# pola-rs/polars

Measured on AMD Instinct MI355X. Metric: rows/sec + achieved HBM GB/s, TPC-H Q1/Q3 SF100, 1/2/4/8 GPU vs CPU, higher is better.
Workload: dtype f64; 1 GPU; tpch_q1_sf100; rows_per_gpu=600000000, algorithmic_bytes_per_gpu_step=25200000000, parallelism=single GPU

## Files before the change

### include/polars_amd.h

```cpp
#ifndef POLARS_AMD_H
#define POLARS_AMD_H

#include <stddef.h>
#include <stdint.h>

#ifdef __cplusplus
extern "C" {
#endif

#define PLX_ABI_MAJOR 0
#define PLX_ABI_MINOR 1

#define PLX_OK 0
#define PLX_ERR_INVALID 1
#define PLX_ERR_HIP 2
#define PLX_ERR_UNSUPPORTED 3
#define PLX_ERR_OOM 4
#define PLX_ERR_SHAPE 5
#define PLX_ERR_NOT_FOUND 6
#define PLX_ERR_CANCELLED 7

typedef enum plx_dtype {
  PLX_BOOL = 0,
  PLX_I8 = 1,
// ... 226 lines not shown
  PLX_AE_CUMULATIVE = 16,
  PLX_AE_RANK = 17,
  PLX_AE_SHIFT = 18,
  PLX_AE_ROLLING = 19
} plx_aexpr_kind;

typedef enum plx_operator {
  PLX_OP_EQ = 0, PLX_OP_NE = 1, PLX_OP_LT = 2, PLX_OP_LE = 3, PLX_OP_GT = 4, PLX_OP_GE = 5,
  PLX_OP_PLUS = 6, PLX_OP_MINUS = 7, PLX_OP_MULTIPLY = 8, PLX_OP_TRUE_DIVIDE = 9,
  PLX_OP_FLOOR_DIVIDE = 10, PLX_OP_MODULUS = 11, PLX_OP_AND = 12, PLX_OP_OR = 13, PLX_OP_XOR = 14
} plx_operator;

typedef struct plx_aexpr {
  int32_t kind;
  int32_t op;
  int32_t lhs;
  int32_t rhs;
  int32_t dtype;
  int32_t is_null;
  plx_scalar lit;
  const char* name;
  int32_t cond;
} plx_aexpr;

typedef enum plx_ir_kind {
  PLX_IR_SCAN = 0,
  PLX_IR_FILTER = 1,
  PLX_IR_SELECT = 2,
  PLX_IR_HSTACK = 3,
  PLX_IR_GROUPBY = 4,
  PLX_IR_JOIN = 5,
  PLX_IR_SORT = 6,
  PLX_IR_SLICE = 7,
  PLX_IR_DISTINCT = 8
} plx_ir_kind;

typedef enum plx_join_order {
  PLX_JOIN_ORDER_NONE = 0,
  PLX_JOIN_ORDER_LEFT = 1,
  PLX_JOIN_ORDER_RIGHT = 2,
  PLX_JOIN_ORDER_LEFT_RIGHT = 3,
  PLX_JOIN_ORDER_RIGHT_LEFT = 4
} plx_join_order;

typedef struct plx_ir {
  int32_t kind;
  int32_t input;
  int32_t input_right;
  int32_t predicate;
  plx_frame frame;
  const int32_t* exprs;
  int32_t n_exprs;
  const int32_t* keys;
  int32_t n_keys;
  const int32_t* keys_right;
  int32_t n_keys_right;
  int32_t how;
  int32_t maintain_order;
  const char* suffix;
  const uint8_t* sort_descending;
  const uint8_t* sort_nulls_last;
  int64_t slice_offset;
  int64_t slice_len;
  int32_t coalesce;
} plx_ir;

#define PLX_PLAN_NO_FUSION 1u
#define PLX_PLAN_NO_PARTITION 4u
#define PLX_PLAN_NO_DIRECT_JOIN 2u

int plx_execute_plan(const plx_ir* ir, int32_t n_ir, const plx_aexpr* exprs, int32_t n_exprs, int32_t root,
                     uint32_t flags, plx_frame* out);
int plx_describe_fusion(const plx_ir* ir, int32_t n_ir, const plx_aexpr* exprs, int32_t n_exprs, int32_t root, int32_t* fusable,
                        int32_t* static_shape_id, char* why_not, size_t why_cap);
int plx_debug_program_json(const plx_ir* ir, int32_t n_ir, const plx_aexpr* exprs, int32_t n_exprs, int32_t root, char* buf, size_t cap);
int plx_jit_selftest(const plx_ir* ir, int32_t n_ir, const plx_aexpr* exprs, int32_t n_exprs, int32_t root);
int plx_jit_stats(int32_t* compiled, double* compile_ms);
int plx_jit_set_min_rows(int64_t min_rows);
const char* plx_last_plan_description(void);
const char* plx_last_plan_encodings(void);
int32_t plx_last_scan_tile_rows(void);
int32_t plx_last_lds_cells(void);
void plx_set_shared_cells(int32_t on);
int32_t plx_cell_plan(int32_t static_shape_id, int32_t n_inputs, const int32_t* dtypes, const int32_t* nullable, int32_t n_ops, const uint8_t* ops, int32_t n_aggs, const uint8_t* aggs,
                      const uint8_t* known, const int64_t* lo, const int64_t* hi, uint64_t wg_rows, uint64_t n_rows, int32_t* out);
uint64_t plx_lds_wg_rows(int64_t n_rows, int32_t grid, int32_t wide);
int32_t plx_wide_tiles_choice(int32_t compiled, int32_t knob_on, int64_t n_rows, int32_t n_inputs, const int32_t* dtypes, const int32_t* nullable, const uint64_t* values,
                              const uint64_t* validity);

int plx_datagen_lineitem_q1(int64_t n_rows, uint64_t seed, plx_column* out_cols);
int plx_datagen_lineitem_q1_host(int64_t row0, int64_t n, uint64_t seed, int64_t* shipdate, uint8_t* returnflag, uint8_t* linestatus,
                                 int64_t* quantity, double* extendedprice, double* discount, double* tax);

int plx_datagen_orders_lineitem(int64_t n_orders, uint64_t seed, plx_column* out_orders, plx_column* out_lineitem);
int plx_datagen_orders_lineitem_host(int64_t order0, int64_t n, int64_t n_orders_total, uint64_t seed, int64_t* orderkey, int64_t* custkey,
                                     int64_t* orderdate, uint32_t* n_lines, int64_t line_cap, int64_t* l_orderkey, double* l_extendedprice,
                                     double* l_discount, int64_t* l_shipdate, int64_t* n_lines_out);
int plx_datagen_customer(int64_t n_customers, uint64_t seed, plx_column* out_cols);
int plx_datagen_customer_host(int64_t row0, int64_t n, uint64_t seed, int64_t* custkey, uint8_t* segment);
int plx_datagen_uniform(int32_t dtype, int64_t n_rows, uint64_t seed, uint32_t stream, int64_t lo, int64_t hi, double scale, plx_column* out);
int plx_datagen_uniform_host(int32_t dtype, int64_t row0, int64_t n, uint64_t seed, uint32_t stream, int64_t lo, int64_t hi, double scale, void* out);
int plx_datagen_zipf(int64_t n_rows, uint64_t seed, uint32_t stream, uint64_t x0_q62, int64_t n_keys, plx_column* out);
int plx_datagen_zipf_host(int64_t row0, int64_t n, uint64_t seed, uint32_t stream, uint64_t x0_q62, int64_t n_keys, int64_t* out);

typedef uint64_t plx_strdict;
int plx_strview_dict_encode(const void* views, const uint8_t* validity, int64_t bit_offset, int64_t n, const void* const* data_buffers, const int64_t* data_sizes,
                            int32_t n_data_buffers, plx_column* out_codes, plx_strdict* out_dict);
int plx_strview_dict_encode_device(plx_column views_u64_pairs, plx_column data_u8, plx_column* out_codes, plx_strdict* out_dict);
int plx_strview_stamp_nulls(plx_column views_u64_pairs, plx_column valid_bool);
int plx_strview_groupby(plx_column views_u64_pairs, plx_column value, plx_column* out_codes, plx_strdict* out_dict, plx_column* out_sum, plx_column* out_count, plx_column* out_len);
#define PLX_STR_MATCH_MAX_PATTERN 64
typedef enum plx_str_match_kind { PLX_STR_STARTS_WITH = 0, PLX_STR_ENDS_WITH = 1, PLX_STR_CONTAINS = 2 } plx_str_match_kind;
int plx_strdict_match(plx_strdict dict, int32_t kind, const uint8_t* pattern, int64_t pattern_len, plx_column* out_bool);
int plx_strview_match(plx_column views_u64_pairs, plx_column data_u8, int32_t kind, const uint8_t* pattern, int64_t pattern_len, plx_column* out_bool);
int plx_strview_match_host(const void* views, const uint8_t* data, int64_t data_len, int64_t n, int32_t kind, const uint8_t* pattern, int64_t pattern_len,
                           uint64_t* out_bits, uint64_t* out_valid);
int plx_bitmap_lookup(plx_column codes, plx_column lut_bool, plx_column* out_bool);
int plx_strdict_info(plx_strdict dict, int64_t* n_strings, int64_t* total_bytes);

typedef enum plx_time_unit { PLX_UNIT_DATE = 0, PLX_UNIT_MS = 1, PLX_UNIT_US = 2, PLX_UNIT_NS = 3 } plx_time_unit;
typedef enum plx_temporal_part_kind {
  PLX_PART_YEAR = 0, PLX_PART_MONTH = 1, PLX_PART_DAY = 2, PLX_PART_QUARTER = 3, PLX_PART_WEEKDAY = 4, PLX_PART_ORDINAL_DAY = 5,
  PLX_PART_HOUR = 6, PLX_PART_MINUTE = 7, PLX_PART_SECOND = 8, PLX_PART_DATE = 9
} plx_temporal_part_kind;
int plx_temporal_part(plx_column col, int part, int unit, plx_column* out);
int plx_temporal_part_host(const void* values, int unit, int part, int64_t n, void* out);

int plx_strdict_to_host(plx_strdict dict, int64_t* offsets, uint8_t* bytes);
int plx_strdict_free(plx_strdict dict);
int plx_datagen_id_views(int64_t n_rows, uint64_t seed, uint32_t stream, int64_t lo, int64_t hi, plx_column* out_views);
int plx_datagen_long_id_views(int64_t n_rows, uint64_t seed, uint32_t stream, int64_t lo, int64_t hi, plx_column* out_views, plx_column* out_data);

typedef uint64_t plx_parquet;
int plx_parquet_open(const char* path, plx_parquet* out);
int plx_parquet_close(plx_parquet file);
int plx_parquet_shape(plx_parquet file, int64_t* num_rows, int32_t* num_row_groups, int32_t* num_columns);
int plx_parquet_column_info(plx_parquet file, int32_t column, const char** name, int32_t* dtype, int32_t* logical, int32_t* nullable);
int plx_parquet_column_timezone(plx_parquet file, int32_t column, const char** timezone);
int plx_parquet_row_group_info(plx_parquet file, int32_t row_group, int64_t* num_rows, int64_t* compressed_bytes);
int plx_parquet_chunk_info(plx_parquet file, int32_t row_group, int32_t column, int32_t* codec, uint32_t* encodings, int64_t* compressed_bytes,
                           int64_t* uncompressed_bytes, int32_t* has_min_max, plx_scalar* min, plx_scalar* max, int64_t* null_count);
int plx_parquet_read(plx_parquet file, const int32_t* row_groups, int32_t n_row_groups, const int32_t* columns, int32_t n_columns, plx_frame* out);
int plx_parquet_categories(plx_parquet file, int32_t column, int64_t* n_strings, int64_t* total_bytes);
int plx_parquet_categories_to_host(plx_parquet file, int32_t column, int64_t* offsets, uint8_t* bytes);
int plx_parquet_column_strdict(plx_parquet file, int32_t column, plx_strdict* out);

typedef uint64_t plx_ipc;
int plx_ipc_open(const char* path, plx_ipc* out);
int plx_ipc_close(plx_ipc file);
int plx_ipc_shape(plx_ipc file, int64_t* num_rows, int32_t* num_batches, int32_t* num_columns);
int plx_ipc_column_info(plx_ipc file, int32_t column, const char** name, int32_t* dtype, int32_t* logical, int32_t* nullable);
int plx_ipc_column_timezone(plx_ipc file, int32_t column, const char** timezone);
int plx_ipc_batch_info(plx_ipc file, int32_t batch, int64_t* num_rows, int64_t* body_bytes, int32_t* compressed);
int plx_ipc_read(plx_ipc file, const int32_t* batches, int32_t n_batches, const int32_t* columns, int32_t n_columns, plx_frame* out);
int plx_ipc_read_string_views(plx_ipc file, const int32_t* batches, int32_t n_batches, int32_t column, plx_column* out_views, plx_column* out_data);
int plx_ipc_categories(plx_ipc file, int32_t column, int64_t* n_strings, int64_t* total_bytes);
int plx_ipc_categories_to_host(plx_ipc file, int32_t column, int64_t* offsets, uint8_t* bytes);
int plx_ipc_column_strdict(plx_ipc file, int32_t column, plx_strdict* out);

typedef uint64_t plx_comm;
int plx_comm_unique_id(uint8_t* out_128_bytes);
int plx_comm_init(const uint8_t* unique_id_128_bytes, int32_t rank, int32_t world_size, plx_comm* out);
int plx_comm_info(plx_comm comm, int32_t* rank, int32_t* world_size);
int plx_comm_free(plx_comm comm);
int plx_exchange_by_key(plx_comm comm, plx_frame frame, const char* key, uint64_t seed, plx_frame* out, uint64_t* rows_sent, uint64_t* bytes_sent);
int plx_allgather_frame(plx_comm comm, plx_frame frame, plx_frame* out);
// ... 52 lines not shown
```

### polars_amd/_ffi.py

```python
from __future__ import annotations

import ctypes as C
import os
import threading
from typing import Optional

os.environ.setdefault("GPU_MAX_HW_QUEUES", "8")

_HERE = os.path.dirname(os.path.abspath(__file__))
LIB_PATH = os.path.join(_HERE, "libpolars_amd.so")

BOOL, I8, I16, I32, I64, U8, U16, U32, U64, F32, F64 = range(11)
EQ, NE, LT, LE, GT, GE = range(6)
ADD, SUB, MUL, TRUE_DIV, FLOOR_DIV, MOD = range(6)
AND, OR, XOR = range(3)
AGG_SUM, AGG_MEAN, AGG_MIN, AGG_MAX, AGG_COUNT, AGG_LEN, AGG_FIRST, AGG_VAR, AGG_STD = range(9)
AGG_QUANTILE = 9
AGG_N_UNIQUE = 10
UNIQUE_ANY, UNIQUE_FIRST, UNIQUE_LAST, UNIQUE_NONE = range(4)
UNIQUE_KEEPS = {"any": UNIQUE_ANY, "first": UNIQUE_FIRST, "last": UNIQUE_LAST, "none": UNIQUE_NONE}
QUANTILE_NEAREST, QUANTILE_LOWER, QUANTILE_HIGHER, QUANTILE_MIDPOINT, QUANTILE_LINEAR = range(5)
QUANTILE_INTERPOLATIONS = {"nearest": QUANTILE_NEAREST, "lower": QUANTILE_LOWER, "higher": QUANTILE_HIGHER, "midpoint": QUANTILE_MIDPOINT, "linear": QUANTILE_LINEAR}
JOIN_INNER, JOIN_LEFT, JOIN_SEMI, JOIN_ANTI, JOIN_FULL, JOIN_RIGHT = range(6)
JOIN_COALESCE_DEFAULT, JOIN_COALESCE, JOIN_KEEP_BOTH = range(3)
# ... 153 lines not shown
    "plx_parquet_column_strdict": (C.c_int, [C.c_uint64, C.c_int32, _u64p]),
    "plx_ipc_open": (C.c_int, [C.c_char_p, _u64p]),
    "plx_ipc_close": (C.c_int, [C.c_uint64]),
    "plx_ipc_shape": (C.c_int, [C.c_uint64, _i64p, _i32p, _i32p]),
    "plx_ipc_column_info": (C.c_int, [C.c_uint64, C.c_int32, C.POINTER(C.c_char_p), _i32p, _i32p, _i32p]),
    "plx_ipc_column_timezone": (C.c_int, [C.c_uint64, C.c_int32, C.POINTER(C.c_char_p)]),
    "plx_ipc_batch_info": (C.c_int, [C.c_uint64, C.c_int32, _i64p, _i64p, _i32p]),
    "plx_ipc_read": (C.c_int, [C.c_uint64, _i32p, C.c_int32, _i32p, C.c_int32, _u64p]),
    "plx_ipc_read_string_views": (C.c_int, [C.c_uint64, _i32p, C.c_int32, C.c_int32, _u64p, _u64p]),
    "plx_ipc_categories": (C.c_int, [C.c_uint64, C.c_int32, _i64p, _i64p]),
    "plx_ipc_categories_to_host": (C.c_int, [C.c_uint64, C.c_int32, C.c_void_p, C.c_void_p]),
    "plx_ipc_column_strdict": (C.c_int, [C.c_uint64, C.c_int32, _u64p]),
    "plx_comm_unique_id": (C.c_int, [C.c_void_p]),
    "plx_comm_init": (C.c_int, [C.c_void_p, C.c_int32, C.c_int32, _u64p]),
    "plx_comm_info": (C.c_int, [C.c_uint64, C.POINTER(C.c_int32), C.POINTER(C.c_int32)]),
    "plx_comm_free": (C.c_int, [C.c_uint64]),
    "plx_exchange_by_key": (C.c_int, [C.c_uint64, C.c_uint64, C.c_char_p, C.c_uint64, _u64p, _u64p, _u64p]),
    "plx_allgather_frame": (C.c_int, [C.c_uint64, C.c_uint64, _u64p]),
    "plx_column_import_arrow": (C.c_int, [C.POINTER(ArrowArray), C.POINTER(ArrowSchema), _u64p]),
    "plx_column_import_series": (C.c_int, [C.POINTER(SeriesExport), _u64p]),
    "plx_column_export_arrow": (C.c_int, [C.c_uint64, C.POINTER(ArrowArray), C.POINTER(ArrowSchema)]),
    "plx_column_export_series": (C.c_int, [C.c_uint64, C.c_char_p, C.POINTER(SeriesExport)]),
    "plx_column_to_host": (C.c_int, [C.c_uint64, C.c_void_p, C.c_void_p, _i32p]),
    "plx_column_copy_to_device": (C.c_int, [C.c_uint64, C.c_void_p, C.c_void_p]),
    "plx_column_info": (C.c_int, [C.c_uint64, _i32p, _i64p, _i64p]),
    "plx_column_device_ptrs": (C.c_int, [C.c_uint64, C.POINTER(C.c_void_p), C.POINTER(C.c_void_p)]),
    "plx_column_retain": (C.c_int, [C.c_uint64]),
    "plx_column_free": (C.c_int, [C.c_uint64]),
    "plx_cmp": (C.c_int, [C.c_int, C.c_uint64, C.c_uint64, _u64p]),
    "plx_cmp_scalar": (C.c_int, [C.c_int, C.c_uint64, Scalar, _u64p]),
    "plx_bitmap_binop": (C.c_int, [C.c_int, C.c_uint64, C.c_uint64, _u64p]),
    "plx_bitmap_not": (C.c_int, [C.c_uint64, _u64p]),
    "plx_arith": (C.c_int, [C.c_int, C.c_uint64, C.c_uint64, _u64p]),
    "plx_arith_scalar": (C.c_int, [C.c_int, C.c_uint64, Scalar, C.c_int, _u64p]),
    "plx_cast": (C.c_int, [C.c_uint64, C.c_int, _u64p]),
    "plx_if_then_else": (C.c_int, [C.c_uint64, C.c_uint64, C.c_uint64, _u64p]),
    "plx_filter": (C.c_int, [C.c_uint64, C.c_uint64, _u64p]),
    "plx_gather": (C.c_int, [C.c_uint64, C.c_uint64, _u64p]),
    "plx_reduce": (C.c_int, [C.c_int, C.c_uint64, C.POINTER(Scalar), _i32p, _i32p]),
    "plx_reduce_var": (C.c_int, [C.c_uint64, C.c_int32, C.c_int32, C.POINTER(Scalar), _i32p, _i32p]),
    "plx_groupby_agg": (C.c_int, [_u64p, C.c_int32, _u64p, _i32p, C.c_int32, C.c_int32, _u64p, _u64p]),
    "plx_groupby_agg_ddof": (C.c_int, [_u64p, C.c_int32, _u64p, _i32p, C.c_int32, C.c_int32, _i32p, _u64p, _u64p]),
    "plx_reduce_quantile": (C.c_int, [C.c_uint64, C.c_double, C.c_int32, C.POINTER(Scalar), _i32p, _i32p]),
    "plx_groupby_agg_params": (C.c_int, [_u64p, C.c_int32, _u64p, _i32p, C.c_int32, C.c_int32, _i32p, C.POINTER(C.c_double), _i32p, _u64p, _u64p]),
    "plx_window_agg": (C.c_int, [_u64p, C.c_int32, _u64p, _i32p, C.c_int32, _i32p, C.POINTER(C.c_double), _i32p, _u64p]),
    "plx_cumulative": (C.c_int, [_u64p, C.c_int32, C.c_uint64, C.c_int32, C.c_int32, _u64p]),
    "plx_rank": (C.c_int, [_u64p, C.c_int32, C.c_uint64, C.c_int32, C.c_int32, _u64p]),
    "plx_shift": (C.c_int, [_u64p, C.c_int32, C.c_uint64, C.c_int64, C.POINTER(Scalar), C.c_int32, _u64p]),
    "plx_rolling": (C.c_int, [_u64p, C.c_int32, C.c_uint64, C.c_int32, C.c_int64, C.c_int64, C.c_int32, _u64p]),
    "plx_join_indices": (C.c_int, [C.c_int, C.c_uint64, C.c_uint64, _u64p, _u64p]),
    "plx_datagen_lineitem_q1": (C.c_int, [C.c_int64, C.c_uint64, _u64p]),
    "plx_datagen_lineitem_q1_host": (C.c_int, [C.c_int64, C.c_int64, C.c_uint64, C.c_void_p, C.c_void_p, C.c_void_p, C.c_void_p, C.c_void_p, C.c_void_p, C.c_void_p]),
    "plx_datagen_orders_lineitem": (C.c_int, [C.c_int64, C.c_uint64, _u64p, _u64p]),
    "plx_datagen_orders_lineitem_host": (C.c_int, [C.c_int64, C.c_int64, C.c_int64, C.c_uint64, C.c_void_p, C.c_void_p, C.c_void_p, C.c_void_p, C.c_int64,
                                                   C.c_void_p, C.c_void_p, C.c_void_p, C.c_void_p, _i64p]),
    "plx_datagen_uniform": (C.c_int, [C.c_int32, C.c_int64, C.c_uint64, C.c_uint32, C.c_int64, C.c_int64, C.c_double, _u64p]),
    "plx_datagen_customer": (C.c_int, [C.c_int64, C.c_uint64, _u64p]),
    "plx_datagen_customer_host": (C.c_int, [C.c_int64, C.c_int64, C.c_uint64, C.c_void_p, C.c_void_p]),
    "plx_datagen_uniform_host": (C.c_int, [C.c_int32, C.c_int64, C.c_int64, C.c_uint64, C.c_uint32, C.c_int64, C.c_int64, C.c_double, C.c_void_p]),
    "plx_datagen_zipf": (C.c_int, [C.c_int64, C.c_uint64, C.c_uint32, C.c_uint64, C.c_int64, _u64p]),
    "plx_datagen_zipf_host": (C.c_int, [C.c_int64, C.c_int64, C.c_uint64, C.c_uint32, C.c_uint64, C.c_int64, C.c_void_p]),
    "plx_debug_program_json": (C.c_int, [C.POINTER(IR), C.c_int32, C.POINTER(AExpr), C.c_int32, C.c_int32, C.c_char_p, C.c_size_t]),
    "plx_reduce_n_unique": (C.c_int, [C.c_uint64, C.POINTER(C.c_uint32)]),
    "plx_distinct_mask": (C.c_int, [_u64p, C.c_int32, C.c_int32, _u64p]),
    "plx_sort_indices": (C.c_int, [_u64p, C.c_int32, C.POINTER(C.c_uint8), C.POINTER(C.c_uint8), C.c_int64, _u64p]),
    "plx_hash_partition": (C.c_int, [C.c_uint64, C.c_int32, C.c_uint64, _u64p, _i64p]),
    "plx_frame_new": (C.c_int, [C.POINTER(C.c_char_p), _u64p, C.c_int32, _u64p]),
    "plx_frame_free": (C.c_int, [C.c_uint64]),
    "plx_frame_concat": (C.c_int, [_u64p, C.c_int32, _u64p]),
    "plx_frame_shape": (C.c_int, [C.c_uint64, _i64p, _i32p]),
    "plx_frame_column": (C.c_int, [C.c_uint64, C.c_int32, C.POINTER(C.c_char_p), _u64p]),
    "plx_frame_dtypes": (C.c_int, [C.c_uint64, _i32p]),
    "plx_frame_to_host": (C.c_int, [C.c_uint64, C.POINTER(C.c_void_p), C.POINTER(C.c_void_p), _i32p]),
    "plx_execute_plan": (C.c_int, [C.POINTER(IR), C.c_int32, C.POINTER(AExpr), C.c_int32, C.c_int32, C.c_uint32, _u64p]),
    "plx_describe_fusion": (C.c_int, [C.POINTER(IR), C.c_int32, C.POINTER(AExpr), C.c_int32, C.c_int32, _i32p, _i32p, C.c_char_p, C.c_size_t]),
    "plx_jit_selftest": (C.c_int, [C.POINTER(IR), C.c_int32, C.POINTER(AExpr), C.c_int32, C.c_int32]),
    "plx_jit_stats": (C.c_int, [_i32p, C.POINTER(C.c_double)]),
    "plx_jit_set_min_rows": (C.c_int, [C.c_int64]),
    "plx_last_plan_description": (C.c_char_p, []),
    "plx_last_plan_encodings": (C.c_char_p, []),
    "plx_last_scan_tile_rows": (C.c_int32, []),
    "plx_last_lds_cells": (C.c_int32, []),
    "plx_set_shared_cells": (None, [C.c_int32]),
    "plx_cell_plan": (C.c_int32, [C.c_int32, C.c_int32, C.POINTER(C.c_int32), C.POINTER(C.c_int32), C.c_int32, C.POINTER(C.c_uint8), C.c_int32, C.POINTER(C.c_uint8),
                                  C.POINTER(C.c_uint8), C.POINTER(C.c_int64), C.POINTER(C.c_int64), C.c_uint64, C.c_uint64, C.POINTER(C.c_int32)]),
    "plx_lds_wg_rows": (C.c_uint64, [C.c_int64, C.c_int32, C.c_int32]),
    "plx_wide_tiles_choice": (C.c_int32, [C.c_int32, C.c_int32, C.c_int64, C.c_int32, C.POINTER(C.c_int32), C.POINTER(C.c_int32), C.POINTER(C.c_uint64), C.POINTER(C.c_uint64)]),
    "plx_profile_enable": (C.c_int, [C.c_int]),
    "plx_profile_fetch": (C.c_int, [C.POINTER(ProfileRecord), C.c_int32, _i32p]),
    "plx_profile_clear": (C.c_int, []),
}

_lib: Optional[C.CDLL] = None


def lib() -> C.CDLL:
    global _lib
    if _lib is None:
        if not os.path.exists(LIB_PATH):
            raise ImportError(
                f"{LIB_PATH} is missing: build the HIP extension first "
                "(python -c 'import __graft_entry__ as g; g.build()' or make -C polars_amd/csrc). "
                "There is no CPU fallback in polars_amd.")
        l = C.CDLL(LIB_PATH, mode=C.RTLD_GLOBAL)
        for name, (res, args) in SIGNATURES.items():
            fn = getattr(l, name)
            fn.restype = res
            fn.argtypes = args
        _lib = l
    return _lib


def check(status: int) -> None:
    if status != 0:
        msg = lib().plx_last_error().decode("utf-8", "replace")
        if status == ERR_UNSUPPORTED:
            raise UnsupportedError(status, msg)
        raise PlxError(status, msg)


_initialised = False


def init(device: Optional[int] = None) -> None:
    global _initialised
    if device is None:
        device = int(os.environ.get("LOCAL_RANK", "0"))
    check(lib().plx_init(device))
    _initialised = True


def ensure_init() -> None:
    if not _initialised:
        init()


_tls = threading.local()


def set_plan_note(note) -> None:
    _tls.plan_note = note


def last_plan() -> str:
    note = getattr(_tls, "plan_note", None)
    return note if note is not None else lib().plx_last_plan_description().decode()


def last_plan_encodings() -> str:
    return lib().plx_last_plan_encodings().decode()


def last_scan_tile_rows() -> int:
    return int(lib().plx_last_scan_tile_rows())


def last_lds_cells() -> int:
    return int(lib().plx_last_lds_cells())


def set_shared_cells(on: bool) -> None:
    lib().plx_set_shared_cells(int(bool(on)))


def cell_plan(facts, wg_rows, n_rows, static_shape_id=-1, dtypes=(), nullable=(), ops=(), aggs=()):
    n_aggs = len(facts)
    ni, no = len(dtypes), len(ops)
    out = (C.c_int32 * (2 + 2 * 16))()
    flat_ops = [int(x) for op in ops for x in op]
    flat_aggs = [int(x) for a in aggs for x in a]
    r = lib().plx_cell_plan(int(static_shape_id), ni, (C.c_int32 * max(ni, 1))(*[int(d) for d in dtypes]), (C.c_int32 * max(ni, 1))(*[int(x) for x in nullable]),
                            no, (C.c_uint8 * max(len(flat_ops), 1))(*flat_ops), len(aggs), (C.c_uint8 * max(len(flat_aggs), 1))(*flat_aggs),
                            (C.c_uint8 * 16)(*[int(f[0]) for f in facts]), (C.c_int64 * 16)(*[int(f[1]) for f in facts]), (C.c_int64 * 16)(*[int(f[2]) for f in facts]),
                            int(wg_rows), int(n_rows), out)
    if r < 0:
        raise ValueError("plx_cell_plan: bad arguments")
    return int(out[0]), int(out[1]), [int(out[2 + k]) for k in range(r)], [int(out[2 + r + k]) for k in range(r)]


def wide_tiles_choice(compiled, knob_on, n_rows, dtypes, nullable, values, validity) -> int:
    n = len(dtypes)
    return int(lib().plx_wide_tiles_choice(int(bool(compiled)), int(bool(knob_on)), int(n_rows), n, (C.c_int32 * n)(*[int(d) for d in dtypes]),
                                           (C.c_int32 * n)(*[int(bool(x)) for x in nullable]), (C.c_uint64 * n)(*[int(v) for v in values]), (C.c_uint64 * n)(*[int(v) for v in validity])))


def jit_set_min_rows(min_rows: int) -> None:
    check(lib().plx_jit_set_min_rows(int(min_rows)))


def encoded_set_decimal_min_rows(min_rows: int) -> None:
    check(lib().plx_encoded_set_decimal_min_rows(int(min_rows)))


def encoded_decimal_min_rows() -> int:
    return int(lib().plx_encoded_decimal_min_rows())


def jit_stats():
    n, ms = C.c_int32(), C.c_double()
    check(lib().plx_jit_stats(C.byref(n), C.byref(ms)))
    return n.value, ms.value
```

### polars_amd/csrc/abi.cpp

```cpp
#include <cstdio>
#include <cstring>
#include <memory>
#include <mutex>

#include "core.hpp"
#include "datagen_device.hpp"
#include "distinct.hpp"
#include "encoded_inputs.hpp"
#include "engine.hpp"
#include "fused_shapes.hpp"
#include "jit.hpp"
#include "join.hpp"
#include "kernels.hpp"
#include "kernels_fused.hpp"
#include "ops.hpp"
#include "cumulative.hpp"
#include "quantile.hpp"
#include "rolling.hpp"
#include "scan.hpp"
#include "sort.hpp"
#include "strmatch.hpp"
#include "temporal.hpp"

namespace plx {
// ... 543 lines not shown
  PLX_REQUIRE(by && n_by > 0 && out_idx, PLX_ERR_INVALID, "sort_indices: need at least one key column");
  std::vector<sort::SortKey> keys;
  for (int i = 0; i < n_by; i++) {
    sort::SortKey k;
    k.col = get_column(by[i]); k.descending = descending && descending[i]; k.nulls_last = nulls_last && nulls_last[i];
    keys.push_back(k);
  }
  std::string d;
  ColumnPtr idx = sort::sort_indices(keys, limit, &d);
  t_plan_desc = d;
  *out_idx = register_column(idx);
  PLX_CATCH
}

int plx_hash_partition(plx_column key, int32_t n_partitions, uint64_t seed, plx_column* out_perm, int64_t* counts_out) {
  PLX_TRY
  PLX_REQUIRE(out_perm && counts_out, PLX_ERR_INVALID, "null pointer");
  ColumnPtr perm;
  join::hash_partition(get_column(key), n_partitions, seed, perm, counts_out);
  *out_perm = register_column(perm);
  PLX_CATCH
}

int plx_frame_new(const char* const* names, const plx_column* cols, int32_t n_cols, plx_frame* out) {
  PLX_TRY
  PLX_REQUIRE(out && (n_cols == 0 || (names && cols)), PLX_ERR_INVALID, "null pointer");
  auto f = std::make_shared<Frame>();
  for (int i = 0; i < n_cols; i++) {
    ColumnPtr c = get_column(cols[i]);
    if (i == 0) f->height = c->len;
    PLX_REQUIRE(c->len == f->height, PLX_ERR_SHAPE, std::string("frame columns have different lengths (") + names[i] + ")");
    PLX_REQUIRE(f->find(names[i]) < 0, PLX_ERR_INVALID, std::string("duplicate column name ") + names[i]);
    f->names.push_back(names[i]); f->cols.push_back(c);
  }
  *out = register_frame(f);
  PLX_CATCH
}
int plx_frame_free(plx_frame f) { PLX_TRY free_frame(f); PLX_CATCH }
int plx_frame_concat(const plx_frame* frames, int32_t n_frames, plx_frame* out) {
  PLX_TRY
  PLX_REQUIRE(frames && out && n_frames >= 1, PLX_ERR_INVALID, "frame_concat: bad arguments");
  std::vector<FramePtr> fs;
  for (int32_t i = 0; i < n_frames; i++) fs.push_back(get_frame(frames[i]));
  auto o = std::make_shared<Frame>();
  o->names = fs[0]->names;
  for (const FramePtr& f : fs) {
    PLX_REQUIRE(f->names == o->names, PLX_ERR_SHAPE, "frame_concat: frames have different columns");
    o->height += f->height;
  }
  for (size_t c = 0; c < o->names.size(); c++) {
    std::vector<ColumnPtr> chunks;
    for (const FramePtr& f : fs) chunks.push_back(f->cols[c]);
    o->cols.push_back(ops::concat(chunks));
  }
  *out = register_frame(o);
  PLX_CATCH
}
int plx_frame_shape(plx_frame f, int64_t* height, int32_t* width) {
  PLX_TRY
  FramePtr fr = get_frame(f);
  if (height) *height = fr->height;
  if (width) *width = (int32_t)fr->cols.size();
  PLX_CATCH
}
int plx_frame_column(plx_frame f, int32_t i, const char** name_out, plx_column* col_out) {
  PLX_TRY
  FramePtr fr = get_frame(f);
  PLX_REQUIRE(i >= 0 && i < (int)fr->cols.size(), PLX_ERR_INVALID, "column index out of range");
  if (name_out) *name_out = fr->names[i].c_str();
  if (col_out) *col_out = register_column(fr->cols[i]);
  PLX_CATCH
}

int plx_frame_dtypes(plx_frame f, int32_t* dtypes_out) {
  PLX_TRY
  FramePtr fr = get_frame(f);
  PLX_REQUIRE(dtypes_out || fr->cols.empty(), PLX_ERR_INVALID, "null pointer");
  for (size_t i = 0; i < fr->cols.size(); i++) dtypes_out[i] = fr->cols[i]->dtype;
  PLX_CATCH
}
int plx_frame_to_host(plx_frame f, void* const* values_out, uint8_t* const* validity_out, int32_t* has_validity_out) {
  PLX_TRY
  FramePtr fr = get_frame(f);
  {
    struct Piece { const void* src; void* dst; size_t bytes; };
    std::vector<Piece> pieces;
    size_t total = 0;
    bool ok = pinned_bounce() != nullptr;
    for (size_t i = 0; ok && i < fr->cols.size(); i++) {
      const ColumnPtr& c = fr->cols[i];
      if (!(c->values || c->len == 0)) { ok = false; break; }
      const size_t vb = c->dtype == PLX_BOOL ? (size_t)((c->len + 7) / 8) : (size_t)c->len * dtype_width(c->dtype);
      const size_t nb = (size_t)((c->len + 7) / 8);
      if (values_out && values_out[i] && vb) { pieces.push_back({c->values->ptr, values_out[i], vb}); total += (vb + 15) & ~size_t(15); }
      if (validity_out && validity_out[i] && nb && c->validity) { pieces.push_back({c->validity->ptr, validity_out[i], nb}); total += (nb + 15) & ~size_t(15); }
      if (total > kBounceBytes) ok = false;
    }
    if (ok && !pieces.empty()) {
      Buf staging = dev_alloc(total);
      std::vector<size_t> offs(pieces.size());
      size_t at = 0;
      for (size_t j = 0; j < pieces.size(); j++) { offs[j] = at; at += (pieces[j].bytes + 15) & ~size_t(15); }
      for (size_t base = 0; base < pieces.size(); base += k::kPackMax) {
        k::PackBatch b{}; b.n = (int)std::min<size_t>(k::kPackMax, pieces.size() - base);
        for (int j = 0; j < b.n; j++) { b.src[j] = pieces[base + j].src; b.bytes[j] = (uint32_t)pieces[base + j].bytes; b.off[j] = (uint32_t)offs[base + j]; }
        k::pack_buffers(b, staging->ptr);
      }
      std::lock_guard<std::mutex> lk(bounce_mutex());
      uint8_t* host = reinterpret_cast<uint8_t*>(pinned_bounce());
      PLX_HIP(hipMemcpyAsync(host, staging->ptr, total, hipMemcpyDeviceToHost, stream()));
      PLX_HIP(hipStreamSynchronize(stream()));
      for (size_t j = 0; j < pieces.size(); j++) memcpy(pieces[j].dst, host + offs[j], pieces[j].bytes);
      for (size_t i = 0; i < fr->cols.size(); i++) {
        const ColumnPtr& c = fr->cols[i];
        const size_t nb = (size_t)((c->len + 7) / 8);
        if (validity_out && validity_out[i] && nb && !c->validity) memset(validity_out[i], 0xff, nb);
        if (has_validity_out) has_validity_out[i] = c->validity ? 1 : 0;
      }
      return PLX_OK;
    }
    if (ok && pieces.empty() && !fr->cols.empty()) {
      for (size_t i = 0; i < fr->cols.size(); i++) if (has_validity_out) has_validity_out[i] = fr->cols[i]->validity ? 1 : 0;
      return PLX_OK;
    }
  }
  for (size_t i = 0; i < fr->cols.size(); i++) {
    const ColumnPtr& c = fr->cols[i];
    PLX_REQUIRE(c->values || c->len == 0, PLX_ERR_INVALID, "placeholder column has no data");
    const size_t vb = c->dtype == PLX_BOOL ? (size_t)((c->len + 7) / 8) : (size_t)c->len * dtype_width(c->dtype);
    const size_t nb = (size_t)((c->len + 7) / 8);
    if (values_out && values_out[i] && vb) PLX_HIP(hipMemcpyAsync(values_out[i], c->values->ptr, vb, hipMemcpyDeviceToHost, stream()));
    if (validity_out && validity_out[i] && nb) {
      if (c->validity) PLX_HIP(hipMemcpyAsync(validity_out[i], c->validity->ptr, nb, hipMemcpyDeviceToHost, stream()));
      else memset(validity_out[i], 0xff, nb);
    }
    if (has_validity_out) has_validity_out[i] = c->validity ? 1 : 0;
  }
  PLX_HIP(hipStreamSynchronize(stream()));
  PLX_CATCH
}

extern "C++" {
namespace {
thread_local std::string t_plugin_error;
struct PluginCtx { uint64_t bitflags; };

hipStream_t plugin_thread_stream() {
  static thread_local hipStream_t s = nullptr;
  if (!s) PLX_HIP(hipStreamCreateWithFlags(&s, hipStreamNonBlocking));
  return s;
}
std::string pickle_str_value(const uint8_t* kw, size_t n, const char* key) {
  std::vector<std::string> toks;
  for (size_t i = 0; i < n;) {
    const uint8_t c = kw[i];
    size_t len = 0, hdr = 0;
    if ((c == 0x8c || c == 'U') && i + 1 < n) { len = kw[i + 1]; hdr = 2; }
    else if (c == 'X' && i + 4 < n) { len = (size_t)kw[i + 1] | ((size_t)kw[i + 2] << 8) | ((size_t)kw[i + 3] << 16) | ((size_t)kw[i + 4] << 24); hdr = 5; }
    if (hdr && i + hdr + len <= n) { toks.emplace_back((const char*)kw + i + hdr, len); i += hdr + len; }
    else i++;
  }
  for (size_t i = 0; i + 1 < toks.size(); i++) if (toks[i] == key) return toks[i + 1];
  return "";
}
long long pickle_int_value(const uint8_t* kw, size_t n, const char* key, long long absent) {
  const size_t klen = strlen(key);
// ... 536 lines not shown
    for (uint32_t q = 0; q < r.n_lines; q++, at++) {
      if (!want_lines) continue;
      PLX_REQUIRE(at < line_cap, PLX_ERR_INVALID, "datagen: line arrays too small");
      const datagen::Q3LineRow lr = datagen::q3_line_row(seed, (uint64_t)(order0 + j), q, r.orderdate);
      if (l_orderkey) l_orderkey[at] = r.orderkey;
      if (l_extendedprice) l_extendedprice[at] = lr.extendedprice;
      if (l_discount) l_discount[at] = lr.discount;
      if (l_shipdate) l_shipdate[at] = lr.shipdate;
    }
  }
  if (n_lines_out) *n_lines_out = at;
  PLX_CATCH
}
int plx_datagen_customer(int64_t n_customers, uint64_t seed, plx_column* out_cols) {
  PLX_TRY
  PLX_REQUIRE(n_customers >= 0 && out_cols, PLX_ERR_INVALID, "datagen: bad arguments");
  ColumnPtr k = make_column(PLX_I64, n_customers, false), sgm = make_column(PLX_U8, n_customers, false);
  k->null_count = 0; sgm->null_count = 0;
  k::datagen_customer(n_customers, seed, k->values->as<int64_t>(), sgm->values->as<uint8_t>());
  out_cols[0] = register_column(k); out_cols[1] = register_column(sgm);
  PLX_CATCH
}
int plx_datagen_customer_host(int64_t row0, int64_t n, uint64_t seed, int64_t* custkey, uint8_t* segment) {
  PLX_TRY
  PLX_REQUIRE(row0 >= 0 && n >= 0, PLX_ERR_INVALID, "datagen: bad arguments");
  for (int64_t j = 0; j < n; j++) {
    if (custkey) custkey[j] = row0 + j + 1;
    if (segment) segment[j] = datagen::customer_segment(seed, (uint64_t)(row0 + j + 1));
  }
  PLX_CATCH
}
int plx_datagen_uniform(int32_t dtype, int64_t n_rows, uint64_t seed, uint32_t stream_id, int64_t lo, int64_t hi, double scale, plx_column* out) {
  PLX_TRY
  PLX_REQUIRE(n_rows >= 0 && out && hi > lo && stream_id < 8, PLX_ERR_INVALID, "datagen: bad arguments");
  PLX_REQUIRE(dtype == PLX_I64 || dtype == PLX_U32 || dtype == PLX_F64, PLX_ERR_UNSUPPORTED, "datagen_uniform: dtype must be Int64, UInt32 or Float64");
  ColumnPtr c = make_column(dtype, n_rows, false); c->null_count = 0;
  k::datagen_uniform(dtype, n_rows, seed, stream_id, lo, hi, scale, c->values->ptr);
  *out = register_column(c);
  PLX_CATCH
}
int plx_datagen_uniform_host(int32_t dtype, int64_t row0, int64_t n, uint64_t seed, uint32_t stream_id, int64_t lo, int64_t hi, double scale, void* out) {
  PLX_TRY
  PLX_REQUIRE(row0 >= 0 && n >= 0 && (out || n == 0) && hi > lo && stream_id < 8, PLX_ERR_INVALID, "datagen: bad arguments");
  PLX_REQUIRE(dtype == PLX_I64 || dtype == PLX_U32 || dtype == PLX_F64, PLX_ERR_UNSUPPORTED, "datagen_uniform: dtype must be Int64, UInt32 or Float64");
  for (int64_t j = 0; j < n; j++) {
    const int64_t v = datagen::uniform_value(seed, stream_id, (uint64_t)(row0 + j), lo, hi);
    if (dtype == PLX_I64) reinterpret_cast<int64_t*>(out)[j] = v;
    else if (dtype == PLX_U32) reinterpret_cast<uint32_t*>(out)[j] = (uint32_t)v;
    else reinterpret_cast<double*>(out)[j] = (double)v * scale;
  }
  PLX_CATCH
}

int plx_datagen_zipf(int64_t n_rows, uint64_t seed, uint32_t stream_id, uint64_t x0_q62, int64_t n_keys, plx_column* out) {
  PLX_TRY
  PLX_REQUIRE(n_rows >= 0 && out && n_keys > 0 && stream_id < 8 && x0_q62 > 0 && x0_q62 < (1ull << 62), PLX_ERR_INVALID, "datagen_zipf: bad arguments");
  ColumnPtr c = make_column(PLX_I64, n_rows, false); c->null_count = 0;
  k::datagen_zipf(n_rows, seed, stream_id, x0_q62, n_keys, c->values->as<int64_t>());
  *out = register_column(c);
  PLX_CATCH
}
int plx_datagen_zipf_host(int64_t row0, int64_t n, uint64_t seed, uint32_t stream_id, uint64_t x0_q62, int64_t n_keys, int64_t* out) {
  PLX_TRY
  PLX_REQUIRE(row0 >= 0 && n >= 0 && (out || n == 0) && n_keys > 0 && stream_id < 8 && x0_q62 > 0 && x0_q62 < (1ull << 62), PLX_ERR_INVALID, "datagen_zipf: bad arguments");
  for (int64_t j = 0; j < n; j++) out[j] = datagen::zipf_value(seed, stream_id, (uint64_t)(row0 + j), x0_q62, n_keys);
  PLX_CATCH
}

int plx_execute_plan(const plx_ir* ir, int32_t n_ir, const plx_aexpr* exprs, int32_t n_exprs, int32_t root, uint32_t flags, plx_frame* out) {
  PLX_TRY
  PLX_REQUIRE(out, PLX_ERR_INVALID, "null out pointer");
  engine::Plan p = engine::import_plan(ir, n_ir, exprs, n_exprs, flags);
  FramePtr f = engine::execute(p, root);
  t_plan_desc = p.desc;
  t_plan_encoded = p.encoded;
  *out = register_frame(f);
  PLX_CATCH
}
const char* plx_last_plan_description(void) { return t_plan_desc.c_str(); }
const char* plx_last_plan_encodings(void) { return t_plan_encoded.c_str(); }
int32_t plx_last_scan_tile_rows(void) { return k::last_scan_tile_rows(); }
int32_t plx_last_lds_cells(void) { return k::last_lds_cells(); }
void plx_set_shared_cells(int32_t on) { k::set_shared_cells(on != 0); }
uint64_t plx_lds_wg_rows(int64_t n_rows, int32_t grid, int32_t wide) { return (n_rows < 0 || grid < 1) ? 0 : k::lds_agg_wg_rows_of(n_rows, grid, wide != 0); }
int32_t plx_cell_plan(int32_t static_shape_id, int32_t n_inputs, const int32_t* dtypes, const int32_t* nullable, int32_t n_ops, const uint8_t* ops, int32_t n_aggs, const uint8_t* aggs,
                      const uint8_t* known, const int64_t* lo, const int64_t* hi, uint64_t wg_rows, uint64_t n_rows, int32_t* out) {
  if (!known || !lo || !hi || !out) return -1;
  fused::Shape sh{};
  if (static_shape_id >= 0) {
    if (static_shape_id >= fused::kNumStaticShapes) return -1;
    sh = fused::static_shape(static_shape_id);
  } else {
    if (n_inputs < 0 || n_inputs > fused::kMaxInputs || n_ops < 0 || n_ops > fused::kMaxOps || n_aggs < 0 || n_aggs > fused::kMaxAggs) return -1;
    if ((n_inputs && (!dtypes || !nullable)) || (n_ops && !ops) || (n_aggs && !aggs)) return -1;
    sh.n_inputs = (uint8_t)n_inputs; sh.n_ops = (uint8_t)n_ops; sh.n_aggs = (uint8_t)n_aggs; sh.pred = fused::kNone; sh.key = fused::kNone;
    for (int i = 0; i < n_inputs; i++) { sh.in_dtype[i] = (uint8_t)dtypes[i]; sh.in_nullable[i] = (uint8_t)(nullable[i] != 0); }
    for (int i = 0; i < n_ops; i++) sh.ops[i] = fused::Op{ops[5 * i], ops[5 * i + 1], ops[5 * i + 2], ops[5 * i + 3], ops[5 * i + 4], {0, 0, 0}};
    for (int i = 0; i < n_aggs; i++) sh.aggs[i] = fused::Agg{aggs[2 * i], aggs[2 * i + 1]};
  }
  fused::AggFacts f{};
  f.wg_rows = wg_rows; f.n_rows = n_rows;
  for (int k = 0; k < sh.n_aggs; k++) { f.known[k] = known[k]; f.lo[k] = lo[k]; f.hi[k] = hi[k]; }
  const fused::CellPlan p = fused::plan_cells(sh, f);
  out[0] = p.n_cells; out[1] = p.shift;
  for (int k = 0; k < sh.n_aggs; k++) { out[2 + k] = p.cell[k]; out[2 + sh.n_aggs + k] = p.from[k] == fused::kNone ? -1 : (int)p.from[k]; }
  return sh.n_aggs;
}
int32_t plx_wide_tiles_choice(int32_t compiled, int32_t knob_on, int64_t n_rows, int32_t n_inputs, const int32_t* dtypes, const int32_t* nullable, const uint64_t* values,
                              const uint64_t* validity) {
  if (n_inputs < 0 || n_inputs > fused::kMaxInputs || (n_inputs && (!dtypes || !nullable || !values || !validity))) return -1;
  fused::Shape sh{}; fused::Args args{};
  sh.n_inputs = (uint8_t)n_inputs; sh.pred = fused::kNone; sh.key = fused::kNone;
  args.n_rows = n_rows;
  for (int i = 0; i < n_inputs; i++) {
    sh.in_dtype[i] = (uint8_t)dtypes[i]; sh.in_nullable[i] = (uint8_t)(nullable[i] != 0);
    args.in[i].values = (const void*)(uintptr_t)values[i]; args.in[i].validity = (const uint64_t*)(uintptr_t)validity[i];
  }
  return k::wide_tiles_choice(sh, args, compiled != 0, knob_on != 0) ? 1 : 0;
}

int plx_debug_program_json(const plx_ir* ir, int32_t n_ir, const plx_aexpr* exprs, int32_t n_exprs, int32_t root, char* buf, size_t cap) {
  PLX_TRY
  PLX_REQUIRE(buf && cap > 0, PLX_ERR_INVALID, "null buffer");
  engine::Plan p = engine::import_plan(ir, n_ir, exprs, n_exprs, 0);
  std::string json, why;
  if (!engine::dump_program_json(p, root, &json, &why)) fail(PLX_ERR_UNSUPPORTED, "not a fusable pipeline: " + why);
  PLX_REQUIRE(json.size() + 1 <= cap, PLX_ERR_INVALID, "buffer too small for the program dump (" + std::to_string(json.size() + 1) + " bytes)");
  memcpy(buf, json.c_str(), json.size() + 1);
  PLX_CATCH
}

int plx_describe_fusion(const plx_ir* ir, int32_t n_ir, const plx_aexpr* exprs, int32_t n_exprs, int32_t root, int32_t* fusable, int32_t* static_shape_id,
                        char* why_not, size_t why_cap) {
  PLX_TRY
  engine::Plan p = engine::import_plan(ir, n_ir, exprs, n_exprs, 0);
  auto dump = [](const fused::Shape& sh) {
    std::string d = "inputs=" + std::to_string(sh.n_inputs) + " pred=" + std::to_string(sh.pred) + " key=" + std::to_string(sh.key) + " ops=[";
    for (int i = 0; i < sh.n_ops; i++) d += "(" + std::to_string(sh.ops[i].code) + "," + std::to_string(sh.ops[i].dst) + "," + std::to_string(sh.ops[i].a) + "," + std::to_string(sh.ops[i].b) + "," + std::to_string(sh.ops[i].c) + ")";
    d += "] aggs=[";
    for (int i = 0; i < sh.n_aggs; i++) d += "(" + std::to_string(sh.aggs[i].kind) + "," + std::to_string(sh.aggs[i].src) + ")";
    d += "] in_dtype=[";
    for (int i = 0; i < sh.n_inputs; i++) d += std::to_string(sh.in_dtype[i]) + (sh.in_nullable[i] ? "?" : "") + ",";
    d += "]";
    if (sh.n_keys) { d += " keys=["; for (int i = 0; i < sh.n_keys; i++) d += std::to_string(sh.keys[i]) + ","; d += "]"; }
    return d;
  };
  std::string why;
  int sid = -1;
  bool ok;
  PLX_REQUIRE(root >= 0 && root < (int)p.ir.size(), PLX_ERR_INVALID, "bad root");
  const engine::IRN& rn = p.ir[root];
  if (rn.kind == PLX_IR_GROUPBY && rn.input >= 0 && p.ir[rn.input].kind == PLX_IR_JOIN) {
    std::vector<fused::Shape> shapes;
    ok = engine::describe_join_fusion(p, root, &shapes, &why);
    if (ok) {
      sid = fused::find_static_shape(shapes[2]);
      t_plan_desc = dump(shapes[0]);
      for (size_t i = 1; i < shapes.size(); i++) t_plan_desc += "\n" + dump(shapes[i]);
    }
  } else {
    fused::Shape sh{};
    ok = engine::describe_fusion(p, root, &sh, &sid, &why);
    if (ok) t_plan_desc = dump(sh);
  }
  if (fusable) *fusable = ok ? 1 : 0;
  if (static_shape_id) *static_shape_id = sid;
// ... 103 lines not shown
  Buf codes, dviews, svalid;
  int64_t nd = 0, snulls = 0;
  k::strview_dict_encode(views, validity_holder ? validity_holder->valid_words() : nullptr, data ? data->as<uint8_t>() : nullptr, buf_base ? buf_base->as<uint64_t>() : nullptr, n, &codes, &dviews, &nd,
                         from_stamps && !validity_holder ? &svalid : nullptr, &snulls);
  auto c = std::make_shared<Column>();
  c->dtype = PLX_U32; c->len = n; c->values = codes;
  if (validity_holder && validity_holder->validity) c->validity = validity_holder->validity;
  else if (snulls > 0) { c->validity = svalid; c->null_count = snulls; }
  else c->null_count = 0;
  if (nd > 0) { c->range_state = 1; c->range_min = 0; c->range_max = nd - 1; c->range_trusted = true; }
  auto d = std::make_unique<StrDict>();
  d->views = dviews; d->data = data; d->n = nd;
  *out_codes = register_column(c);
  *out_dict = register_strdict(std::move(d));
}
}
namespace plx {
void strview_encode_device(const uint64_t* views, const ColumnPtr& validity_holder, Buf data, int64_t n, plx_column* out_codes, plx_strdict* out_dict) {
  Buf bb = dev_alloc_zero(8);
  encode_on_device(views, validity_holder, data, bb, n, out_codes, out_dict);
}
void strview_encode_device_bases(const uint64_t* views, const ColumnPtr& validity_holder, Buf data, Buf buf_base, int64_t n, plx_column* out_codes, plx_strdict* out_dict) {
  encode_on_device(views, validity_holder, data, buf_base, n, out_codes, out_dict);
}
}
}

int plx_strview_dict_encode(const void* views, const uint8_t* validity, int64_t bit_offset, int64_t n, const void* const* data_buffers, const int64_t* data_sizes,
                            int32_t n_data_buffers, plx_column* out_codes, plx_strdict* out_dict) {
  PLX_TRY
  PLX_REQUIRE(out_codes && out_dict && n >= 0 && (views || n == 0) && n_data_buffers >= 0 && (n_data_buffers == 0 || (data_buffers && data_sizes)), PLX_ERR_INVALID, "strview_dict_encode: bad arguments");
  device();
  Buf dv = dev_alloc((size_t)std::max<int64_t>(n, 1) * 16);
  if (n) h2d_sync_pinned(dv->ptr, views, (size_t)n * 16);
  ColumnPtr vh;
  if (validity) {
    std::vector<uint8_t> zeros((size_t)n);
    vh = column_from_host(PLX_U8, zeros.data(), validity, bit_offset, n);
  }
  uint64_t total = 0;
  std::vector<uint64_t> base((size_t)std::max(n_data_buffers, 1), 0);
  for (int i = 0; i < n_data_buffers; i++) { base[i] = total; total += (uint64_t)data_sizes[i]; }
  Buf data = dev_alloc((size_t)total + 64), bb = dev_alloc(sizeof(uint64_t) * base.size());
  for (int i = 0; i < n_data_buffers; i++) {
    if (!data_sizes[i]) continue;
    if ((uint64_t)data_sizes[i] >= ((uint64_t)32 << 20)) h2d_sync_pinned((uint8_t*)data->ptr + base[i], data_buffers[i], (size_t)data_sizes[i]);
    else h2d_async((uint8_t*)data->ptr + base[i], data_buffers[i], (size_t)data_sizes[i]);
  }
  h2d_async(bb->ptr, base.data(), sizeof(uint64_t) * base.size());
  PLX_HIP(hipStreamSynchronize(stream()));
  encode_on_device(dv->as<uint64_t>(), vh, data, bb, n, out_codes, out_dict);
  PLX_CATCH
}
int plx_strview_dict_encode_device(plx_column views_u64_pairs, plx_column data_u8, plx_column* out_codes, plx_strdict* out_dict) {
  PLX_TRY
  PLX_REQUIRE(out_codes && out_dict, PLX_ERR_INVALID, "null pointer");
  ColumnPtr v = get_column(views_u64_pairs);
  PLX_REQUIRE(v->dtype == PLX_U64 && v->len % 2 == 0 && (v->values || v->len == 0), PLX_ERR_INVALID, "views must be a UInt64 column of 2 n words");
  Buf data, bb = dev_alloc_zero(8);
  if (data_u8) { ColumnPtr d = get_column(data_u8); PLX_REQUIRE(d->dtype == PLX_U8, PLX_ERR_INVALID, "data must be a UInt8 column"); data = d->values; }
  const int64_t n = v->len / 2;
  encode_on_device(v->values ? v->values->as<uint64_t>() : nullptr, nullptr, data, bb, n, out_codes, out_dict, true);
  PLX_CATCH
}
int plx_strview_stamp_nulls(plx_column views_u64_pairs, plx_column valid_bool) {
  PLX_TRY
  ColumnPtr v = get_column(views_u64_pairs), m = get_column(valid_bool);
  PLX_REQUIRE(v->dtype == PLX_U64 && v->len % 2 == 0, PLX_ERR_INVALID, "views must be a UInt64 column of 2 n words");
  PLX_REQUIRE(m->dtype == PLX_BOOL, PLX_ERR_INVALID, "the validity of the views is a Boolean column (true = valid: the array's validity bitmap as its values)");
  PLX_REQUIRE(m->len == v->len / 2, PLX_ERR_SHAPE, "validity column and views differ in length");
  PLX_REQUIRE((v->values && m->values) || v->len == 0, PLX_ERR_INVALID, "placeholder column has no data");
  if (!v->len) return PLX_OK;
  ColumnPtr eff = m;
  if (m->validity) {
    auto a = std::make_shared<Column>(); a->dtype = PLX_BOOL; a->len = m->len; a->values = m->values; a->null_count = 0;
    auto b = std::make_shared<Column>(); b->dtype = PLX_BOOL; b->len = m->len; b->values = m->validity; b->null_count = 0;
    eff = ops::bool_binop(PLX_AND, a, b);
  }
  if (!v->values->owned || v->values.use_count() > 1) {
    Buf copy = dev_alloc(v->values->bytes);
    PLX_HIP(hipMemcpyAsync(copy->ptr, v->values->ptr, v->values->bytes, hipMemcpyDeviceToDevice, stream()));
    v->values = copy;
  }
  k::strview_stamp_nulls(v->values->as<uint64_t>(), eff->values->as<uint64_t>(), m->len);
  PLX_HIP(hipStreamSynchronize(stream()));
  PLX_CATCH
}
extern "C++" {
namespace {
void check_match_args(int32_t kind, const uint8_t* pattern, int64_t pattern_len) {
  PLX_REQUIRE(kind >= PLX_STR_STARTS_WITH && kind <= PLX_STR_CONTAINS, PLX_ERR_INVALID, "string match: kind outside 0..2 (plx_str_match_kind)");
  PLX_REQUIRE(pattern_len >= 0 && (pattern || pattern_len == 0), PLX_ERR_INVALID, "string match: bad pattern");
  PLX_REQUIRE(pattern_len <= PLX_STR_MATCH_MAX_PATTERN, PLX_ERR_UNSUPPORTED,
              "string match: a pattern of " + std::to_string(pattern_len) + " bytes; patterns of more than " + std::to_string(PLX_STR_MATCH_MAX_PATTERN) + " bytes are not on this path");
}
void check_match_flags(uint32_t flags) {
  PLX_REQUIRE(!(flags & strmatch::kFlagOutside), PLX_ERR_INVALID, "string match: a view points outside its buffer");
  PLX_REQUIRE(!(flags & strmatch::kFlagNoData), PLX_ERR_INVALID, "string match: a string of more than 12 bytes needs the data buffer for this predicate, and none was given");
}
ColumnPtr bool_column(int64_t n, Buf values, Buf validity, int64_t null_count) {
  auto c = std::make_shared<Column>();
  c->dtype = PLX_BOOL; c->len = n; c->values = std::move(values); c->validity = std::move(validity); c->null_count = null_count;
  return c;
}
}
}
static_assert(PLX_STR_MATCH_MAX_PATTERN == strmatch::kMaxPattern && PLX_STR_STARTS_WITH == strmatch::kStartsWith && PLX_STR_ENDS_WITH == strmatch::kEndsWith && PLX_STR_CONTAINS == strmatch::kContains,
              "polars_amd.h and strmatch.hpp disagree");

int plx_strdict_match(plx_strdict dict, int32_t kind, const uint8_t* pattern, int64_t pattern_len, plx_column* out_bool) {
  PLX_TRY
  PLX_REQUIRE(out_bool, PLX_ERR_INVALID, "null pointer");
  check_match_args(kind, pattern, pattern_len);
  StrDict& d = get_strdict(dict);
  device();
  Buf bits = dev_alloc(bitmap_bytes(d.n)), valid = dev_alloc(bitmap_bytes(d.n));
  const uint32_t flags = k::strview_match(d.views->as<uint64_t>(), nullptr, false, d.data ? d.data->as<uint8_t>() : nullptr, d.data ? (uint64_t)d.data->bytes : 0, true, d.n,
                                          kind, pattern, pattern_len, bits->as<uint64_t>(), valid->as<uint64_t>());
  check_match_flags(flags);
  *out_bool = register_column(bool_column(d.n, bits, nullptr, 0));
  PLX_CATCH
}
int plx_strview_match(plx_column views_u64_pairs, plx_column data_u8, int32_t kind, const uint8_t* pattern, int64_t pattern_len, plx_column* out_bool) {
  PLX_TRY
  PLX_REQUIRE(out_bool, PLX_ERR_INVALID, "null pointer");
  check_match_args(kind, pattern, pattern_len);
  ColumnPtr v = get_column(views_u64_pairs);
  PLX_REQUIRE(v->dtype == PLX_U64 && v->len % 2 == 0, PLX_ERR_INVALID, "views must be a UInt64 column of 2 n words");
  PLX_REQUIRE(v->values || v->len == 0, PLX_ERR_INVALID, "placeholder column has no data");
  PLX_REQUIRE(!v->validity || column_null_count(v) == 0, PLX_ERR_INVALID, "views column carries a validity bitmap with nulls: the nulls of a raw view column are stamped views (plx_strview_stamp_nulls)");
  Buf data;
  uint64_t data_len = 0;
  if (data_u8) {
    ColumnPtr d = get_column(data_u8);
    PLX_REQUIRE(d->dtype == PLX_U8, PLX_ERR_INVALID, "data must be a UInt8 column");
    PLX_REQUIRE(d->values || d->len == 0, PLX_ERR_INVALID, "placeholder column has no data");
    data = d->values; data_len = (uint64_t)d->len;
  }
  device();
  const int64_t n = v->len / 2;
  Buf bits = dev_alloc(bitmap_bytes(n)), valid = dev_alloc(bitmap_bytes(n));
  const uint32_t flags = k::strview_match(v->values ? v->values->as<uint64_t>() : nullptr, nullptr, true, data ? data->as<uint8_t>() : nullptr, data_len, false, n,
                                          kind, pattern, pattern_len, bits->as<uint64_t>(), valid->as<uint64_t>());
  check_match_flags(flags);
  const int64_t n_valid = n ? k::bitmap_popcount(valid->as<uint64_t>(), n) : 0;
  *out_bool = register_column(n_valid == n ? bool_column(n, bits, nullptr, 0) : bool_column(n, bits, valid, n - n_valid));
  PLX_CATCH
}
int plx_strview_match_host(const void* views, const uint8_t* data, int64_t data_len, int64_t n, int32_t kind, const uint8_t* pattern, int64_t pattern_len, uint64_t* out_bits,
                           uint64_t* out_valid) {
  PLX_TRY
  PLX_REQUIRE(n >= 0 && (views || n == 0) && (out_bits && out_valid || n == 0) && data_len >= 0, PLX_ERR_INVALID, "strview_match_host: bad arguments");
  check_match_args(kind, pattern, pattern_len);
  const strmatch::Pattern pat = strmatch::make_pattern(pattern, pattern_len);
  const strmatch::Pool pool{data, data ? (uint64_t)data_len : 0, 0};
  const uint32_t flags = strmatch::match_views_host(views, pool, n, kind, pat, out_bits, out_valid);
  check_match_flags(flags);
  PLX_CATCH
}
int plx_bitmap_lookup(plx_column codes, plx_column lut_bool, plx_column* out_bool) {
  PLX_TRY
  PLX_REQUIRE(out_bool, PLX_ERR_INVALID, "null pointer");
  *out_bool = register_column(ops::bitmap_lookup(get_column(codes), get_column(lut_bool)));
  PLX_CATCH
}

// ... 129 lines not shown
```

### polars_amd/csrc/comm.cpp

```cpp
#include <dlfcn.h>

#include <algorithm>
#include <cstring>
#include <mutex>

#include "core.hpp"
#include "join.hpp"
#include "ops.hpp"

namespace plx {
namespace {

typedef struct { char internal[128]; } NcclId;
typedef void* NcclComm;
enum { kNcclUint8 = 1, kNcclInt64 = 4 };
struct Rccl {
  void* so = nullptr;
  int (*GetUniqueId)(NcclId*) = nullptr;
  int (*CommInitRank)(NcclComm*, int, NcclId, int) = nullptr;
  int (*CommDestroy)(NcclComm) = nullptr;
  int (*CommCount)(const NcclComm, int*) = nullptr;
  int (*CommUserRank)(const NcclComm, int*) = nullptr;
  int (*Send)(const void*, size_t, int, int, NcclComm, hipStream_t) = nullptr;
  int (*Recv)(void*, size_t, int, int, NcclComm, hipStream_t) = nullptr;
  int (*AllGather)(const void*, void*, size_t, int, NcclComm, hipStream_t) = nullptr;
  int (*GroupStart)() = nullptr;
  int (*GroupEnd)() = nullptr;
  const char* (*GetErrorString)(int) = nullptr;
};
Rccl& rccl() {
  static Rccl r;
  static std::once_flag once;
  std::call_once(once, [] {
    for (const char* name : {"librccl.so.1", "librccl.so", "/opt/rocm/lib/librccl.so.1"}) { r.so = dlopen(name, RTLD_NOW | RTLD_GLOBAL); if (r.so) break; }
    if (!r.so) return;
    auto sym = [&](const char* n) { return dlsym(r.so, n); };
    r.GetUniqueId = (decltype(r.GetUniqueId))sym("ncclGetUniqueId");
    r.CommInitRank = (decltype(r.CommInitRank))sym("ncclCommInitRank");
    r.CommDestroy = (decltype(r.CommDestroy))sym("ncclCommDestroy");
    r.CommCount = (decltype(r.CommCount))sym("ncclCommCount");
    r.CommUserRank = (decltype(r.CommUserRank))sym("ncclCommUserRank");
    r.Send = (decltype(r.Send))sym("ncclSend");
    r.Recv = (decltype(r.Recv))sym("ncclRecv");
    r.AllGather = (decltype(r.AllGather))sym("ncclAllGather");
    r.GroupStart = (decltype(r.GroupStart))sym("ncclGroupStart");
    r.GroupEnd = (decltype(r.GroupEnd))sym("ncclGroupEnd");
    r.GetErrorString = (decltype(r.GetErrorString))sym("ncclGetErrorString");
  });
  if (!r.so || !r.GetUniqueId || !r.CommInitRank || !r.Send || !r.Recv || !r.AllGather || !r.GroupStart || !r.GroupEnd)
    fail(PLX_ERR_HIP, "librccl could not be loaded (multi-GPU exchange needs RCCL)");
  return r;
}
void nccl_check(int rc, const char* what) {
  if (rc != 0) fail(PLX_ERR_HIP, std::string(what) + ": " + (rccl().GetErrorString ? rccl().GetErrorString(rc) : "rccl error") + " (" + std::to_string(rc) + ")");
}

struct Comm { NcclComm nccl = nullptr; int rank = 0, ws = 1; };

constexpr size_t kP2PChunk = size_t(1) << 29;
void send_chunked(const uint8_t* src, size_t bytes, int peer, Comm& c) {
  for (size_t o = 0; o < bytes; o += kP2PChunk) nccl_check(rccl().Send(src + o, std::min(kP2PChunk, bytes - o), kNcclUint8, peer, c.nccl, stream()), "ncclSend");
}
void recv_chunked(uint8_t* dst, size_t bytes, int peer, Comm& c) {
  for (size_t o = 0; o < bytes; o += kP2PChunk) nccl_check(rccl().Recv(dst + o, std::min(kP2PChunk, bytes - o), kNcclUint8, peer, c.nccl, stream()), "ncclRecv");
}
std::mutex g_comm_mu;
std::vector<std::unique_ptr<Comm>> g_comms;

Comm& get_comm(uint64_t h) {
  std::lock_guard<std::mutex> lk(g_comm_mu);
  if (h == 0 || h > g_comms.size() || !g_comms[h - 1]) fail(PLX_ERR_INVALID, "invalid communicator handle");
  return *g_comms[h - 1];
}

std::vector<int64_t> allgather_i64(Comm& c, const Buf& send, size_t n) {
  const int ws = c.ws;
  Buf all = dev_alloc(sizeof(int64_t) * n * (size_t)ws);
  nccl_check(rccl().AllGather(send->ptr, all->ptr, n, kNcclInt64, c.nccl, stream()), "ncclAllGather(counts)");
  std::vector<int64_t> host(n * (size_t)ws);
  d2h_sync(host.data(), all->ptr, host.size() * 8);
  return host;
}

struct Wire { ColumnPtr data; size_t width; };
ColumnPtr bitmap_as_bytes(const Buf& bits, int64_t n) {
  auto b = std::make_shared<Column>();
  b->dtype = PLX_BOOL; b->len = n; b->values = bits; b->null_count = 0;
  return ops::cast(b, PLX_U8);
}
Buf bytes_as_bitmap(const ColumnPtr& bytes) {
  plx_scalar zero; zero.u = 0;
  return ops::cmp_scalar(PLX_NE, bytes, zero)->values;
}
void column_wires(const ColumnPtr& col, bool with_validity, std::vector<Wire>& out) {
  if (col->dtype == PLX_BOOL) out.push_back({bitmap_as_bytes(col->values, col->len), 1});
  else {
    auto v = std::make_shared<Column>(*col);
    v->validity = nullptr;
    out.push_back({v, (size_t)dtype_width(col->dtype)});
  }
  if (with_validity) {
    if (col->validity) out.push_back({bitmap_as_bytes(col->validity, col->len), 1});
    else { plx_scalar one; one.u = 1; out.push_back({ops::full_column(PLX_U8, one, true, col->len), 1}); }
  }
}
ColumnPtr column_from_wires(int dtype, int64_t n, bool with_validity, const std::vector<ColumnPtr>& recv, size_t& wi) {
  ColumnPtr o;
  if (dtype == PLX_BOOL) {
    o = std::make_shared<Column>();
    o->dtype = PLX_BOOL; o->len = n; o->values = bytes_as_bitmap(recv[wi++]);
  } else o = recv[wi++];
  o->dtype = dtype;
  if (with_validity) { o->validity = bytes_as_bitmap(recv[wi++]); o->null_count = -1; }
  else { o->validity = nullptr; o->null_count = 0; }
  return o;
}

}

namespace comm {

void unique_id(uint8_t* out128) {
  NcclId id;
  nccl_check(rccl().GetUniqueId(&id), "ncclGetUniqueId");
  memcpy(out128, id.internal, 128);
}

uint64_t init(const uint8_t* id128, int rank, int ws) {
  PLX_REQUIRE(ws >= 1 && rank >= 0 && rank < ws && id128, PLX_ERR_INVALID, "comm_init: bad arguments");
  device();
  NcclId id;
  memcpy(id.internal, id128, 128);
  auto c = std::make_unique<Comm>();
  c->rank = rank; c->ws = ws;
  nccl_check(rccl().CommInitRank(&c->nccl, ws, id, rank), "ncclCommInitRank");
  std::lock_guard<std::mutex> lk(g_comm_mu);
  g_comms.push_back(std::move(c));
  return (uint64_t)g_comms.size();
}

void destroy(uint64_t h) {
  std::unique_ptr<Comm> c;
  {
    std::lock_guard<std::mutex> lk(g_comm_mu);
    if (h == 0 || h > g_comms.size() || !g_comms[h - 1]) return;
    c = std::move(g_comms[h - 1]);
  }
  (void)hipStreamSynchronize(stream());
  if (c->nccl && rccl().CommDestroy) (void)rccl().CommDestroy(c->nccl);
}

void info(uint64_t h, int* rank, int* ws) {
  Comm& c = get_comm(h);
  int r = c.rank, w = c.ws;
  if (c.nccl && rccl().CommCount && rccl().CommUserRank) {
    nccl_check(rccl().CommCount(c.nccl, &w), "ncclCommCount");
    nccl_check(rccl().CommUserRank(c.nccl, &r), "ncclCommUserRank");
    PLX_REQUIRE(r == c.rank && w == c.ws, PLX_ERR_HIP, "communicator disagrees with its initialisation: rank " + std::to_string(r) + " of " + std::to_string(w) +
                " (initialised as " + std::to_string(c.rank) + " of " + std::to_string(c.ws) + ")");
  }
  if (rank) *rank = r;
  if (ws) *ws = w;
}

FramePtr exchange_by_key(uint64_t h, const FramePtr& in, const std::string& key, uint64_t seed, uint64_t* rows_sent, uint64_t* bytes_sent) {
  Comm& c = get_comm(h);
  const int ws = c.ws;
  const int ki = in->find(key);
  PLX_REQUIRE(ki >= 0, PLX_ERR_NOT_FOUND, "exchange_by_key: key column not found: " + key);
  const size_t nc = in->cols.size();
  ColumnPtr perm;
  Buf counts_dev;
  join::hash_partition_dev(in->cols[ki], ws, seed, perm, counts_dev);
  Buf send = dev_alloc(sizeof(int64_t) * ((size_t)ws + nc));
  PLX_HIP(hipMemcpyAsync(send->ptr, counts_dev->ptr, sizeof(int64_t) * (size_t)ws, hipMemcpyDeviceToDevice, stream()));
  std::vector<int64_t> flags(nc, 0);
  for (size_t i = 0; i < nc; i++) flags[i] = (in->cols[i]->validity && in->cols[i]->null_count != 0) ? 1 : 0;
  if (nc) h2d_async((uint8_t*)send->ptr + sizeof(int64_t) * (size_t)ws, flags.data(), sizeof(int64_t) * nc);
  const size_t stride = (size_t)ws + nc;
  const std::vector<int64_t> all = allgather_i64(c, send, stride);
  std::vector<int64_t> send_cnt((size_t)ws), recv_cnt((size_t)ws), send_off((size_t)ws + 1, 0), recv_off((size_t)ws + 1, 0);
// ... 78 lines not shown
```

### polars_amd/csrc/core.cpp

```cpp
#include "core.hpp"

#include <algorithm>
#include <atomic>
#include <chrono>
#include <cstdio>
#include <cstdlib>

namespace plx {

static thread_local std::string t_last_error;
void set_last_error(const std::string& m) { t_last_error = m; }
const std::string& last_error_ref() { return t_last_error; }

const char* dtype_name(int dt) {
  static const char* n[] = {"bool", "i8", "i16", "i32", "i64", "u8", "u16", "u32", "u64", "f32", "f64"};
  return (dt >= 0 && dt <= PLX_F64) ? n[dt] : "?";
}

static Device g_dev;
static std::mutex g_dev_mu;
static thread_local hipStream_t t_stream = nullptr;
static thread_local bool t_stream_set = false;

bool device_ready() { return g_dev.ordinal >= 0; }
// ... 146 lines not shown
void* pinned_bounce() {
  static void* buf = [] { void* p = nullptr; if (hipHostMalloc(&p, kBounceBytes, hipHostMallocDefault) != hipSuccess) { (void)hipGetLastError(); p = nullptr; } return p; }();
  return buf;
}
static std::mutex g_bounce_mu;
std::mutex& bounce_mutex() { return g_bounce_mu; }
void d2h_sync(void* dst, const void* src, size_t bytes) {
  if (bytes == 0) return;
  void* b = bytes <= 4096 ? pinned_bounce() : nullptr;
  if (b) {
    std::lock_guard<std::mutex> lk(g_bounce_mu);
    PLX_HIP(hipMemcpyAsync(b, src, bytes, hipMemcpyDeviceToHost, stream()));
    PLX_HIP(hipStreamSynchronize(stream()));
    memcpy(dst, b, bytes);
    return;
  }
  PLX_HIP(hipMemcpyAsync(dst, src, bytes, hipMemcpyDeviceToHost, stream()));
  PLX_HIP(hipStreamSynchronize(stream()));
}
void h2d_async(void* dst, const void* src, size_t bytes) {
  if (bytes == 0) return;
  PLX_HIP(hipMemcpyAsync(dst, src, bytes, hipMemcpyHostToDevice, stream()));
}

static const size_t kPinThreshold = size_t(32) << 20;
void h2d_sync_pinned(void* dst, const void* src, size_t bytes) {
  if (bytes == 0) return;
  static const bool pin = [] { const char* e = getenv("PLX_PIN_UPLOADS"); return !(e && e[0] == '0'); }();
  bool registered = false;
  if (pin && bytes >= kPinThreshold) registered = hipHostRegister(const_cast<void*>(src), bytes, hipHostRegisterDefault) == hipSuccess;
  if (!registered) (void)hipGetLastError();
  const hipError_t e = hipMemcpyAsync(dst, src, bytes, hipMemcpyHostToDevice, stream());
  const hipError_t e2 = hipStreamSynchronize(stream());
  if (registered) (void)hipHostUnregister(const_cast<void*>(src));
  PLX_HIP(e);
  PLX_HIP(e2);
}

ColumnPtr make_column(int dtype, int64_t len, bool with_validity) {
  auto c = std::make_shared<Column>();
  c->dtype = dtype; c->len = len;
  c->values = (dtype == PLX_BOOL) ? dev_alloc_zero(bitmap_bytes(len)) : dev_alloc(values_bytes(dtype, len));
  if (with_validity) c->validity = dev_alloc_zero(bitmap_bytes(len)); else c->null_count = 0;
  return c;
}

static std::vector<uint8_t> repack_bits(const uint8_t* bits, int64_t bit_offset, int64_t len) {
  std::vector<uint8_t> out(bitmap_bytes(len), 0);
  if (bit_offset % 8 == 0) { memcpy(out.data(), bits + bit_offset / 8, (size_t)((len + 7) / 8)); }
  else {
    for (int64_t i = 0; i < len; i++) {
      int64_t j = i + bit_offset;
      if ((bits[j >> 3] >> (j & 7)) & 1) out[i >> 3] |= uint8_t(1u << (i & 7));
    }
  }
  if (len & 7) out[(len - 1) >> 3] &= uint8_t((1u << (len & 7)) - 1);
  return out;
}

ColumnPtr column_from_host(int dtype, const void* values, const uint8_t* validity, int64_t bit_offset, int64_t len) {
  PLX_REQUIRE(dtype >= PLX_BOOL && dtype <= PLX_F64, PLX_ERR_INVALID, "column_from_host: bad dtype");
  PLX_REQUIRE(len >= 0, PLX_ERR_INVALID, "column_from_host: negative length");
  auto c = std::make_shared<Column>();
  c->dtype = dtype; c->len = len;
  std::vector<uint8_t> vbits, nbits;
  if (dtype == PLX_BOOL) {
    c->values = dev_alloc_zero(bitmap_bytes(len));
    if (len) { vbits = repack_bits((const uint8_t*)values, bit_offset, len); h2d_async(c->values->ptr, vbits.data(), vbits.size()); }
  } else {
    c->values = dev_alloc(values_bytes(dtype, len));
    h2d_sync_pinned(c->values->ptr, values, (size_t)len * dtype_width(dtype));
  }
  if (validity) {
    nbits = repack_bits(validity, bit_offset, len);
    int64_t nulls = 0;
    for (int64_t i = 0; i < len; i++) nulls += !((nbits[i >> 3] >> (i & 7)) & 1);
    c->null_count = nulls;
    if (nulls > 0) { c->validity = dev_alloc_zero(bitmap_bytes(len)); h2d_async(c->validity->ptr, nbits.data(), nbits.size()); }
  } else c->null_count = 0;
  PLX_HIP(hipStreamSynchronize(stream()));
  return c;
}

void column_to_host(const ColumnPtr& c, void* values_out, uint8_t* validity_out, int32_t* has_validity) {
  size_t vb = c->dtype == PLX_BOOL ? (size_t)((c->len + 7) / 8) : (size_t)c->len * dtype_width(c->dtype);
  if (values_out && vb) PLX_HIP(hipMemcpyAsync(values_out, c->values->ptr, vb, hipMemcpyDeviceToHost, stream()));
  size_t nb = (size_t)((c->len + 7) / 8);
  if (validity_out && nb) {
    if (c->validity) PLX_HIP(hipMemcpyAsync(validity_out, c->validity->ptr, nb, hipMemcpyDeviceToHost, stream()));
    else memset(validity_out, 0xff, nb);
  }
  if (has_validity) *has_validity = c->validity ? 1 : 0;
  PLX_HIP(hipStreamSynchronize(stream()));
}

namespace {
std::mutex g_h_mu;
std::unordered_map<uint64_t, std::pair<ColumnPtr, int>> g_cols;
std::unordered_map<uint64_t, FramePtr> g_frames;
uint64_t g_next_handle = 1;
}

plx_column register_column(ColumnPtr c) {
  std::lock_guard<std::mutex> lk(g_h_mu);
  uint64_t h = g_next_handle++;
  g_cols[h] = {std::move(c), 1};
  return h;
}
ColumnPtr get_column(plx_column h) {
  std::lock_guard<std::mutex> lk(g_h_mu);
  auto it = g_cols.find(h);
  if (it == g_cols.end()) fail(PLX_ERR_INVALID, "invalid column handle " + std::to_string(h));
  return it->second.first;
}
void retain_column(plx_column h) {
  std::lock_guard<std::mutex> lk(g_h_mu);
  auto it = g_cols.find(h);
  if (it == g_cols.end()) fail(PLX_ERR_INVALID, "invalid column handle " + std::to_string(h));
  it->second.second++;
}
void free_column(plx_column h) {
  ColumnPtr keep;
  std::lock_guard<std::mutex> lk(g_h_mu);
  auto it = g_cols.find(h);
  if (it == g_cols.end()) fail(PLX_ERR_INVALID, "invalid column handle " + std::to_string(h));
  if (--it->second.second == 0) { keep = std::move(it->second.first); g_cols.erase(it); }
}
plx_frame register_frame(FramePtr f) {
  std::lock_guard<std::mutex> lk(g_h_mu);
  uint64_t h = g_next_handle++;
  g_frames[h] = std::move(f);
  return h;
}
FramePtr get_frame(plx_frame h) {
  std::lock_guard<std::mutex> lk(g_h_mu);
  auto it = g_frames.find(h);
  if (it == g_frames.end()) fail(PLX_ERR_INVALID, "invalid frame handle " + std::to_string(h));
  return it->second;
}
void free_frame(plx_frame h) {
  FramePtr keep;
  std::lock_guard<std::mutex> lk(g_h_mu);
  auto it = g_frames.find(h);
  if (it == g_frames.end()) fail(PLX_ERR_INVALID, "invalid frame handle " + std::to_string(h));
  keep = std::move(it->second);
  g_frames.erase(it);
}
void clear_handles() {
  std::lock_guard<std::mutex> lk(g_h_mu);
  g_cols.clear(); g_frames.clear();
}

namespace {
struct Rec { std::string name; hipEvent_t a, b; uint64_t bytes, rows; };
std::mutex g_p_mu;
bool g_prof_on = false;
hipEvent_t g_prof_origin = nullptr;
std::vector<Rec> g_recs;
}

void profile_enable(bool on) {
  std::lock_guard<std::mutex> lk(g_p_mu);
  if (on && !g_prof_origin) { PLX_HIP(hipEventCreate(&g_prof_origin)); }
  if (on) PLX_HIP(hipEventRecord(g_prof_origin, stream()));
  g_prof_on = on;
}
ProfileScope::ProfileScope(const char* name, uint64_t algo_bytes, uint64_t rows) {
// ... 37 lines not shown
```

### polars_amd/csrc/core.hpp

```cpp
#pragma once
#include <hip/hip_runtime_api.h>

#include <atomic>
#include <cstdint>
#include <cstring>
#include <exception>
#include <map>
#include <memory>
#include <mutex>
#include <string>
#include <unordered_map>
#include <vector>

#include "../../include/polars_amd.h"

namespace plx {

struct Error : std::exception {
  int code;
  std::string msg;
  Error(int c, std::string m) : code(c), msg(std::move(m)) {}
  const char* what() const noexcept override { return msg.c_str(); }
};
[[noreturn]] inline void fail(int code, const std::string& m) { throw Error(code, m); }
void set_last_error(const std::string& m);

#define PLX_HIP(expr)                                                                          \
  do {                                                                                         \
    hipError_t _e = (expr);                                                                    \
    if (_e != hipSuccess)                                                                      \
      ::plx::fail(PLX_ERR_HIP, std::string(#expr) + ": " + hipGetErrorString(_e) + " (" __FILE__ ":" + std::to_string(__LINE__) + ")"); \
  } while (0)
#define PLX_REQUIRE(cond, code, msg) \
  do { if (!(cond)) ::plx::fail(code, msg); } while (0)

inline int dtype_width(int dt) {
  switch (dt) {
    case PLX_I8: case PLX_U8: return 1;
    case PLX_I16: case PLX_U16: return 2;
    case PLX_I32: case PLX_U32: case PLX_F32: return 4;
    case PLX_I64: case PLX_U64: case PLX_F64: return 8;
    default: return 0;
  }
}
inline bool dtype_is_float(int dt) { return dt == PLX_F32 || dt == PLX_F64; }
inline bool dtype_is_signed(int dt) { return dt >= PLX_I8 && dt <= PLX_I64; }
inline bool dtype_is_unsigned(int dt) { return dt >= PLX_U8 && dt <= PLX_U64; }
inline bool dtype_is_int(int dt) { return dt >= PLX_I8 && dt <= PLX_U64; }
const char* dtype_name(int dt);
inline size_t bitmap_bytes(int64_t n) { return (size_t)(((n + 63) / 64) * 8 + 8); }
inline size_t values_bytes(int dt, int64_t n) { return dt == PLX_BOOL ? bitmap_bytes(n) : (size_t)n * dtype_width(dt); }

struct Device {
  int ordinal = -1;
  int cu_count = 256;
  uint64_t hbm_bytes = 0;
  std::string name;
  hipStream_t own_stream = nullptr;
  std::atomic<int> cancel{0};
};
Device& device();
bool device_ready();
hipStream_t stream();
void set_thread_stream(hipStream_t s);
void check_cancel();

struct DevBuf {
  void* ptr = nullptr;
  size_t bytes = 0;
  size_t cap = 0;
  bool owned = true;
  ~DevBuf();
  template <class T> T* as() const { return reinterpret_cast<T*>(ptr); }
};
using Buf = std::shared_ptr<DevBuf>;
Buf dev_alloc(size_t bytes);
Buf dev_alloc_zero(size_t bytes);
Buf dev_alloc_transient(size_t bytes);
void pool_reserve(size_t bytes);
Buf dev_borrow(void* p, size_t bytes);
void pool_stats(uint64_t* in_use, uint64_t* high_water);
void pool_trim(bool force = false);

struct EncodedShadow {
  enum Kind { kNone = 0, kAffine = 1, kDict = 2, kDecimal = 3 };
  int kind = kNone;
  int width = 0;
  int64_t base = 0;
  uint64_t stride = 1;
  Buf codes;
  Buf dict;
  int n_dict = 0;
  int scans = 0;
  bool never_encode = false;
};
struct Column {
  int dtype = PLX_I64;
  int64_t len = 0;
  Buf values;
  Buf validity;
  int64_t null_count = -1;
  int range_state = 0;
  int64_t range_min = 0, range_max = 0;
  bool range_trusted = true;
  bool range_assumed = false;
  bool range_verified = false;
  bool no_assume = false;
  std::shared_ptr<void> key_sample;
  int order_state = 0;
  std::shared_ptr<EncodedShadow> shadow;
  bool repeats_as_build_key = false;
  const void* data() const { return values ? values->ptr : nullptr; }
  const uint64_t* valid_words() const { return validity ? validity->as<uint64_t>() : nullptr; }
};
using ColumnPtr = std::shared_ptr<Column>;

struct Frame {
  std::vector<std::string> names;
  std::vector<ColumnPtr> cols;
  int64_t height = 0;
  int find(const std::string& n) const {
    for (size_t i = 0; i < names.size(); i++) if (names[i] == n) return (int)i;
    return -1;
  }
};
using FramePtr = std::shared_ptr<Frame>;

ColumnPtr make_column(int dtype, int64_t len, bool with_validity);
ColumnPtr column_from_host(int dtype, const void* values, const uint8_t* validity, int64_t bit_offset, int64_t len);
int64_t column_null_count(const ColumnPtr& c);
void column_to_host(const ColumnPtr& c, void* values_out, uint8_t* validity_out, int32_t* has_validity);

plx_column register_column(ColumnPtr c);
ColumnPtr get_column(plx_column h);
void retain_column(plx_column h);
void free_column(plx_column h);
plx_frame register_frame(FramePtr f);
FramePtr get_frame(plx_frame h);
void free_frame(plx_frame h);

struct ProfileScope {
  int idx = -1;
  ProfileScope(const char* name, uint64_t algo_bytes, uint64_t rows);
  ~ProfileScope();
};
void profile_enable(bool on);
int profile_fetch(plx_profile_record* out, int cap);
void profile_clear();

void d2h_sync(void* dst, const void* src, size_t bytes);
constexpr size_t kBounceBytes = size_t(1) << 20;
void* pinned_bounce();
std::mutex& bounce_mutex();
void h2d_async(void* dst, const void* src, size_t bytes);
void h2d_sync_pinned(void* dst, const void* src, size_t bytes);

}
```

### polars_amd/csrc/engine.cpp

```cpp
#include "engine.hpp"

#include <algorithm>
#include <atomic>
#include <cmath>
#include <functional>
#include <memory>
#include <numeric>
#include <optional>
#include <set>
#include <sstream>

#include "cumulative.hpp"
#include "distinct.hpp"
#include "encoded_inputs.hpp"
#include "fused_shapes.hpp"
#include "jit.hpp"
#include "join.hpp"
#include "kernels.hpp"
#include "kernels_fused.hpp"
#include "ops.hpp"
#include "quantile.hpp"
#include "rolling.hpp"
#include "sort.hpp"
#include "temporal.hpp"
#include "variance.hpp"

namespace plx {
namespace engine {

using namespace fused;

struct Unsupported : std::exception {
  std::string why;
  explicit Unsupported(std::string w) : why(std::move(w)) {}
  const char* what() const noexcept override { return why.c_str(); }
};

Plan import_plan(const plx_ir* ir, int n_ir, const plx_aexpr* ae, int n_ae, uint32_t flags) {
  Plan p;
  p.flags = flags;
  PLX_REQUIRE(ir && n_ir > 0, PLX_ERR_INVALID, "execute_plan: empty IR arena");
  for (int i = 0; i < n_ae; i++) {
    AE e;
    e.kind = ae[i].kind; e.op = ae[i].op; e.lhs = ae[i].lhs; e.rhs = ae[i].rhs; e.dtype = ae[i].dtype; e.is_null = ae[i].is_null; e.lit = ae[i].lit;
    if (ae[i].name) e.name = ae[i].name;
    if (e.kind == PLX_AE_TERNARY) {
      e.cond = ae[i].cond;
      PLX_REQUIRE(e.cond >= 0 && e.lhs >= 0 && e.rhs >= 0, PLX_ERR_INVALID, "ternary expression needs a predicate (cond), a then (lhs) and an otherwise (rhs) input");
    }
    if (e.kind == PLX_AE_BITMAP_LOOKUP) {
      PLX_REQUIRE(e.lhs >= 0, PLX_ERR_INVALID, "bitmap lookup needs an integer input (lhs)");
      e.lut = get_column(ae[i].lit.u);
      PLX_REQUIRE(e.lut->dtype == PLX_BOOL, PLX_ERR_INVALID, "bitmap lookup: the lookup bitmap must be a Boolean column");
      PLX_REQUIRE(!e.lut->validity || e.lut->null_count == 0 || (e.lut->values && column_null_count(e.lut) == 0), PLX_ERR_INVALID, "bitmap lookup: the lookup bitmap must not hold nulls");
    }
    if (e.kind == PLX_AE_TEMPORAL) {
      PLX_REQUIRE(e.lhs >= 0, PLX_ERR_INVALID, "date part needs a Date / Datetime input (lhs)");
      PLX_REQUIRE(e.lit.u < (uint64_t)temporal::kNumUnits && temporal::part_ok(e.op, (int)e.lit.u), PLX_ERR_INVALID,
                  "date part: part " + std::to_string(e.op) + " of unit " + std::to_string((long long)e.lit.i) + " (plx_temporal_part_kind 0..9, plx_time_unit 0..3; the time of day and date() exist for a Datetime only)");
    }
    if (e.kind == PLX_AE_AGG && (e.op == PLX_AGG_VAR || e.op == PLX_AGG_STD))
      PLX_REQUIRE(e.lhs >= 0 && e.lit.u <= 255, PLX_ERR_INVALID, "var / std: the node carries ddof 0..255 in lit.u, got " + std::to_string((long long)e.lit.i));
    if (e.kind == PLX_AE_AGG && e.op == PLX_AGG_QUANTILE)
      PLX_REQUIRE(e.lhs >= 0 && quantile::q_ok(e.lit.f64) && quantile::interpolation_ok(e.dtype), PLX_ERR_INVALID,
                  "quantile: the node carries q in [0, 1] in lit.f64 and a plx_quantile_interpolation 0..4 in its dtype slot, got q=" + std::to_string(e.lit.f64) + ", interpolation=" + std::to_string(e.dtype));
    PLX_REQUIRE(e.lhs < i && e.rhs < i && e.cond < i, PLX_ERR_INVALID, "AExpr arena must be topologically ordered (children before parents)");
    if (e.kind == PLX_AE_WINDOW_KEY) {
      PLX_REQUIRE(e.lhs >= 0, PLX_ERR_INVALID, "window key link needs a key expression (lhs)");
      PLX_REQUIRE(e.rhs < 0 || ae[e.rhs].kind == PLX_AE_WINDOW_KEY, PLX_ERR_INVALID, "window key link: rhs must be the next link or -1");
    }
    if (e.kind == PLX_AE_WINDOW) {
      PLX_REQUIRE(e.lhs >= 0, PLX_ERR_INVALID, "window expression needs a function (lhs)");
      PLX_REQUIRE(e.rhs >= 0 && ae[e.rhs].kind == PLX_AE_WINDOW_KEY, PLX_ERR_INVALID, "window expression without a key: rhs must be the first PLX_AE_WINDOW_KEY link");
      int n_links = 0;
      for (int l = e.rhs; l >= 0; l = ae[l].rhs) n_links++;
      PLX_REQUIRE(n_links <= window::kMaxKeys, PLX_ERR_UNSUPPORTED, "window over " + std::to_string(n_links) + " keys; a window takes 1.." + std::to_string(window::kMaxKeys) + " keys on this path");
    }
    if (e.kind == PLX_AE_CUMULATIVE) {
      PLX_REQUIRE(e.lhs >= 0, PLX_ERR_INVALID, "cumulative expression needs an operand (lhs)");
      PLX_REQUIRE(cumulative::op_ok(e.op), PLX_ERR_INVALID, "cumulative expression: op " + std::to_string(e.op) + " is no plx_cum_op (0 = sum, 1 = min, 2 = max, 3 = count)");
      PLX_REQUIRE(e.lit.u <= 1, PLX_ERR_INVALID, "cumulative expression: reverse rides in lit.u as 0 / 1, got " + std::to_string((long long)e.lit.i));
    }
    if (e.kind == PLX_AE_RANK) {
      PLX_REQUIRE(e.lhs >= 0, PLX_ERR_INVALID, "rank expression needs an operand (lhs)");
      PLX_REQUIRE(cumulative::method_ok(e.op), PLX_ERR_INVALID, "rank expression: method " + std::to_string(e.op) + " is no plx_rank_method (0 = average, 1 = min, 2 = max, 3 = dense, 4 = ordinal)");
      PLX_REQUIRE(e.lit.u <= 1, PLX_ERR_INVALID, "rank expression: descending rides in lit.u as 0 / 1, got " + std::to_string((long long)e.lit.i));
    }
    if (e.kind == PLX_AE_SHIFT) {
      PLX_REQUIRE(e.lhs >= 0, PLX_ERR_INVALID, "shift / diff expression needs an operand (lhs)");
      PLX_REQUIRE(e.op == 0 || e.op == 1, PLX_ERR_INVALID, "shift / diff expression: op " + std::to_string(e.op) + " is neither 0 (shift) nor 1 (diff)");
      PLX_REQUIRE(e.rhs < 0 || (e.op == 0 && e.rhs < i && ae[e.rhs].kind == PLX_AE_LITERAL && !ae[e.rhs].is_null), PLX_ERR_INVALID,
                  "shift expression: fill_value (rhs) must be a non-null literal node or -1, and diff takes none");
    }
    if (e.kind == PLX_AE_ROLLING) {
      PLX_REQUIRE(e.lhs >= 0, PLX_ERR_INVALID, "rolling expression needs an operand (lhs)");
      PLX_REQUIRE(rolling::op_ok(e.op), PLX_ERR_INVALID, "rolling expression: op " + std::to_string(e.op) + " is no plx_rolling_op (0 = sum, 1 = mean, 2 = min, 3 = max)");
      const rolling::Params rp = rolling::unpack_params(e.lit.u);
      PLX_REQUIRE(rp.window >= 1 && rp.window <= 0x7fffffffull, PLX_ERR_INVALID, "rolling expression: window_size (lit.u bits 0..31) must be at least 1 and below 2^31, got " + std::to_string((long long)rp.window));
// ... 1160 lines not shown
    const int64_t step = (n + ((int64_t)1 << 20) - 1) >> 20;
    const bool dict_ok = (step <= 1 || enc::dict_collect(col->values->as<uint64_t>(), col->valid_words(), n, step, &pats)) &&
                         enc::dict_collect(col->values->as<uint64_t>(), col->valid_words(), n, 1, &pats);
    if (!dict_ok) return build_decimal_shadow(col, step);
    if (pats.empty()) return nullptr;
    s->kind = EncodedShadow::kDict; s->width = 1; s->n_dict = (int)pats.size();
    pats.resize(kDictSlots, 0);
    s->dict = dev_alloc(sizeof(uint64_t) * kDictSlots);
    s->codes = dev_alloc(groups);
    h2d_async(s->dict->ptr, pats.data(), sizeof(uint64_t) * kDictSlots);
    PLX_HIP(hipStreamSynchronize(stream()));
    if (!enc::dict_encode(col->values->as<uint64_t>(), col->valid_words(), n, s->dict->as<unsigned long long>(), s->n_dict, s->codes->as<uint8_t>())) return nullptr;
    return s;
  }
  int64_t mn, mx;
  if (col->range_state == 1 && col->range_trusted && !col->range_assumed) { mn = col->range_min; mx = col->range_max; }
  else {
    const k::ReduceResult rr = k::reduce_all(col->dtype, col->data(), col->valid_words(), n);
    if (rr.n_valid == 0) return nullptr;
    mn = (int64_t)rr.minmax_lo; mx = (int64_t)rr.minmax_hi;
  }
  uint64_t g = 0;
  if (enc::affine_needs_gcd(mn, mx)) {
    if (col->dtype != PLX_I64) return nullptr;
    g = enc::affine_gcd(col->values->as<int64_t>(), col->valid_words(), n, mn);
  }
  const enc::AffineChoice ch = enc::choose_affine(mn, mx, g);
  if (!ch.ok || ch.width * 4 > dtype_width(col->dtype)) return nullptr;
  s->kind = EncodedShadow::kAffine; s->width = ch.width; s->base = ch.base; s->stride = ch.stride;
  s->codes = dev_alloc(groups * (size_t)ch.width);
  if (!enc::affine_encode(col->dtype, col->data(), col->valid_words(), n, ch.base, ch.stride, ch.width, s->codes->ptr)) return nullptr;
  return s;
}
static std::shared_ptr<EncodedShadow> encoded_shadow_for_scan(const ColumnPtr& col, bool may_build) {
  if (!encoded_inputs_enabled()) return nullptr;
  std::shared_ptr<EncodedShadow> s = std::atomic_load(&col->shadow);
  if (s && s->kind != EncodedShadow::kNone) return s;
  if (!may_build || (s && s->never_encode) || !col->values || !col->values->owned || col->len <= 0) return nullptr;
  if (col->dtype != PLX_I64 && col->dtype != PLX_F64 && col->dtype != PLX_I32 && col->dtype != PLX_U32) return nullptr;
  auto next = std::make_shared<EncodedShadow>();
  next->scans = (s ? s->scans : 0) + 1;
  if (next->scans >= 2) {
    std::shared_ptr<EncodedShadow> built;
    try { built = build_shadow(col); }
    catch (const Error& e) { if (e.code != PLX_ERR_OOM) throw; (void)hipGetLastError(); }
    if (built) { built->scans = next->scans; next = built; }
    else next->never_encode = true;
  }
  std::atomic_store(&col->shadow, next);
  return next->kind != EncodedShadow::kNone ? next : nullptr;
}
struct ScanProgram { Shape shape; Args args; int static_id; std::string note; };
static ScanProgram scan_program_with_encodings(const Compiler& c, bool may_build) {
  ScanProgram sp{c.shape, c.args, -1, ""};
  enc::InputEncoding e[kMaxInputs];
  bool any = false;
  for (int i = 0; i < c.shape.n_inputs; i++) {
    const ColumnPtr& col = c.cols[c.input_cols[i]];
    if (c.args.in[i].values != col->data() || c.args.n_rows != col->len) continue;
    const std::shared_ptr<EncodedShadow> s = encoded_shadow_for_scan(col, may_build);
    if (!s) continue;
    e[i].kind = s->kind; e[i].width = s->width; e[i].base = s->base; e[i].stride = s->stride;
    e[i].codes = s->codes ? s->codes->ptr : nullptr; e[i].dict = s->dict ? s->dict->as<unsigned long long>() : nullptr;
    any = true;
  }
  uint32_t taken = 0;
  if (any && enc::encode_program(c.shape, c.args, e, &sp.shape, &sp.args, &taken)) {
    sp.note = "encoded{";
    bool first = true;
    for (int i = 0; i < c.shape.n_inputs; i++) {
      if (!((taken >> i) & 1u)) continue;
      std::string name = "?";
      for (size_t j = 0; j < c.df->cols.size(); j++) if (c.df->cols[j] == c.cols[c.input_cols[i]]) name = c.df->names[j];
      sp.note += std::string(first ? "" : ",") + name + ":" + (e[i].kind == EncodedShadow::kDict ? "dict" : e[i].kind == EncodedShadow::kDecimal ? "decimal" : "affine") + std::to_string(8 * e[i].width);
      first = false;
    }
    sp.note += "}";
  }
  sp.static_id = find_static_shape(sp.shape);
  return sp;
}

namespace {
struct GroupByRun {
  Compiler& c; const KeyPlan& kp; const Shape& sh; const Args& args;
  const int len_idx, static_id;
  const bool may_partition;
  FusedAggResult& res; std::string& desc;
};
std::string scan_tag(int static_id, int64_t n_rows) { return std::string("fused_scan[") + jit::program_mode(static_id, n_rows) + "]+"; }

void finish_table(GroupByRun& q, const Buf& cells, int64_t G, const Buf& oob) {
  compact_into(nullptr, cells->as<uint64_t>(), G, -1, q.sh.n_aggs, q.len_idx, q.res);
  check_oob_flag(oob);
  q.res.key_valid = nullptr;
}
bool input_value_bounds(const GroupByRun& q, int i, int64_t* lo, int64_t* hi) {
  if (i < 0 || i >= (int)q.c.input_cols.size() || q.args.in[i].validity) return false;
  const ColumnPtr& col = q.c.cols[q.c.input_cols[i]];
  const std::shared_ptr<EncodedShadow> s = std::atomic_load(&col->shadow);
  const bool codes = s && s->kind == EncodedShadow::kAffine && s->codes && q.args.in[i].values == s->codes->ptr;
  if (!codes && q.args.in[i].values != col->data()) {
    const char* p = (const char*)q.args.in[i].values; const char* b = (const char*)col->data();
    if (!b || p < b || p >= b + (size_t)col->len * dtype_width(col->dtype) || q.sh.in_dtype[i] != col->dtype) return false;
  }
  switch (q.sh.in_dtype[i]) {
    case PLX_U8: *lo = 0; *hi = 255; return true;
    case PLX_U16: *lo = 0; *hi = 65535; return true;
    case PLX_U32: *lo = 0; *hi = 0xffffffffll; return true;
    case PLX_I8: *lo = -128; *hi = 127; return true;
    case PLX_I16: *lo = -32768; *hi = 32767; return true;
    case PLX_I32: *lo = INT32_MIN; *hi = INT32_MAX; return true;
    case PLX_I64: case PLX_U64:
      if (codes || col->range_state != 1 || !col->range_trusted || col->range_assumed) return false;
      if (q.sh.in_dtype[i] == PLX_U64 && col->range_min < 0) return false;
      *lo = col->range_min; *hi = col->range_max; return true;
    default: return false;
  }
}
CellPlan shared_cells_plan(const GroupByRun& q) {
  AggFacts f{};
  f.n_rows = (uint64_t)q.args.n_rows; f.wg_rows = k::lds_agg_wg_rows(q.args.n_rows);
  for (int k = 0; k < q.sh.n_aggs; k++) {
    if (q.sh.aggs[k].kind != AGG_SUM_I) continue;
    const int in = affine_source_input(q.sh, q.sh.aggs[k].src);
    int64_t lo = 0, hi = 0;
    if (in < 0 || !input_value_bounds(q, in, &lo, &hi) || !affine_source_interval(q.sh, q.args, q.sh.aggs[k].src, &lo, &hi)) continue;
    f.known[k] = 1; f.lo[k] = lo; f.hi[k] = hi;
  }
  return plan_cells(q.sh, f);
}
void lds_table(GroupByRun& q) {
  const int G = 1 << q.kp.total_bits;
  Buf cells = dev_alloc(sizeof(uint64_t) * (size_t)G * q.sh.n_aggs);
  Buf oob = untrusted_key_bounds(q.c) ? dev_alloc_zero(8) : nullptr;
  const CellPlan cell_plan = shared_cells_plan(q);
  k::fused_lds_agg(q.sh, q.args, G, q.static_id, cells->as<uint64_t>(), oob ? oob->as<unsigned int>() : nullptr, &cell_plan);
  q.desc += scan_tag(q.static_id, q.args.n_rows) + "lds_table(G=" + std::to_string(G) + ",copies=" + std::to_string(k::lds_agg_copies(G, q.sh.n_aggs)) + ")";
  finish_table(q, cells, G, oob);
}
void dense_hbm_table(GroupByRun& q) {
  const int64_t G = (int64_t)1 << q.kp.total_bits;
  Buf cells = dev_alloc(sizeof(uint64_t) * (size_t)(G + 1) * q.sh.n_aggs);
  k::init_agg_cells(cells->as<uint64_t>(), G + 1, q.sh);
  Buf oob = untrusted_key_bounds(q.c) ? dev_alloc_zero(8) : nullptr;
  DenseTable t; t.acc = cells->as<unsigned long long>(); t.key_min = 0; t.n_groups = G; t.oob = oob ? oob->as<unsigned int>() : nullptr;
  k::fused_dense_agg(q.sh, q.args, t, q.static_id);
  q.desc += scan_tag(q.static_id, q.args.n_rows) + "dense_hbm_table(G=" + std::to_string(G) + ")";
  finish_table(q, cells, G, oob);
}

enum PartKeys { kPackedIds , kKeysWithValidity, kWideWords };
void take_partitioned(GroupByRun& q, PartKeys keys, int64_t g, const Buf& ok, const Buf& okv, const Buf& oacc, int64_t stride, const std::string& pd) {
  FusedAggResult& res = q.res;
  res.n_groups = g; res.n_aggs = q.sh.n_aggs; res.acc = oacc;
  if (keys == kWideWords) { res.wide_words = ok; res.wide_valid = okv; res.wide_stride = stride; }
  else { res.packed_keys = ok; res.key_valid = keys == kKeysWithValidity ? okv : nullptr; }
  q.desc += scan_tag(q.static_id, q.args.n_rows) + pd;
}
bool partitioned_v1(GroupByRun& q, double est_groups, bool any_nullable, PartKeys keys) {
  PartitionPlan pp;
  if (!k::partition_plan(q.sh, est_groups, any_nullable, &pp)) return false;
  std::string pd;
  Buf ok, okv, oacc;
  const int64_t g = k::partitioned_agg(q.sh, q.args, pp, q.static_id, &ok, &okv, &oacc, &pd);
  if (g < 0) { q.desc += "lds-overflow+"; return false; }
  take_partitioned(q, keys, g, ok, okv, oacc, 0, pd);
  return true;
}
struct PartTry {
  double plan_for = 0;
  double fallback = 0;
  int packed_bits = -1;
  std::vector<uint64_t> hot;
  k::SrcRange ranges[kMaxSrc];
  k::SrcRange key_rng;
  ColumnPtr stat_col;
  int attempts = 3;
  bool grow_to_largest = false;
  PartKeys keys = kPackedIds;
};
bool partitioned_v2(GroupByRun& q, PartTry& t) {
  for (int attempt = 0; attempt < t.attempts; attempt++) {
    PartPlan2 p2;
    auto plan = [&](double groups) { return k::partition_plan2(q.sh, groups, t.packed_bits, q.len_idx, q.args.n_rows, (int)t.hot.size(), &p2, t.ranges, &t.key_rng); };
    if (!plan(t.plan_for) && !(attempt == 0 && t.fallback > 0 && plan(t.fallback))) return false;
    std::string pd;
    Buf ok, okv, oacc;
    int64_t key_range[2] = {1, 0}, stride = 0;
    const int64_t g = k::partitioned_agg2(q.sh, q.args, p2, q.static_id, t.hot, &ok, &okv, &oacc, &pd, t.stat_col ? key_range : nullptr, &stride);
    if (g >= 0) {
      if (t.stat_col && key_range[0] <= key_range[1]) { t.stat_col->range_state = 1; t.stat_col->range_min = key_range[0]; t.stat_col->range_max = key_range[1]; t.stat_col->range_trusted = true; pd += "+key_range_learned"; }
      if (p2.check_src) mark_sources_verified(q.c);
      if (t.keys == kKeysWithValidity) q.desc += "hot=" + std::to_string(t.hot.size()) + "+";
      take_partitioned(q, t.keys, g, ok, okv, oacc, stride, pd);
      return true;
    }
    if (g == -2) { q.desc += "v2-unavailable+"; return false; }
    q.desc += t.attempts == 1 ? "lds-overflow+" : "lds-overflow(P=" + std::to_string(1u << p2.log2_parts) + ")+";
    if (p2.log2_parts >= 9) return false;
    t.plan_for = std::max(t.plan_for * 2.0, t.grow_to_largest ? (double)((uint64_t)p2.n_slots << 9) * 0.8 : (double)((uint64_t)p2.n_slots << p2.log2_parts) * 1.01);
  }
  return false;
}

bool partitioned_packed_ids(GroupByRun& q) {
  const int bits = q.kp.total_bits;
  const int64_t n = q.args.n_rows;
  const double est = std::min((double)((uint64_t)1 << std::min(bits, 40)), (double)n);
  if (part_version() != 2) return partitioned_v1(q, est, false, kPackedIds);
  PartTry t;
  t.plan_for = est; t.packed_bits = bits; t.attempts = 1;
  if (hot_keys_enabled() || bits > 25) {
    double g_est = 1e18;
    const int64_t d = sample_keys_cached(plain_key_column(q.c, q.kp), q.sh, q.args, q.static_id, q.len_idx, kPartSampleRows, hot_keys_enabled() ? &t.hot : nullptr, &g_est, q.desc);
    if (d >= 0) t.plan_for = std::min(est, std::min(g_est, (double)n) * 1.3);
    q.desc += "sample(distinct=" + std::to_string(d) + ",hot=" + std::to_string(t.hot.size()) + ")+";
  }
  const double hint = q.c.plan.group_hint;
  if (hint > 0) { t.plan_for = std::min(est, hint * 1.02 + 64.0); q.desc += "groups<=" + std::to_string((int64_t)hint) + "(plan)+"; }
  source_ranges(q.c, t.ranges);
  if (bits < 48 && !untrusted_key_bounds(q.c)) { t.key_rng.known = true; t.key_rng.mn = 0; t.key_rng.mx = (int64_t)(((uint64_t)1 << bits) - 1); }
  return partitioned_v2(q, t);
}

struct HashSizing { double groups = -1.0; std::vector<uint64_t> hot; int log2_cap = 0; };
HashSizing size_hash_table(GroupByRun& q) {
  const KeyPlan& kp = q.kp;
  const int64_t n = q.args.n_rows;
  HashSizing hs;
  const int64_t S = (int64_t)1 << 22;
  if (n <= 2 * S) { hs.log2_cap = std::max(10, ceil_log2_u64((uint64_t)n * 2)); return hs; }
  Args sa = q.args; sa.n_rows = S;
  FusedAggResult tmp;
  const bool strided = q.may_partition && !kp.wide && part_version() == 2;
  const int64_t Sd = strided || kp.wide ? kPartSampleRows : S;
  double g_est = -1.0;
  int64_t d = kp.wide ? run_wide_agg(q.sh, q.args, 21, kp.wide_nullable, tmp, true, kSampleBlocks, Sd)
                      : (strided ? sample_keys_cached(plain_key_column(q.c, kp), q.sh, q.args, q.static_id, q.len_idx, Sd, hot_keys_enabled() ? &hs.hot : nullptr, &g_est, q.desc)
                                 : run_hash_agg(q.sh, sa, q.static_id, 23, q.len_idx, tmp, true));
  double G = d < 0 ? 1e18 : (g_est >= 0.0 ? g_est : estimate_groups((double)d, (double)Sd));
  G = std::min(G, (double)n);
  const double hint = q.c.plan.group_hint;
  if (hint > 0) { G = std::min(hint, (double)n); q.desc += "groups<=" + std::to_string((int64_t)hint) + "(plan)+"; }
  hs.groups = G;
  hs.log2_cap = std::max(12, ceil_log2_u64((uint64_t)(G * 2.0) + 1));
  q.desc += "sample(distinct=" + std::to_string(d) + "/" + std::to_string(Sd) + ")+";
  return hs;
}
bool partitioned_wide_keys(GroupByRun& q, double G) {
  if (part_version() != 2) return false;
  PartTry t;
  source_ranges(q.c, t.ranges);
  t.plan_for = q.c.plan.group_hint > 0 ? G * 1.02 + 64.0 : G * 1.3;
  t.grow_to_largest = true; t.keys = kWideWords;
  return partitioned_v2(q, t);
}
bool partitioned_single_key(GroupByRun& q, double G, std::vector<uint64_t>& hot) {
  Compiler& c = q.c;
  if (part_version() != 2) {
    bool any_null = c.key >= 0 && c.nodes[c.key].nullable;
    for (auto& a : c.aggs) if (a.second >= 0 && c.nodes[a.second].nullable) any_null = true;
    return partitioned_v1(q, G * 1.3, any_null, kKeysWithValidity);
  }
  PartTry t;
  source_ranges(c, t.ranges);
  ColumnPtr key_col;
  const KeyPart* k0 = q.kp.parts.size() == 1 ? &q.kp.parts[0] : nullptr;
  if (k0 && dtype_is_int(k0->dtype) && k0->dtype != PLX_U64)
    if (const AE* x = plain_column(c.plan, k0->expr)) { const int ci = c.df->find(x->name); if (ci >= 0) key_col = c.df->cols[ci]; }
  if (key_col && q.sh.pred == kNone && key_col->range_state == 0 && key_col->len == q.args.n_rows) t.stat_col = key_col;
  if (key_col && key_col->range_state == 1 && key_col->range_trusted) { t.key_rng.known = true; t.key_rng.mn = key_col->range_min; t.key_rng.mx = key_col->range_max; }
  t.hot = std::move(hot);
  t.plan_for = c.plan.group_hint > 0 ? G * 1.02 + 64.0 : (!t.hot.empty() && G < 1e17) ? G * 4.0 : G * 1.3;
  if (!t.hot.empty()) t.fallback = G * 1.3;
  t.keys = kKeysWithValidity;
  return partitioned_v2(q, t);
}
void hash_hbm_table(GroupByRun& q, int log2_cap) {
  const KeyPlan& kp = q.kp;
  for (int attempt = 0; attempt < 8; attempt++) {
    int64_t g = kp.wide ? run_wide_agg(q.sh, q.args, log2_cap, kp.wide_nullable, q.res, false) : run_hash_agg(q.sh, q.args, q.static_id, log2_cap, q.len_idx, q.res, false);
    if (g >= 0) {
      q.desc += scan_tag(kp.wide ? -1 : q.static_id, q.args.n_rows) + (kp.wide ? "wide_hash_hbm_table(words=" + std::to_string(q.sh.n_keys + (kp.wide_nullable ? 1 : 0)) + ",cap=2^" : "hash_hbm_table(cap=2^") + std::to_string(log2_cap) + ")";
      return;
    }
    log2_cap += 2;
    q.desc += "grow+";
    PLX_REQUIRE(log2_cap <= 34, PLX_ERR_OOM, "group-by hash table would exceed 2^34 slots");
  }
  fail(PLX_ERR_OOM, "group-by hash table kept overflowing");
}
}

static bool lds_table_route(const KeyPlan& kp, const Shape& sh) { return kp.packed && kp.total_bits <= 12 && k::lds_agg_copies(1 << kp.total_bits, sh.n_aggs) > 0; }
static void run_fused_groupby(Compiler& c, const KeyPlan& kp, int len_idx, FusedAggResult& res, std::string& desc, std::string& encoded) {
  const Shape& sh = c.shape;
  const int64_t n = c.args.n_rows;
  res.n_aggs = sh.n_aggs;
  if (n == 0) { res.n_groups = 0; res.acc = dev_alloc(8); res.packed_keys = dev_alloc(8); return; }
  GroupByRun q{c, kp, sh, c.args, len_idx, find_static_shape(sh), !(c.plan.flags & PLX_PLAN_NO_PARTITION) && n >= ((int64_t)1 << 24), res, desc};
  if (lds_table_route(kp, sh)) {
    const ScanProgram sp = scan_program_with_encodings(c, true);
    if (sp.note.empty()) return lds_table(q);
    GroupByRun qe{c, kp, sp.shape, sp.args, len_idx, sp.static_id, q.may_partition, res, desc};
    lds_table(qe);
    encoded += sp.note + "; ";
    return;
  }
  if (kp.packed && kp.total_bits > 12 && q.may_partition && partitioned_packed_ids(q)) return;
  if (kp.packed && kp.total_bits <= 28 && ((size_t)sh.n_aggs << (kp.total_bits + 3)) <= (size_t(8) << 30)) return dense_hbm_table(q);
  HashSizing hs = size_hash_table(q);
  if (q.may_partition && hs.groups >= 4096.0 && (kp.wide ? partitioned_wide_keys(q, hs.groups) : partitioned_single_key(q, hs.groups, hs.hot))) return;
  hash_hbm_table(q, hs.log2_cap);
}

static ColumnPtr finalize_column(const FusedAggResult& r, const FinalSpec& fs, FinBatch& batch) {
  const int64_t G = r.n_groups;
  auto out = std::make_shared<Column>();
  out->dtype = fs.out_dtype; out->len = G;
  out->values = dev_alloc(values_bytes(fs.out_dtype, G));
  const bool nullable = fs.kind == FIN_MEAN || fs.kind == FIN_MINMAX_I || fs.kind == FIN_MINMAX_F || fs.kind == FIN_VAR || fs.kind == FIN_STD;
  if (nullable) out->validity = dev_alloc_zero(bitmap_bytes(G)); else out->null_count = 0;
  FinalSpec f = fs;
  if (fs.kind == FIN_COPY64 && dtype_width(fs.out_dtype) < 4) f.kind = FIN_NARROW;
  PLX_REQUIRE(batch.n < kMaxFinJobs, PLX_ERR_UNSUPPORTED, "too many output columns in one fused aggregation");
  FinJob& j = batch.jobs[batch.n++];
  j = FinJob{};
  j.is_key = 0; j.fs = f; j.out = out->values->ptr; j.out_valid = nullable ? out->validity->as<uint64_t>() : nullptr;
  return out;
}
static void append_aggregate_columns(const Plan& plan, const FusedAggResult& r, const std::vector<int>& agg_nodes, const std::vector<FinalSpec>& specs, const std::vector<int>& out_exprs, FinBatch& batch, Frame& frame) {
  std::map<int, ColumnPtr> overrides;
  for (size_t i = 0; i < agg_nodes.size(); i++) overrides[agg_nodes[i]] = finalize_column(r, specs[i], batch);
  k::finalize_batch(r.acc->as<uint64_t>(), r.n_aggs, r.n_groups, batch);
  Frame groups; groups.height = r.n_groups;
  for (int e : out_exprs) {
    Evaluated ev = eval(plan, e, groups, &overrides);
    frame.names.push_back(output_name(plan, e));
    frame.cols.push_back(broadcast(ev, r.n_groups));
  }
}

static ColumnPtr decode_key_column(const FusedAggResult& r, const KeyPart& part, int key_index, FinBatch& batch) {
  const int64_t G = r.n_groups;
  auto out = std::make_shared<Column>();
  out->dtype = part.dtype; out->len = G;
  out->values = part.dtype == PLX_BOOL ? dev_alloc_zero(bitmap_bytes(G)) : dev_alloc(values_bytes(part.dtype, G));
  if (part.nullable) out->validity = dev_alloc_zero(bitmap_bytes(G)); else out->null_count = 0;
  KeyDecode kd = part.dec;
  if (part.dtype == PLX_F32) kd.dtype = PLX_F32;
  PLX_REQUIRE(batch.n < kMaxFinJobs, PLX_ERR_UNSUPPORTED, "too many output columns in one fused aggregation");
  FinJob& j = batch.jobs[batch.n++];
  j = FinJob{};
  j.is_key = 1; j.kd = kd; j.out = out->values->ptr; j.out_valid = part.nullable ? out->validity->as<uint64_t>() : nullptr;
  if (r.wide_words) {
    j.packed = r.wide_words->as<unsigned long long>() + (size_t)key_index * r.wide_stride;
    j.kvalid = r.wide_valid->as<unsigned char>() + (size_t)key_index * r.wide_stride;
  } else {
    j.packed = r.packed_keys->as<unsigned long long>();
    j.kvalid = r.key_valid ? r.key_valid->as<unsigned char>() : nullptr;
  }
  return out;
}

static ColumnPtr first_row_permutation(const FusedAggResult& r, int first_idx) {
  const int64_t G = r.n_groups;
  std::vector<uint64_t> cells((size_t)G * r.n_aggs);
  d2h_sync(cells.data(), r.acc->ptr, cells.size() * 8);
  std::vector<uint32_t> perm((size_t)G);
  std::iota(perm.begin(), perm.end(), 0u);
  std::sort(perm.begin(), perm.end(), [&](uint32_t a, uint32_t b) { return cells[(size_t)a * r.n_aggs + first_idx] < cells[(size_t)b * r.n_aggs + first_idx]; });
  return column_from_host(PLX_U32, perm.data(), nullptr, 0, G);
}

struct ProgramDump {
  std::string json;
};
static thread_local ProgramDump* t_program_dump = nullptr;
static std::string jstr(const std::string& x) { std::string o = "\""; for (char ch : x) { if (ch == '"' || ch == '\\') o += '\\'; o += ch; } return o + "\""; }
static std::string program_fields(const Compiler& c, const Frame& frame, const Shape* sh_run = nullptr, const Args* args_run = nullptr) {
  std::ostringstream o;
  const Shape& sh = sh_run ? *sh_run : c.shape;
  const Args& args = args_run ? *args_run : c.args;
  o << "\"n_rows\":" << c.args.n_rows << ",\"inputs\":[";
  auto name_of = [&](int col_id) -> std::string {
    const ColumnPtr& buf = c.cols[col_id];
    for (size_t j = 0; j < frame.cols.size(); j++) if (frame.cols[j] == buf) return frame.names[j];
    return "?";
  };
  for (int i = 0; i < sh.n_inputs; i++)
    o << (i ? "," : "") << "{\"name\":" << jstr(name_of(c.input_cols[i])) << ",\"dtype\":" << (int)sh.in_dtype[i] << ",\"nullable\":" << (int)sh.in_nullable[i] << "}";
  o << "],\"ops\":[";
  for (int i = 0; i < sh.n_ops; i++)
    o << (i ? "," : "") << "[" << (int)sh.ops[i].code << "," << (int)sh.ops[i].dst << "," << (int)sh.ops[i].a << "," << (int)sh.ops[i].b << "," << (int)sh.ops[i].c << ",\"" << args.imm[i] << "\"]";
  o << "],\"pred\":" << (int)sh.pred << ",\"key\":" << (int)sh.key << ",\"keys\":[";
  for (int i = 0; i < sh.n_keys; i++) o << (i ? "," : "") << (int)sh.keys[i];
  o << "],\"aggs\":[";
  for (int i = 0; i < sh.n_aggs; i++) o << (i ? "," : "") << "[" << (int)sh.aggs[i].kind << "," << (int)sh.aggs[i].src << "]";
  o << "]";
  const ProgramSplit split = split_program(sh);
  o << ",\"early_mask\":" << split.early << ",\"any_late\":" << (split.any_late ? 1 : 0);
  return o.str();
}
static std::string finals_outputs_fields(const Plan& plan, const std::vector<int>& agg_nodes, const std::vector<FinalSpec>& specs, const std::vector<int>& out_exprs) {
  std::ostringstream o;
  o << "\"finals\":[";
  for (size_t i = 0; i < specs.size(); i++)
    o << (i ? "," : "") << "{\"kind\":" << (int)specs[i].kind << ",\"a\":" << (int)specs[i].a << ",\"b\":" << (int)specs[i].b << ",\"c\":" << (int)specs[i].c << ",\"out_dtype\":" << (int)specs[i].out_dtype << ",\"ddof\":" << (int)specs[i].ddof << "}";
  o << "],\"outputs\":[";
  for (size_t i = 0; i < out_exprs.size(); i++) {
    int e = out_exprs[i];
    while (plan.ae[e].kind == PLX_AE_ALIAS) e = plan.ae[e].lhs;
    int idx = -1;
    for (size_t j = 0; j < agg_nodes.size(); j++) if (agg_nodes[j] == e) idx = (int)j;
    o << (i ? "," : "") << "{\"name\":" << jstr(output_name(plan, out_exprs[i])) << ",\"final\":" << idx << "}";
  }
  o << "]";
  return o.str();
}
static std::string compiled_json(const char* kind, const Plan& plan, const Compiler& c, const ScanProgram& sp, const KeyPlan* kp, const std::vector<int>& agg_nodes,
                                 const std::vector<FinalSpec>& specs, const std::vector<int>& out_exprs, int len_idx, int first_idx, bool maintain_order) {
  std::ostringstream o;
  o << "{\"kind\":\"" << kind << "\"," << program_fields(c, *c.df, &sp.shape, &sp.args);
  if (!sp.note.empty()) o << ",\"encoded\":" << jstr(sp.note);
  o << ",\"len_idx\":" << len_idx << ",\"first_idx\":" << first_idx << ",\"maintain_order\":" << (maintain_order ? 1 : 0);
  if (kp) {
    o << ",\"key_plan\":{\"packed\":" << (kp->packed ? 1 : 0) << ",\"wide\":" << (kp->wide ? 1 : 0) << ",\"parts\":[";
    for (size_t i = 0; i < kp->parts.size(); i++) {
      const KeyPart& kpart = kp->parts[i];
      o << (i ? "," : "") << "{\"name\":" << jstr(output_name(plan, kpart.expr)) << ",\"dtype\":" << kpart.dtype << ",\"nullable\":" << (kpart.nullable ? 1 : 0) << ",\"shift\":" << kpart.dec.shift
        << ",\"mask\":\"" << kpart.dec.mask << "\",\"min\":\"" << kpart.dec.min << "\",\"null_code\":\"" << kpart.dec.null_code << "\"}";
    }
    o << "]}";
  }
  o << "," << finals_outputs_fields(plan, agg_nodes, specs, out_exprs) << "}";
  return o.str();
}
static void dump_compiled(ProgramDump* dump, const char* kind, const Plan& plan, const Compiler& c, const ScanProgram& sp, const KeyPlan* kp, const std::vector<int>& agg_nodes,
                          const std::vector<FinalSpec>& specs, const std::vector<int>& out_exprs, int len_idx, int first_idx, bool maintain_order) {
  if (dump) dump->json = compiled_json(kind, plan, c, sp, kp, agg_nodes, specs, out_exprs, len_idx, first_idx, maintain_order);
}
static int and_predicates(Compiler& c, const std::vector<int>& preds) {
  int p = -1;
  for (int pe : preds) { int n = c.lower(pe); if (c.nodes[n].ty != 'b') throw Unsupported("predicate is not boolean"); p = p < 0 ? n : c.mk(OP_AND, p, n, 'b'); }
  return p;
// ... 2 lines not shown
static bool fused_select(Plan& plan, const IRN& node, const std::vector<int>& preds, const FramePtr& src, FramePtr& out, Shape* shape_out, int* sid_out,
                         std::string* why, bool compile_only) {
  for (int e : node.exprs) if (contains_rowfn(plan, e)) { if (why) *why = rowfn_route_note(plan, e); return false; }
  for (int e : node.exprs) if (contains_window(plan, e)) { if (why) *why = "window expression: per-node route"; return false; }
  for (int e : node.exprs) if (!contains_agg(plan, e) || contains_column_outside_agg(plan, e)) { if (why) *why = "select mixes row expressions and aggregations"; return false; }
  {
    std::vector<int> lit_check;
    for (int e : node.exprs) collect_aggs(plan, e, lit_check);
    for (int a : lit_check)
      if (plan.ae[a].kind == PLX_AE_AGG && !contains_column(plan, plan.ae[a].lhs)) {
        if (why) *why = "aggregate of a literal is a scalar, not a value per row; done by the per-node kernels";
        return false;
      }
  }
  Compiler c(plan, *src);
  c.device_pivot = !compile_only;
  std::vector<int> agg_nodes;
  std::vector<FinalSpec> specs;
  try {
    for (int e : node.exprs) collect_aggs(plan, e, agg_nodes);
    c.decline_order_statistics(agg_nodes);
    c.pred = and_predicates(c, preds);
    for (int a : agg_nodes) specs.push_back(c.lower_agg(a));
    c.finish();
  } catch (const Unsupported& u) { if (why) *why = u.why; return false; }
  const ScanProgram sp = scan_program_with_encodings(c, !compile_only && src->height > 0);
  const int static_id = sp.static_id;
  if (shape_out) *shape_out = sp.shape;
  if (sid_out) *sid_out = static_id;
  if (compile_only) { dump_compiled(t_program_dump, "select", plan, c, sp, nullptr, agg_nodes, specs, node.exprs, -1, -1, false); return true; }
  FusedAggResult r; r.n_groups = 1; r.n_aggs = c.shape.n_aggs;
  std::vector<uint64_t> host(kMaxAggs, 0);
  if (src->height == 0) { for (int k2 = 0; k2 < c.shape.n_aggs; k2++) host[k2] = agg_identity(c.shape.aggs[k2].kind); }
  else k::fused_regagg(sp.shape, sp.args, static_id, host.data());
  r.acc = dev_alloc(sizeof(uint64_t) * kMaxAggs);
  h2d_async(r.acc->ptr, host.data(), sizeof(uint64_t) * (size_t)c.shape.n_aggs);
  PLX_HIP(hipStreamSynchronize(stream()));
  plan.desc += c.var_note + std::string("FusedFilterAgg{fused_scan[") + jit::program_mode(static_id, c.args.n_rows) + "]+register_sink, inputs=" + std::to_string(c.shape.n_inputs) + ", ops=" + std::to_string(c.shape.n_ops) + ", aggs=" + std::to_string(c.shape.n_aggs) + "}; ";
  if (!sp.note.empty()) plan.encoded += sp.note + "; ";
  out = std::make_shared<Frame>();
  out->height = 1;
  FinBatch batch{};
  append_aggregate_columns(plan, r, agg_nodes, specs, node.exprs, batch, *out);
  return true;
}

static bool forget_assumed_bounds(const std::vector<ColumnPtr>& cols) {
  bool guessed = false;
  for (auto& col : cols) if (col->range_assumed) { col->range_state = 0; col->range_trusted = true; col->range_assumed = false; col->range_verified = false; col->no_assume = true; std::atomic_store(&col->key_sample, std::shared_ptr<void>()); guessed = true; }
  return guessed;
}
static bool fused_groupby(Plan& plan, const IRN& node, const std::vector<int>& preds, const FramePtr& src, FramePtr& out, Shape* shape_out, int* sid_out,
                          std::string* why, bool compile_only) {
  for (int e : node.exprs) if (contains_rowfn(plan, e)) { if (why) *why = rowfn_route_note(plan, e); return false; }
  for (int e : node.exprs) if (contains_window(plan, e)) { if (why) *why = "window expression: per-node route"; return false; }
  for (int e : node.exprs) if (!contains_agg(plan, e) || contains_column_outside_agg(plan, e)) { if (why) *why = "group_by aggregation list contains a non-aggregated column"; return false; }
  Compiler c(plan, *src);
  c.device_pivot = !compile_only;
  std::vector<int> agg_nodes;
  std::vector<FinalSpec> specs;
  KeyPlan kp;
  int len_idx = -1, first_idx = -1;
  try {
    for (int e : node.exprs) collect_aggs(plan, e, agg_nodes);
    c.decline_order_statistics(agg_nodes);
    c.pred = and_predicates(c, preds);
    kp = lower_keys(c, node.keys);
    len_idx = c.add_agg(AGG_LEN, -1);
    for (int a : agg_nodes) specs.push_back(c.lower_agg(a));
    if (node.maintain_order) first_idx = c.add_agg(AGG_FIRST_ROW, -1);
    c.finish();
  } catch (const Unsupported& u) { if (why) *why = u.why; return false; }
  if (compile_only) {
    const ScanProgram sp = lds_table_route(kp, c.shape) ? scan_program_with_encodings(c, false) : ScanProgram{c.shape, c.args, find_static_shape(c.shape), ""};
    if (shape_out) *shape_out = sp.shape;
    if (sid_out) *sid_out = sp.static_id;
    dump_compiled(t_program_dump, "group_by", plan, c, sp, &kp, agg_nodes, specs, node.exprs, len_idx, first_idx, node.maintain_order != 0);
    return true;
  }
  if (shape_out) *shape_out = c.shape;
  if (sid_out) *sid_out = find_static_shape(c.shape);
  FusedAggResult r;
  std::string d;
  try {
    run_fused_groupby(c, kp, len_idx, r, d, plan.encoded);
  } catch (const Error& e) {
    if (!forget_assumed_bounds(c.cols) || e.code != PLX_ERR_INVALID) throw;
    plan.desc += "AssumedBoundsViolated{exact statistics, second run}; ";
    return fused_groupby(plan, node, preds, src, out, shape_out, sid_out, why, compile_only);
  }
  plan.desc += kp.note + c.var_note + "FusedFilterGroupBy{" + d + ", inputs=" + std::to_string(c.shape.n_inputs) + ", ops=" + std::to_string(c.shape.n_ops) + ", aggs=" + std::to_string(c.shape.n_aggs) + ", groups=" + std::to_string(r.n_groups) + "}; ";
  out = std::make_shared<Frame>();
  out->height = r.n_groups;
  FinBatch batch{};
  for (size_t pi = 0; pi < kp.parts.size(); pi++) { out->names.push_back(output_name(plan, kp.parts[pi].expr)); out->cols.push_back(decode_key_column(r, kp.parts[pi], (int)pi, batch)); }
  append_aggregate_columns(plan, r, agg_nodes, specs, node.exprs, batch, *out);
  if (node.maintain_order && r.n_groups > 1) {
    ColumnPtr perm = first_row_permutation(r, first_idx);
    for (auto& col : out->cols) col = ops::gather(col, perm);
  }
  return true;
}


static int peel_filters_node(const Plan& plan, int input) { while (plan.ir[input].kind == PLX_IR_FILTER) input = plan.ir[input].input; return input; }
static int peel_filters(const Plan& plan, int input, std::vector<int>& preds) {
  while (plan.ir[input].kind == PLX_IR_FILTER) { preds.push_back(plan.ir[input].predicate); input = plan.ir[input].input; }
  std::reverse(preds.begin(), preds.end());
  return input;
}

struct SemiFilter {
  FramePtr F;
  std::vector<int> fpreds;
  int fkey = -1;
  int pkey = -1;
};
static void collect_columns(const Plan& plan, int e, std::set<std::string>& out) {
  if (e < 0) return;
  const AE& x = plan.ae.at(e);
  if (x.kind == PLX_AE_COLUMN) { out.insert(x.name); return; }
  collect_columns(plan, x.lhs, out);
  collect_columns(plan, x.rhs, out);
  collect_columns(plan, x.cond, out);
}
static const char* join_takes_per_node_route(const IRN& jn) {
  if (jn.how == PLX_JOIN_FULL || jn.how == PLX_JOIN_RIGHT) return "full and right joins take the per-node route";
  if (jn.coalesce == 2) return "coalesce=false (both key columns kept) takes the per-node route";
  return nullptr;
}
static const char* single_key_join(const Plan& plan, const IRN& jn, bool semi_anti, const char* own, const AE*& lkx, const AE*& rkx) {
  if (const char* per_node = join_takes_per_node_route(jn)) return per_node;
  if (own) return own;
  const bool kind = semi_anti ? jn.how == PLX_JOIN_SEMI || jn.how == PLX_JOIN_ANTI : jn.how == PLX_JOIN_INNER || jn.how == PLX_JOIN_LEFT;
  if (!kind || jn.keys.size() != 1 || jn.keys_right.size() != 1) return semi_anti ? "not a single-key semi or anti join" : "not a single-key inner or left join";
  lkx = plain_column(plan, jn.keys[0]);
  rkx = plain_column(plan, jn.keys_right[0]);
  return lkx && rkx ? nullptr : "join keys are expressions";
}
static int resolve_join_side(const Plan& plan, int node, std::set<std::string> used, std::vector<int>& preds, std::vector<SemiFilter>& semis, std::string* why) {
  auto no = [&](const char* m) { if (why) *why = m; return -1; };
  const int n = peel_filters(plan, node, preds);
  if (plan.ir[n].kind == PLX_IR_SCAN) return n;
  if (plan.ir[n].kind != PLX_IR_JOIN) return no("join inputs are not filtered scans");
  const IRN& j = plan.ir[n];
  if (j.how != PLX_JOIN_INNER || j.keys.size() != 1 || j.keys_right.size() != 1) return no("nested join is not a single-key inner join");
  if (j.coalesce == 2) return no("nested join keeps both key columns (coalesce=false)");
  const AE* ka = plain_column(plan, j.keys[0]);
  const AE* kb = plain_column(plan, j.keys_right[0]);
  if (!ka || !kb) return no("nested join keys are expressions");
  std::vector<int> ap, bp;
  const int a = peel_filters(plan, j.input, ap), b = peel_filters(plan, j.input_right, bp);
  if (plan.ir[a].kind != PLX_IR_SCAN || plan.ir[b].kind != PLX_IR_SCAN) return no("nested join inputs are not filtered scans");
  FramePtr A = get_frame(plan.ir[a].frame), B = get_frame(plan.ir[b].frame);
  const int kai = A->find(ka->name), kbi = B->find(kb->name);
  if (kai < 0 || kbi < 0) return no("nested join key column not found");
  if (A->cols[kai]->dtype != B->cols[kbi]->dtype || !dtype_is_int(A->cols[kai]->dtype) || A->cols[kai]->dtype == PLX_U64) return no("nested join key is not a signed / narrow integer column pair of one dtype");
  for (size_t i = 0; i < B->names.size(); i++) if ((int)i != kbi && A->find(B->names[i]) >= 0) return no("nested join sides share a column name (suffix renaming is not modelled)");
  for (int pe : preds) collect_columns(plan, pe, used);
  bool used_a = false, used_b = false;
  for (auto& nm : A->names) used_a = used_a || used.count(nm);
  for (size_t i = 0; i < B->names.size(); i++) if ((int)i != kbi) used_b = used_b || used.count(B->names[i]);
  if (used.count(kb->name) && kb->name != ka->name) return no("the right key of the nested join is referenced above it (coalesced away)");
  SemiFilter sf;
  int payload = -1;
  if (!used_a) { sf.F = A; sf.fpreds = ap; sf.fkey = kai; sf.pkey = kbi; payload = b; preds.insert(preds.begin(), bp.begin(), bp.end()); }
  else if (!used_b) { sf.F = B; sf.fpreds = bp; sf.fkey = kbi; sf.pkey = kai; payload = a; preds.insert(preds.begin(), ap.begin(), ap.end()); }
  else return no("both sides of the nested join are referenced above it");
  semis.push_back(sf);
  return payload;
}
static bool semi_key_range(const SemiFilter& sf, int64_t* mn, int64_t* mx) {
  const ColumnPtr& c = sf.F->cols[sf.fkey];
  if (c->values) return ops::int_range(c, mn, mx);
  if (c->range_state == 1) { *mn = c->range_min; *mx = c->range_max; return true; }
  *mn = 0; *mx = 0;
// ... 1760 lines not shown
```

### polars_amd/csrc/engine.hpp

```cpp
#pragma once
#include <map>
#include <string>
#include <vector>

#include "core.hpp"
#include "fused.hpp"

namespace plx {
namespace engine {

struct AE {
  int kind = 0, op = 0, lhs = -1, rhs = -1, dtype = 0, is_null = 0;
  int cond = -1;
  plx_scalar lit{};
  std::string name;
  ColumnPtr lut;
};
struct IRN {
  int kind = 0, input = -1, input_right = -1, predicate = -1;
  plx_frame frame = 0;
  std::vector<int> exprs, keys, keys_right;
  int how = 0, maintain_order = 0;
  int coalesce = 0;
  std::string suffix = "_right";
  std::vector<uint8_t> sort_descending, sort_nulls_last;
  int64_t slice_offset = 0, slice_len = 0;
};
struct Plan {
  std::vector<IRN> ir;
  std::vector<AE> ae;
  uint32_t flags = 0;
  std::string desc;
  std::string encoded;
  std::map<int, FramePtr> memo;
  double group_hint = 0;
};

Plan import_plan(const plx_ir* ir, int n_ir, const plx_aexpr* ae, int n_ae, uint32_t flags);
FramePtr execute(Plan& plan, int root);

int infer_dtype(const Plan& plan, int e, const Frame& schema);
std::string output_name(const Plan& plan, int e);

struct AggParams { int ddof = 1; double q = 0.5; int interpolation = PLX_QUANTILE_LINEAR; };
void groupby_columns(const std::vector<ColumnPtr>& keys, const std::vector<ColumnPtr>& values, const std::vector<int>& aggs, bool maintain_order,
                     std::vector<ColumnPtr>& out_keys, std::vector<ColumnPtr>& out_aggs, std::string* desc, const std::vector<AggParams>* params = nullptr);

void window_columns(const std::vector<ColumnPtr>& keys, const std::vector<ColumnPtr>& values, const std::vector<int>& aggs, const std::vector<AggParams>* params,
                    std::vector<ColumnPtr>& out_cols, std::string* desc);

bool describe_fusion(Plan& plan, int root, fused::Shape* shape, int* static_id, std::string* why_not);
bool dump_program_json(Plan& plan, int root, std::string* json, std::string* why_not);
bool describe_join_fusion(Plan& plan, int root, std::vector<fused::Shape>* shapes, std::string* why_not);
bool describe_filter_fusion(Plan& plan, int root, fused::Shape* shape, std::string* why_not);
void encoded_set_decimal_min_rows(int64_t min_rows);
int64_t encoded_decimal_min_rows();

}
}
```

### polars_amd/csrc/kernels_fused.hip

```cpp
#include "fused_sinks.hpp"
#include "fused_cells.hpp"
#include "kernels.hpp"
#include "kernels_fused.hpp"
#include "variance.hpp"
#include "scan.hpp"
#include "jit.hpp"
#include <atomic>
#include <cstring>
#include <vector>

#ifdef PLX_HAVE_Q3_SHAPES
#define PLX_STATIC_JOIN_BUILD_CASES \
  case SHAPE_Q3_BUILD: hipLaunchKernelGGL((fused_scan_kernel<StatProg<SHAPE_Q3_BUILD>, JoinBuildSink>), dim3(grid), dim3(kBlock), 0, stream(), sh, args, t); break; \
  case SHAPE_Q3D_BUILD: hipLaunchKernelGGL((fused_scan_kernel<StatProg<SHAPE_Q3D_BUILD>, JoinBuildSink>), dim3(grid), dim3(kBlock), 0, stream(), sh, args, t); break;
#define PLX_STATIC_PROBE_AGG_CASES \
  case SHAPE_Q3_PROBE: hipLaunchKernelGGL((fused_scan_kernel<StatProg<SHAPE_Q3_PROBE>, ProbeAggSink>), dim3(grid), dim3(kBlock), 0, stream(), sh, args, t); break;
#define PLX_STATIC_REGAGG_EXTRA_CASES \
  case SHAPE_Q3_COUNT: launch_static<SHAPE_Q3_COUNT, RegAggSink>(wide, grid, 0, sh, args, sp); break;
#define PLX_STATIC_DIRECT_BUILD_CASES \
  case SHAPE_Q3_BUILD: hipLaunchKernelGGL((fused_scan_kernel<StatProg<SHAPE_Q3_BUILD>, DirectBuildSink>), dim3(grid), dim3(kBlock), 0, stream(), sh, args, t); break; \
  case SHAPE_Q3D_BUILD: hipLaunchKernelGGL((fused_scan_kernel<StatProg<SHAPE_Q3D_BUILD>, DirectBuildSink>), dim3(grid), dim3(kBlock), 0, stream(), sh, args, t); break;
#define PLX_STATIC_DIRECT_PROBE_CASES \
  case SHAPE_Q3_PROBE: hipLaunchKernelGGL((fused_scan_kernel<StatProg<SHAPE_Q3_PROBE>, DirectProbeAggSink>), dim3(grid), dim3(kBlock), 0, stream(), sh, args, t); break;
#ifdef PLX_HAVE_Q3FULL_SHAPES
#define PLX_STATIC_BITMAP_BUILD_CASES \
  case SHAPE_Q3F_SEMI: hipLaunchKernelGGL((fused_scan_kernel<StatProg<SHAPE_Q3F_SEMI>, BitmapBuildSink>), dim3(grid), dim3(kBlock), 0, stream(), sh, args, t); break;
#define PLX_STATIC_Q3F_JOIN_BUILD_CASES \
  case SHAPE_Q3F_BUILD: hipLaunchKernelGGL((fused_scan_kernel<StatProg<SHAPE_Q3F_BUILD>, JoinBuildSink>), dim3(grid), dim3(kBlock), 0, stream(), sh, args, t); break;
#define PLX_STATIC_Q3F_DIRECT_BUILD_CASES \
  case SHAPE_Q3F_BUILD: hipLaunchKernelGGL((fused_scan_kernel<StatProg<SHAPE_Q3F_BUILD>, DirectBuildSink>), dim3(grid), dim3(kBlock), 0, stream(), sh, args, t); break;
#define PLX_STATIC_Q3F_REGAGG_CASES \
  case SHAPE_Q3F_COUNT: launch_static<SHAPE_Q3F_COUNT, RegAggSink>(wide, grid, 0, sh, args, sp); break;
#else
#define PLX_STATIC_BITMAP_BUILD_CASES
#define PLX_STATIC_Q3F_JOIN_BUILD_CASES
#define PLX_STATIC_Q3F_DIRECT_BUILD_CASES
#define PLX_STATIC_Q3F_REGAGG_CASES
#endif
#else
#define PLX_STATIC_BITMAP_BUILD_CASES
#define PLX_STATIC_Q3F_JOIN_BUILD_CASES
#define PLX_STATIC_Q3F_DIRECT_BUILD_CASES
#define PLX_STATIC_Q3F_REGAGG_CASES
#define PLX_STATIC_DIRECT_BUILD_CASES
#define PLX_STATIC_DIRECT_PROBE_CASES
#define PLX_STATIC_JOIN_BUILD_CASES
#define PLX_STATIC_PROBE_AGG_CASES
#define PLX_STATIC_REGAGG_EXTRA_CASES
#endif

#include <cstdlib>

namespace plx {
namespace k {

static std::string scope_name(const char* aot, const char* other, int static_id) { return static_id >= 0 ? std::string(aot) + "#" + std::to_string(static_id) : std::string(other); }


using namespace dev;
using namespace fused;

__global__ __launch_bounds__(kBlock) void partials_finish_kernel(Shape sh, const unsigned long long* __restrict__ partials, int np, int cells,
                                                                 int cell_stride, unsigned long long* __restrict__ out) {
  __shared__ uint64_t red[kBlock / 64];
  const int cell = blockIdx.x;
  const uint8_t kind = sh.aggs[cell % sh.n_aggs].kind;
  uint64_t x = agg_identity_dev(kind);
  for (int i = threadIdx.x; i < np; i += blockDim.x) x = agg_combine(kind, x, partials[(size_t)i * cell_stride + cell]);
#pragma unroll
  for (int m = 32; m >= 1; m >>= 1) x = agg_combine(kind, x, shfl_xor_u64(x, m));
  if (lane_id() == 0) red[threadIdx.x >> 6] = x;
  __syncthreads();
  if (threadIdx.x == 0) {
    for (int w = 1; w < (int)(blockDim.x >> 6); w++) x = agg_combine(kind, x, red[w]);
    out[cell] = x;
  }
}

static int scan_grid(int64_t n_rows, int blocks_per_cu, const char* knob = nullptr, int tile_rows = kTileRows) {
  if (knob) { const char* e = getenv(knob); const int v = e ? atoi(e) : 0; if (v >= 1 && v <= 32) blocks_per_cu = v; }
  int64_t ntiles = (n_rows + tile_rows - 1) / tile_rows;
  return grid_for(ntiles, kBlock / 64, blocks_per_cu);
}
static_assert(!trust_nullable<StatProg<SHAPE_Q1>, LdsAggSink>() && !trust_nullable<StatProg<SHAPE_CFG2>, RegAggSink>() && !trust_nullable<StatProg<SHAPE_CFG2_NULLX>, RegAggSink>(),
// ... 702 lines not shown
      else reinterpret_cast<uint16_t*>(out)[g] = (uint16_t)cell[sp.a];
      break;
    case FIN_MEAN: {
      const uint64_t cnt = cell[sp.b];
      valid = cnt != 0;
      double m = valid ? as_f(cell[sp.a]) / (double)cnt : 0.0;
      if (sp.out_dtype == PLX_F32) reinterpret_cast<float*>(out)[g] = (float)m; else reinterpret_cast<double*>(out)[g] = m;
    } break;
    case FIN_MINMAX_I: {
      valid = cell[sp.b] != 0;
      const uint64_t v = valid ? cell[sp.a] : 0;
      switch (dtype_width_dev(sp.out_dtype)) {
        case 1: reinterpret_cast<uint8_t*>(out)[g] = (uint8_t)v; break;
        case 2: reinterpret_cast<uint16_t*>(out)[g] = (uint16_t)v; break;
        case 4: reinterpret_cast<uint32_t*>(out)[g] = (uint32_t)v; break;
        default: reinterpret_cast<uint64_t*>(out)[g] = v; break;
      }
    } break;
    case FIN_VAR: case FIN_STD: {
      const double n = (double)cell[sp.b];
      const double v = variance::finalize(n, variance::from_shifted(n, as_f(cell[sp.a]), as_f(cell[sp.c])), (int)sp.ddof, sp.kind == FIN_STD, &valid);
      if (sp.out_dtype == PLX_F32) reinterpret_cast<float*>(out)[g] = (float)v; else reinterpret_cast<double*>(out)[g] = v;
    } break;
    default: {
      valid = cell[sp.b] != 0;
      double v = valid ? as_f(cell[sp.a]) : 0.0;
      if (valid && cell[sp.c] == 0) v = __longlong_as_double(0x7ff8000000000000ll);
      reinterpret_cast<double*>(out)[g] = v;
    } break;
  }
  return valid;
}
__device__ __forceinline__ bool decode_one(const unsigned long long* packed, const unsigned char* kvalid, const KeyDecode& kd, void* out, int64_t g, bool& bit) {
  const uint64_t code = (packed[g] >> kd.shift) & kd.mask;
  const bool valid = (!kvalid || kvalid[g]) && (kd.mask == ~0ull || code != kd.null_code);
  const uint64_t v = valid ? code + (uint64_t)kd.min : 0;
  bit = valid && (v & 1);
  switch (kd.dtype) {
    case PLX_BOOL: break;
    case PLX_I8: case PLX_U8: reinterpret_cast<uint8_t*>(out)[g] = (uint8_t)v; break;
    case PLX_I16: case PLX_U16: reinterpret_cast<uint16_t*>(out)[g] = (uint16_t)v; break;
    case PLX_I32: case PLX_U32: reinterpret_cast<uint32_t*>(out)[g] = (uint32_t)v; break;
    case PLX_F32: { double d = as_f(v); reinterpret_cast<float*>(out)[g] = (float)d; } break;
    default: reinterpret_cast<uint64_t*>(out)[g] = v; break;
  }
  return valid;
}

__global__ __launch_bounds__(kBlock) void finalize_kernel(const unsigned long long* __restrict__ acc, int n_aggs, int64_t G, FinalSpec sp,
                                                          void* __restrict__ out, uint64_t* __restrict__ out_valid) {
  const int lane = lane_id();
  const int64_t nwords = (G + 63) >> 6;
  const int64_t wave = ((int64_t)blockIdx.x * blockDim.x + threadIdx.x) >> 6;
  const int64_t nwaves = ((int64_t)gridDim.x * blockDim.x) >> 6;
  for (int64_t w = wave; w < nwords; w += nwaves) {
    const int64_t g = w * 64 + lane;
    bool valid = false;
    if (g < G) valid = finalize_one(acc + (size_t)g * n_aggs, sp, out, g);
    if (out_valid) { uint64_t m = ballot(valid); if (lane == 0) out_valid[w] = m; }
  }
}

__global__ __launch_bounds__(kBlock) void finalize_batch_kernel(const unsigned long long* __restrict__ acc, int n_aggs, int64_t G, FinBatch b) {
  const int lane = lane_id();
  const int64_t nwords = (G + 63) >> 6;
  const int64_t wave = ((int64_t)blockIdx.x * blockDim.x + threadIdx.x) >> 6;
  const int64_t nwaves = ((int64_t)gridDim.x * blockDim.x) >> 6;
  for (int64_t w = wave; w < nwords; w += nwaves) {
    const int64_t g = w * 64 + lane;
    for (int j = 0; j < b.n; j++) {
      const FinJob& job = b.jobs[j];
      bool valid = false, bit = false;
      if (g < G) valid = job.is_key ? decode_one(job.packed, job.kvalid, job.kd, job.out, g, bit) : finalize_one(acc + (size_t)g * n_aggs, job.fs, job.out, g);
      if (job.is_key && job.kd.dtype == PLX_BOOL) { uint64_t bb = ballot(bit); if (lane == 0) reinterpret_cast<uint64_t*>(job.out)[w] = bb; }
      if (job.out_valid) { uint64_t m = ballot(valid); if (lane == 0) job.out_valid[w] = m; }
    }
  }
}
void finalize_batch(const uint64_t* acc, int n_aggs, int64_t G, const FinBatch& b) {
  if (G == 0 || b.n == 0) return;
  hipLaunchKernelGGL(finalize_batch_kernel, dim3(grid_for(G, kBlock)), dim3(kBlock), 0, stream(), (const unsigned long long*)acc, n_aggs, G, b);
  PLX_HIP(hipGetLastError());
}
void finalize_aggs(const uint64_t* acc, int n_aggs, int64_t G, const FinalSpec& sp, void* out, uint64_t* out_valid) {
  if (G == 0) return;
  hipLaunchKernelGGL(finalize_kernel, dim3(grid_for(G, kBlock)), dim3(kBlock), 0, stream(), (const unsigned long long*)acc, n_aggs, G, sp, out, out_valid);
  PLX_HIP(hipGetLastError());
}

__global__ __launch_bounds__(kBlock) void decode_key_kernel(const unsigned long long* __restrict__ packed, const unsigned char* __restrict__ kvalid, int64_t G,
                                                            KeyDecode kd, void* __restrict__ out, uint64_t* __restrict__ out_valid) {
  const int lane = lane_id();
  const int64_t nwords = (G + 63) >> 6;
  const int64_t wave = ((int64_t)blockIdx.x * blockDim.x + threadIdx.x) >> 6;
  const int64_t nwaves = ((int64_t)gridDim.x * blockDim.x) >> 6;
  for (int64_t w = wave; w < nwords; w += nwaves) {
    const int64_t g = w * 64 + lane;
    bool valid = false, bit = false;
    if (g < G) valid = decode_one(packed, kvalid, kd, out, g, bit);
    if (kd.dtype == PLX_BOOL) { uint64_t b = ballot(bit); if (lane == 0) reinterpret_cast<uint64_t*>(out)[w] = b; }
    if (out_valid) { uint64_t m = ballot(valid); if (lane == 0) out_valid[w] = m; }
  }
}
void decode_key(const uint64_t* packed, const uint8_t* kvalid, int64_t G, const KeyDecode& kd, void* out, uint64_t* out_valid) {
  if (G == 0) return;
  hipLaunchKernelGGL(decode_key_kernel, dim3(grid_for(G, kBlock)), dim3(kBlock), 0, stream(), (const unsigned long long*)packed, (const unsigned char*)kvalid, G, kd, out, out_valid);
  PLX_HIP(hipGetLastError());
}

int64_t table_compact(const uint64_t* keys, const uint64_t* acc, int64_t n_slots, int64_t cap, int n_aggs, int occ_agg, uint64_t* out_keys,
                      uint8_t* out_key_valid, uint64_t* out_acc) {
  Buf counter = dev_alloc_zero(8);
  ProfileScope ps("table_compact", (uint64_t)n_slots * 8 * (uint64_t)(1 + n_aggs), (uint64_t)n_slots);
  hipLaunchKernelGGL(hash_compact_kernel, dim3(compact_grid(n_slots)), dim3(kBlock), 0, stream(), (const unsigned long long*)keys,
                     (const unsigned long long*)acc, n_slots, cap, n_aggs, occ_agg, counter->as<unsigned long long>(), (unsigned long long*)out_keys,
                     (unsigned char*)out_key_valid, (unsigned long long*)out_acc);
  PLX_HIP(hipGetLastError());
  uint64_t n = 0;
  d2h_sync(&n, counter->ptr, 8);
  return (int64_t)n;
}

}

namespace fused {
int find_static_shape(const Shape& s) {
  for (int id = 0; id < kNumStaticShapes; id++) {
    Shape t = static_shape(id);
    if (memcmp(&t, &s, sizeof(Shape)) == 0) return id;
  }
  return -1;
}
}
}
```

### polars_amd/csrc/kernels_fused.hpp

```cpp
#pragma once
#include <string>
#include <vector>

#include "core.hpp"
#include "fused.hpp"
#include "fused_cells.hpp"

namespace plx {
namespace k {

void fused_regagg(const fused::Shape& sh, const fused::Args& args, int static_id, uint64_t* out_host);
int lds_agg_copies(int n_groups, int n_aggs);
void fused_lds_agg(const fused::Shape& sh, const fused::Args& args, int n_groups, int static_id, uint64_t* out_dev, unsigned int* oob = nullptr ,
                   const fused::CellPlan* cell_plan = nullptr );
uint64_t lds_agg_wg_rows(int64_t n_rows);
uint64_t lds_agg_wg_rows_of(int64_t n_rows, int grid, bool wide);
int last_lds_cells();
void set_shared_cells(bool on);

bool wide_tiles_choice(const fused::Shape& sh, const fused::Args& args, bool compiled, bool knob_on);
int last_scan_tile_rows();

void fused_dense_agg(const fused::Shape& sh, const fused::Args& args, const fused::DenseTable& t, int static_id);
void fused_hash_agg(const fused::Shape& sh, const fused::Args& args, const fused::HashTable& t, int static_id);
void fused_wide_agg(const fused::Shape& sh, const fused::Args& args, const fused::WideTable& t);
int64_t wide_compact(const fused::WideTable& t, int n_keys, int n_aggs, int64_t out_stride, uint64_t* out_words, uint8_t* out_kvalid, uint64_t* out_acc);
void fused_join_build(const fused::Shape& sh, const fused::Args& args, const fused::JoinAggTable& t, int static_id);
void fused_probe_agg(const fused::Shape& sh, const fused::Args& args, const fused::JoinAggTable& t, int static_id);
int64_t join_agg_compact(const fused::JoinAggTable& t, int n_aggs, int len_idx, uint64_t* out_keys, uint32_t* out_rows, uint64_t* out_acc);
void canonicalise_chains(const fused::JoinAggTable& t, const fused::RepCols& rc, unsigned int max_chain, unsigned int* flags);
int64_t rows_agg_compact(const uint64_t* acc, int64_t n_rows, int n_aggs, int len_idx, uint32_t* out_rows, uint64_t* out_acc);
int64_t chains_agg_compact(const fused::JoinAggTable& t, const fused::Shape& sh, const uint64_t* acc, int len_idx, Buf* out_rows, Buf* out_acc);
int64_t scan_waves(int64_t n_rows);
void fused_ballots(const fused::Shape& sh, const fused::Args& args, const fused::BallotOut& out, int static_id);
void fused_bitmap_build(const fused::Shape& sh, const fused::Args& args, const fused::BitmapBuild& t, int static_id);
void fused_direct_build(const fused::Shape& sh, const fused::Args& args, const fused::DirectJoinTable& t, int static_id);
void fused_direct_probe_agg(const fused::Shape& sh, const fused::Args& args, const fused::DirectJoinTable& t, int static_id);
void fused_direct_hits(const fused::Shape& sh, const fused::Args& args, const fused::DirectJoinTable& t, const fused::BallotOut& out, int static_id);
void direct_slot_rows(const fused::DirectJoinTable& t, int64_t n_used, uint32_t* slot_row);
uint64_t direct_rank(const fused::DirectJoinTable& t, uint32_t* rank_out, int64_t n_used, uint64_t* n_pairs_dev, uint64_t* pairs_out);
int64_t direct_agg_compact(const fused::DirectJoinTable& t, int64_t n_used, int n_aggs, int len_idx, uint64_t* out_keys, uint32_t* out_rows, uint64_t* out_acc);
void fill_u64(uint64_t* p, int64_t n, uint64_t v);
void init_agg_cells(uint64_t* acc, int64_t n_slots, const fused::Shape& sh);
int64_t table_compact(const uint64_t* keys, const uint64_t* acc, int64_t n_slots, int64_t cap, int n_aggs, int occ_agg, uint64_t* out_keys,
                      uint8_t* out_key_valid, uint64_t* out_acc);

void finalize_aggs(const uint64_t* acc, int n_aggs, int64_t G, const fused::FinalSpec& sp, void* out, uint64_t* out_valid);
bool partition_plan(const fused::Shape& sh, double est_groups, bool any_nullable, fused::PartitionPlan* out);
int64_t partitioned_agg(const fused::Shape& sh, const fused::Args& args, const fused::PartitionPlan& pp, int static_id, Buf* out_keys, Buf* out_kvalid,
                        Buf* out_acc, std::string* desc);
struct SrcRange { bool known = false; int64_t mn = 0, mx = 0; bool check = false;  };
bool partition_plan2(const fused::Shape& sh, double est_groups, int packed_bits, int len_idx, int64_t n_rows, int n_hot, fused::PartPlan2* out,
                     const SrcRange* src_ranges = nullptr , const SrcRange* key_range = nullptr );
void select_hot_keys(const fused::HashTable& t, int n_aggs, int len_idx, uint64_t threshold, std::vector<uint64_t>* out, uint64_t* hot_rows = nullptr);
int64_t partitioned_agg2(const fused::Shape& sh, const fused::Args& args, const fused::PartPlan2& pp, int static_id, const std::vector<uint64_t>& hot_keys, Buf* out_keys,
                         Buf* out_kvalid, Buf* out_acc, std::string* desc, int64_t* key_range_out = nullptr, int64_t* wide_stride_out = nullptr);
void touch_filter_set(const int64_t* keys, const uint64_t* validity, int64_t n, unsigned int log2_bits, uint64_t* filter);
bool partitioned_probe_hits(const fused::Shape& sh, const fused::Args& args, const fused::DirectJoinTable& dt, uint64_t n_build, int static_id, ColumnPtr* hits, std::string* desc);
bool partitioned_hash_probe_hits(const fused::Shape& sh, const fused::Args& args, const fused::JoinAggTable& ht, uint64_t n_build, int static_id, ColumnPtr* hits, std::string* desc);
struct JoinCells { Buf key, row; };
bool partitioned_join_build(const fused::Shape& sh, const fused::Args& args, int static_id, const fused::JoinAggTable& t, JoinCells* cells, std::string* desc);
int64_t cells_agg_compact(const JoinCells& cells, const uint64_t* acc, int64_t n_cells, int n_aggs, int len_idx, uint64_t* out_keys, uint32_t* out_rows, uint64_t* out_acc);
double sample_sortedness(const ColumnPtr& c);
bool sample_minmax(const ColumnPtr& c, int64_t* mn, int64_t* mx, int blocks = 64);
void finalize_batch(const uint64_t* acc, int n_aggs, int64_t G, const fused::FinBatch& b);
void decode_key(const uint64_t* packed, const uint8_t* kvalid, int64_t G, const fused::KeyDecode& kd, void* out, uint64_t* out_valid);

}
}
```

### polars_amd/csrc/kernels_join.hip

```cpp
#include "dev.hpp"
#include "fused.hpp"
#include "join.hpp"
#include "join_driver.hpp"
#include "join_keys.hpp"
#include "kernels.hpp"
#include "ops.hpp"
#include "scan.hpp"

namespace plx {
namespace join {

using namespace dev;
using k::kBlock;

struct Table {
  unsigned long long* keys;
  Chains ch;
};
struct SingleKey {
  using Keys = KeyCol;
  using Table = join::Table;
  static __device__ __forceinline__ bool hash_row(const KeyCol& kc, int64_t i, uint64_t* key) {
    if (!key_valid(kc, i)) return false;
    *key = load_key(kc, i);
// ... 14 lines not shown
      }
      slot = (slot + 1) & (cap - 1);
    }
  }
  static __device__ __forceinline__ int64_t find_or_claim(const Table& t, const KeyCol&, int64_t, uint64_t key) { return walk<true>(t, key); }
  static __device__ __forceinline__ int64_t find(const Table& t, const KeyCol&, int64_t, const KeyCol&, uint64_t key) { return walk<false>(t, key); }

  using HostKeys = ColumnPtr;
  static int64_t rows(const ColumnPtr& c) { return c->len; }
  static constexpr uint64_t kSlotsBeyondCap = 1;
  static constexpr bool kRefuseLargeOutputAlways = false;
  static constexpr const char* kPlanPrefix = "";
  static constexpr const char *kBuildScope = "join_build", *kCountScope = "join_probe_count", *kEmitScope = "join_probe_emit";
  static constexpr uint64_t kBuildSlotBytes = 0, kCountSlotBytes = 4, kEmitSlotBytes = 8;
  std::string plan_lead() const { return std::string(); }
  uint64_t key_bytes = 0;
  Buf keys;
  KeyCol probe, build;
  Table table;
  void prepare(const ColumnPtr& probe_key, const ColumnPtr& build_key, const Chains& ch) {
    const uint64_t slots = (1ull << ch.log2_cap) + kSlotsBeyondCap;
    keys = dev_alloc(sizeof(uint64_t) * slots);
    PLX_HIP(hipMemsetAsync(keys->ptr, 0xff, sizeof(uint64_t) * slots, stream()));
    table.keys = keys->as<unsigned long long>(); table.ch = ch;
    probe = key_col(probe_key); build = key_col(build_key);
    key_bytes = dtype_width(build_key->dtype) ? dtype_width(build_key->dtype) : 1;
  }
  void launch_build(int grid);
  void launch_count(int grid, int how, uint32_t* counts, uint8_t* matched);
  void launch_emit(int grid, int left_join, const uint64_t* offsets, uint32_t* out_probe, uint32_t* out_build);
};

__global__ __launch_bounds__(kBlock) void join_build_kernel(KeyCol build, Table t) { join_build_rows<SingleKey>(build, t); }
__global__ __launch_bounds__(kBlock) void join_count_kernel(KeyCol probe, Table t, int how, uint32_t* __restrict__ counts) { join_count_rows<SingleKey, false>(probe, probe, t, how, counts, nullptr); }
__global__ __launch_bounds__(kBlock) void join_full_count_kernel(KeyCol probe, Table t, uint32_t* __restrict__ counts, uint8_t* __restrict__ matched) {
  join_count_rows<SingleKey, true>(probe, probe, t, 1, counts, matched);
}
__global__ __launch_bounds__(kBlock) void join_emit_kernel(KeyCol probe, Table t, int left_join, const uint64_t* __restrict__ offsets, uint32_t* __restrict__ out_probe,
                                                           uint32_t* __restrict__ out_build) {
  join_emit_rows<SingleKey>(probe, probe, t, left_join, offsets, out_probe, out_build);
}
void SingleKey::launch_build(int grid) { hipLaunchKernelGGL(join_build_kernel, dim3(grid), dim3(kBlock), 0, stream(), build, table); }
void SingleKey::launch_count(int grid, int how, uint32_t* counts, uint8_t* matched) {
  if (matched) hipLaunchKernelGGL(join_full_count_kernel, dim3(grid), dim3(kBlock), 0, stream(), probe, table, counts, matched);
  else hipLaunchKernelGGL(join_count_kernel, dim3(grid), dim3(kBlock), 0, stream(), probe, table, how, counts);
}
void SingleKey::launch_emit(int grid, int left_join, const uint64_t* offsets, uint32_t* out_probe, uint32_t* out_build) {
  hipLaunchKernelGGL(join_emit_kernel, dim3(grid), dim3(kBlock), 0, stream(), probe, table, left_join, offsets, out_probe, out_build);
}

__global__ __launch_bounds__(kBlock) void join_unmatched_mask_kernel(const uint8_t* __restrict__ matched, int64_t n, unsigned long long* __restrict__ mask) {
  const int lane = lane_id();
  const int64_t nwords = (n + 63) >> 6;
  const int64_t wave = ((int64_t)blockIdx.x * blockDim.x + threadIdx.x) >> 6, nwaves = ((int64_t)gridDim.x * blockDim.x) >> 6;
  for (int64_t w = wave; w < nwords; w += nwaves) {
    const int64_t i = w * 64 + lane;
    const uint64_t m = ballot(i < n && matched[i] == 0);
    if (lane == 0) mask[w] = m;
  }
}
__global__ __launch_bounds__(kBlock) void join_append_unmatched_kernel(const uint32_t* __restrict__ rows, int64_t n, uint32_t* __restrict__ out_probe, uint32_t* __restrict__ out_build) {
  for (int64_t i = (int64_t)blockIdx.x * blockDim.x + threadIdx.x; i < n; i += (int64_t)gridDim.x * blockDim.x) { out_probe[i] = kNoRow; out_build[i] = rows[i]; }
}

__global__ __launch_bounds__(kBlock) void join_emit_kept_kernel(const uint32_t* __restrict__ counts, const uint64_t* __restrict__ offsets, int64_t n, uint32_t* __restrict__ out_probe) {
  for (int64_t i = (int64_t)blockIdx.x * blockDim.x + threadIdx.x; i < n; i += (int64_t)gridDim.x * blockDim.x)
    if (counts[i]) out_probe[offsets[i]] = (uint32_t)i;
}

void emit_kept_rows(const uint32_t* counts, const uint64_t* offsets, int64_t n, uint32_t* out_probe) {
  hipLaunchKernelGGL(join_emit_kept_kernel, dim3(k::grid_for(n, kBlock * 2)), dim3(kBlock), 0, stream(), counts, offsets, n, out_probe);
  PLX_HIP(hipGetLastError());
}

ColumnPtr make_idx_column(int64_t n, int64_t min_alloc_rows) {
  auto c = std::make_shared<Column>();
  c->dtype = PLX_U32; c->len = n; c->values = dev_alloc(values_bytes(PLX_U32, std::max(n, min_alloc_rows))); c->null_count = 0;
  return c;
}
void null_out_no_row(ColumnPtr& idx) {
  if (!idx->len) return;
  plx_scalar s; s.u = kNoRow;
  ColumnPtr ok = ops::cmp_scalar(PLX_NE, idx, s);
  idx->validity = ok->values; idx->null_count = -1;
  if (column_null_count(idx) == 0) { idx->validity = nullptr; idx->null_count = 0; }
}

Buf unmatched_build_rows(const uint8_t* matched, int64_t nb, int64_t* n_out) {
  *n_out = 0;
  if (nb == 0) return nullptr;
  const int64_t nwords = (nb + 63) >> 6;
  Buf mask = dev_alloc(sizeof(uint64_t) * (size_t)nwords);
  {
    ProfileScope ps("join_unmatched_mask", (uint64_t)nb + (uint64_t)nwords * 8, (uint64_t)nb);
    hipLaunchKernelGGL(join_unmatched_mask_kernel, dim3(k::grid_for(nb, kBlock * 4)), dim3(kBlock), 0, stream(), matched, nb, mask->as<unsigned long long>());
    PLX_HIP(hipGetLastError());
  }
  const k::FilterPlan fp = k::filter_prepare(mask->as<uint64_t>(), nb);
  *n_out = fp.n_out;
  Buf rows = dev_alloc(sizeof(uint32_t) * (size_t)std::max<int64_t>(fp.n_out, 1));
  k::filter_rowids(fp, rows->as<uint32_t>());
  PLX_HIP(hipStreamSynchronize(stream()));
  return rows;
}
void append_unmatched(const Buf& rows, int64_t n, int64_t at, const ColumnPtr& probe_idx, const ColumnPtr& build_idx) {
  if (n == 0) return;
  PLX_REQUIRE(at >= 0 && at + n <= probe_idx->len && probe_idx->len == build_idx->len, PLX_ERR_SHAPE, "full join: the unmatched build rows do not fit the pair list");
  ProfileScope ps("join_append_unmatched", (uint64_t)n * 12, (uint64_t)n);
  hipLaunchKernelGGL(join_append_unmatched_kernel, dim3(k::grid_for(n, kBlock * 4)), dim3(kBlock), 0, stream(), rows->as<uint32_t>(), n, probe_idx->values->as<uint32_t>() + at,
                     build_idx->values->as<uint32_t>() + at);
  PLX_HIP(hipGetLastError());
  PLX_HIP(hipStreamSynchronize(stream()));
}

template <class W>
__global__ __launch_bounds__(kBlock) void coalesce_key_kernel(const W* __restrict__ lkey, const uint64_t* __restrict__ lvalid, const W* __restrict__ rkey, const uint64_t* __restrict__ rvalid,
                                                              const uint32_t* __restrict__ li, const uint32_t* __restrict__ ri, int64_t n, W* __restrict__ out,
                                                              unsigned long long* __restrict__ out_validity) {
  const int lane = lane_id();
  const int64_t nwords = (n + 63) >> 6;
  const int64_t wave = ((int64_t)blockIdx.x * blockDim.x + threadIdx.x) >> 6, nwaves = ((int64_t)gridDim.x * blockDim.x) >> 6;
  for (int64_t w = wave; w < nwords; w += nwaves) {
    const int64_t i = w * 64 + lane;
    bool ok = false;
    if (i < n) {
      const uint32_t l = li[i];
      const bool from_left = l != kNoRow;
      const uint32_t j = from_left ? l : ri[i];
      ok = j != kNoRow;
      const W* src = from_left ? lkey : rkey;
      const uint64_t* val = from_left ? lvalid : rvalid;
      out[i] = ok ? src[j] : (W)0;
      if (ok && val) ok = (val[j >> 6] >> (j & 63)) & 1;
    }
    if (out_validity) { const uint64_t m = ballot(ok); if (lane == 0) out_validity[w] = m; }
  }
}
ColumnPtr coalesce_keys(const ColumnPtr& lkey, const ColumnPtr& rkey, const ColumnPtr& left_idx, const ColumnPtr& right_idx) {
  PLX_REQUIRE(lkey->dtype == rkey->dtype, PLX_ERR_INVALID, std::string("coalesced join key: the key columns have different dtypes (") + dtype_name(lkey->dtype) + ", " + dtype_name(rkey->dtype) + ")");
  const int w = lkey->dtype == PLX_BOOL ? 0 : dtype_width(lkey->dtype);
  PLX_REQUIRE(w == 1 || w == 2 || w == 4 || w == 8, PLX_ERR_UNSUPPORTED, std::string("full join with coalesce on a ") + dtype_name(lkey->dtype) + " key: keys of 1, 2, 4 or 8 bytes coalesce");
  PLX_REQUIRE(left_idx->dtype == PLX_U32 && right_idx->dtype == PLX_U32 && left_idx->len == right_idx->len, PLX_ERR_INVALID, "coalesced join key: two u32 index columns of one length");
  const int64_t n = left_idx->len;
  const bool need_valid = lkey->validity || rkey->validity;
  ColumnPtr out = make_column(lkey->dtype, n, need_valid);
  if (n == 0) return out;
  if (need_valid) out->null_count = -1;
  ProfileScope ps("join_coalesce_key", (uint64_t)n * (8 + 2 * (uint64_t)w), (uint64_t)n);
  const int grid = k::grid_for(n, kBlock * 2);
  unsigned long long* ov = need_valid ? out->validity->as<unsigned long long>() : nullptr;
#define C(W) hipLaunchKernelGGL((coalesce_key_kernel<W>), dim3(grid), dim3(kBlock), 0, stream(), (const W*)lkey->data(), lkey->valid_words(), (const W*)rkey->data(), rkey->valid_words(), \
                                left_idx->values->as<uint32_t>(), right_idx->values->as<uint32_t>(), n, (W*)out->values->ptr, ov)
  switch (w) {
    case 1: C(uint8_t); break;
    case 2: C(uint16_t); break;
    case 4: C(uint32_t); break;
    default: C(uint64_t); break;
  }
#undef C
  PLX_HIP(hipGetLastError());
  return out;
}

void join_indices(int how, const ColumnPtr& left_key, const ColumnPtr& right_key, ColumnPtr& left_idx, ColumnPtr& right_idx, std::string* desc, bool* dup_build_keys, int64_t* unmatched_build) {
  PLX_REQUIRE(left_key->dtype == right_key->dtype, PLX_ERR_INVALID,
              std::string("join keys have different dtypes (") + dtype_name(left_key->dtype) + ", " + dtype_name(right_key->dtype) + ")");
// ... 211 lines not shown
```

### polars_amd/csrc/ops.cpp

```cpp
#include "ops.hpp"
#include "variance.hpp"

#include <cmath>
#include <cstdlib>

#include "kernels.hpp"
#include "quantile.hpp"
#include "sort.hpp"
#include "temporal.hpp"

namespace plx {

int64_t column_null_count(const ColumnPtr& c) {
  if (!c->validity) return 0;
  if (c->null_count < 0) c->null_count = c->len - k::bitmap_popcount(c->valid_words(), c->len);
  return c->null_count;
}

namespace ops {

static void require_same_len(const ColumnPtr& a, const ColumnPtr& b, const char* what) {
  PLX_REQUIRE(a->len == b->len, PLX_ERR_SHAPE, std::string(what) + ": length mismatch " + std::to_string(a->len) + " vs " + std::to_string(b->len));
}
static void require_same_dtype(const ColumnPtr& a, const ColumnPtr& b, const char* what) {
// ... 261 lines not shown
      else r.v.u = rr.isum;
      return r;
    }
    case PLX_AGG_MEAN: {
      r.dtype = dt == PLX_F32 ? PLX_F32 : PLX_F64;
      if (n_valid == 0) { r.valid = false; return r; }
      double m = rr.fsum / (double)n_valid;
      if (dt == PLX_F32) r.v.f32 = (float)m; else r.v.f64 = m;
      return r;
    }
    case PLX_AGG_MIN: case PLX_AGG_MAX: {
      r.dtype = dt;
      if (n_valid == 0) { r.valid = false; return r; }
      uint64_t bits = op == PLX_AGG_MIN ? rr.minmax_lo : rr.minmax_hi;
      if (dtype_is_float(dt)) {
        double d; memcpy(&d, &bits, 8);
        if (rr.n_ordered == 0) d = std::nan("");
        if (dt == PLX_F32) r.v.f32 = (float)d; else r.v.f64 = d;
      } else r.v.u = bits;
      return r;
    }
    default: fail(PLX_ERR_INVALID, "reduce: bad aggregation");
  }
}

ScalarValue reduce_var(const ColumnPtr& c, int ddof, bool want_std) {
  PLX_REQUIRE(ddof >= 0 && ddof <= 255, PLX_ERR_INVALID, "var / std: ddof must be 0..255");
  if (!(dtype_is_int(c->dtype) || dtype_is_float(c->dtype))) fail(PLX_ERR_UNSUPPORTED, std::string("var / std of a ") + dtype_name(c->dtype) + " column: numeric columns only");
  ScalarValue r; r.v.u = 0; r.dtype = c->dtype == PLX_F32 ? PLX_F32 : PLX_F64;
  const variance::Moments m = k::reduce_var(c->dtype, c->data(), c->valid_words(), c->len);
  bool valid = false;
  const double v = variance::finalize(m.n, m.m2, ddof, want_std, &valid);
  r.valid = valid;
  if (valid) { if (r.dtype == PLX_F32) r.v.f32 = (float)v; else r.v.f64 = v; }
  return r;
}

ScalarValue reduce_quantile(const ColumnPtr& c, double q, int interpolation, std::string* desc) {
  PLX_REQUIRE(quantile::q_ok(q), PLX_ERR_INVALID, "quantile: q must be a real number in [0, 1], got " + std::to_string(q));
  PLX_REQUIRE(quantile::interpolation_ok(interpolation), PLX_ERR_INVALID, "quantile: interpolation " + std::to_string(interpolation) + " is no plx_quantile_interpolation (0..4)");
  if (!(dtype_is_int(c->dtype) || dtype_is_float(c->dtype))) fail(PLX_ERR_UNSUPPORTED, std::string("median / quantile of a ") + dtype_name(c->dtype) + " column: integer and float columns only");
  PLX_REQUIRE(c->values || c->len == 0, PLX_ERR_INVALID, "placeholder column has no data");
  ScalarValue r; r.v.u = 0; r.valid = false; r.dtype = c->dtype == PLX_F32 ? PLX_F32 : PLX_F64;
  const int64_t n_valid = c->len - column_null_count(c);
  if (n_valid <= 0) { if (desc) *desc = "quantile_select[rows=" + std::to_string(c->len) + ", valid=0]"; return r; }
  const quantile::Rank rk = quantile::rank_of((uint64_t)n_valid, q, interpolation);
  const sort::SelectedRanks sel = sort::select_ranks(c, n_valid, rk.lo, rk.hi, desc);
  const double v = quantile::combine(quantile::decode(c->dtype, sel.code_lo), quantile::decode(c->dtype, sel.code_hi), rk.frac, interpolation);
  r.valid = true;
  if (r.dtype == PLX_F32) r.v.f32 = (float)v; else r.v.f64 = v;
  return r;
}

ScalarValue reduce_n_unique(const ColumnPtr& c, std::string* desc) {
  const char* e = getenv("PLX_NUNIQUE_ROUTE");
  const bool force_sort = e && std::string(e) == "sort";
  ScalarValue r; r.v.u = 0; r.valid = true; r.dtype = PLX_U32;
  r.v.u = sort::n_unique_column(c, force_sort, desc);
  return r;
}

ColumnPtr full_column(int dtype, plx_scalar v, bool valid, int64_t len) {
  auto out = std::make_shared<Column>();
  out->dtype = dtype; out->len = len;
  if (dtype == PLX_BOOL) {
    out->values = dev_alloc_zero(bitmap_bytes(len));
    if (valid && (v.u & 1) && len) {
      PLX_HIP(hipMemsetAsync(out->values->ptr, 0xff, (size_t)((len + 7) / 8), stream()));
      k::bitmap_op(0, out->values->as<uint64_t>(), out->values->as<uint64_t>(), len, out->values->as<uint64_t>());
    }
  } else {
    out->values = dev_alloc(values_bytes(dtype, len));
    k::fill(dtype_width(dtype), out->values->ptr, valid ? v.u : 0, len);
  }
  if (!valid) { out->validity = all_null_validity(len); out->null_count = len; } else out->null_count = 0;
  return out;
}
ColumnPtr scalar_column(const ScalarValue& s) { return full_column(s.dtype, s.v, s.valid, 1); }

ColumnPtr fill_null(const ColumnPtr& c, plx_scalar v) {
  if (!c->validity || column_null_count(c) == 0) {
    if (!c->validity) return c;
    auto same = std::make_shared<Column>(*c);
    same->validity = nullptr; same->null_count = 0;
    return same;
  }
  auto out = std::make_shared<Column>();
  out->dtype = c->dtype; out->len = c->len; out->null_count = 0;
  const int w = dtype_width(c->dtype);
  out->values = w ? dev_alloc(values_bytes(c->dtype, c->len)) : dev_alloc_zero(bitmap_bytes(c->len));
  k::fill_null(w, c->values->ptr, c->validity->as<uint64_t>(), v.u, c->len, out->values->ptr);
  if (c->range_state == 1) out->range_state = 0;
  return out;
}

plx_scalar scalar_of(const ColumnPtr& c, bool* valid) {
  plx_scalar s; s.u = 0;
  uint8_t v = 0xff; int32_t hv = 0;
  uint64_t buf[2] = {0, 0};
  column_to_host(c, buf, &v, &hv);
  *valid = v & 1;
  if (c->dtype == PLX_BOOL) s.u = buf[0] & 1; else memcpy(&s, buf, (size_t)dtype_width(c->dtype));
  return s;
}

ColumnPtr bitmap_lookup(const ColumnPtr& codes, const ColumnPtr& lut) {
  PLX_REQUIRE(dtype_is_int(codes->dtype), PLX_ERR_INVALID, std::string("bitmap lookup: codes must be an integer column, not ") + dtype_name(codes->dtype));
  PLX_REQUIRE(lut->dtype == PLX_BOOL, PLX_ERR_INVALID, "bitmap lookup: the lookup bitmap must be a Boolean column");
  PLX_REQUIRE(!lut->validity || column_null_count(lut) == 0, PLX_ERR_INVALID, "bitmap lookup: the lookup bitmap must not hold nulls");
  PLX_REQUIRE((codes->values || codes->len == 0) && (lut->values || lut->len == 0), PLX_ERR_INVALID, "placeholder column has no data");
  auto out = std::make_shared<Column>();
  out->dtype = PLX_BOOL; out->len = codes->len;
  out->values = dev_alloc(bitmap_bytes(codes->len));
  k::bitmap_lookup(codes->dtype, codes->data(), codes->valid_words(), codes->len, lut->values ? lut->values->as<uint64_t>() : nullptr, (uint64_t)lut->len, out->values->as<uint64_t>());
  out->validity = codes->validity; out->null_count = codes->null_count;
  return out;
}

int temporal_part_dtype(int part) { return temporal::part_width(part) == 4 ? PLX_I32 : temporal::part_width(part) == 2 ? PLX_I16 : PLX_I8; }
ColumnPtr temporal_part(const ColumnPtr& c, int part, int unit) {
  PLX_REQUIRE(temporal::unit_ok(unit) && part >= 0 && part < temporal::kNumParts, PLX_ERR_INVALID, "temporal part: part " + std::to_string(part) + " / unit " + std::to_string(unit) + " out of range");
  PLX_REQUIRE(c->dtype == (unit == temporal::kUnitDate ? PLX_I32 : PLX_I64), PLX_ERR_INVALID,
              std::string("temporal part: a Date is an Int32 column and a Datetime an Int64 column, got ") + dtype_name(c->dtype) + " with unit " + std::to_string(unit));
  PLX_REQUIRE(temporal::part_ok(part, unit), PLX_ERR_INVALID, "temporal part: the time of day and date() exist for a Datetime only");
  PLX_REQUIRE(c->values || c->len == 0, PLX_ERR_INVALID, "placeholder column has no data");
  auto out = std::make_shared<Column>();
  out->dtype = temporal_part_dtype(part); out->len = c->len;
  out->values = dev_alloc(values_bytes(out->dtype, c->len));
  k::temporal_part(unit, part, c->data(), c->len, out->values->ptr);
  out->validity = c->validity; out->null_count = c->null_count;
  return out;
}

ColumnPtr if_then_else(const ColumnPtr& mask, const ColumnPtr& a, const ColumnPtr& b) {
  PLX_REQUIRE(mask->dtype == PLX_BOOL, PLX_ERR_INVALID, "if_then_else: the mask must be Boolean");
  require_same_dtype(a, b, "if_then_else");
  int64_t len = 1;
  for (const ColumnPtr* c : {&mask, &a, &b}) if ((*c)->len != 1) len = (*c)->len;
  for (const ColumnPtr* c : {&mask, &a, &b})
    PLX_REQUIRE((*c)->len == len || (*c)->len == 1, PLX_ERR_SHAPE, "if_then_else: length mismatch " + std::to_string((*c)->len) + " vs " + std::to_string(len) + " (only a length-1 operand broadcasts)");
  ColumnPtr m = mask;
  if (m->len != len) { bool v; const plx_scalar s = scalar_of(m, &v); m = full_column(PLX_BOOL, s, v, len); }
  struct Side { const void* values = nullptr; const uint64_t* validity = nullptr; plx_scalar s{}; bool s_valid = true; bool nullable = false; };
  auto side_of = [&](const ColumnPtr& c) {
    Side sd;
    if (c->len != len) { sd.s = scalar_of(c, &sd.s_valid); sd.nullable = !sd.s_valid; }
    else { sd.values = c->values ? c->values->ptr : nullptr; sd.nullable = c->validity && c->null_count != 0; sd.validity = sd.nullable ? c->valid_words() : nullptr; }
    return sd;
  };
  const Side sa = side_of(a), sb = side_of(b);
  auto out = std::make_shared<Column>();
  out->dtype = a->dtype; out->len = len;
  const int w = dtype_width(a->dtype);
  out->values = w ? dev_alloc(values_bytes(a->dtype, len)) : dev_alloc_zero(bitmap_bytes(len));
  if (sa.nullable || sb.nullable) { out->validity = dev_alloc_zero(bitmap_bytes(len)); out->null_count = -1; } else out->null_count = 0;
  if (len) k::select(w, m->values->as<uint64_t>(), m->valid_words(), sa.values, sa.validity, sa.s, sa.s_valid, sb.values, sb.validity, sb.s, sb.s_valid, len,
                     out->values->ptr, out->validity ? out->validity->as<uint64_t>() : nullptr);
  return out;
}

ColumnPtr concat(const std::vector<ColumnPtr>& chunks) {
  PLX_REQUIRE(!chunks.empty(), PLX_ERR_INVALID, "concat: no chunks");
  if (chunks.size() == 1) return chunks[0];
  int64_t total = 0; bool any_valid = false;
  for (auto& c : chunks) { require_same_dtype(chunks[0], c, "concat"); total += c->len; any_valid |= (bool)c->validity; }
  auto out = std::make_shared<Column>();
  out->dtype = chunks[0]->dtype; out->len = total;
// ... 45 lines not shown
```

Measured before the change: 442.6 billion rows/s.

## Fuse group-by compaction, finalize and download into one tail kernel with host mirror

For small LDS-table group-bys, a single-workgroup kernel compacts occupied slots, decodes keys, finalizes aggregates, and writes both device columns and a packed result block. One pinned copy then brings the block to the host, and it is attached to the columns as a host mirror. Later frame_to_host calls serve from that mirror instead of issuing per-column device-to-host copies, which removes launches and syncs on the Q1 tail. It adds mirror-invalidation points wherever a column is mutated, and the risk is a stale mirror if one is missed. The path is on by default and can be turned off with PLX_GROUPBY_TAIL=0.

After: 451.4 billion rows/s (median of 6 runs). +2.0%, better.

```diff
diff --git a/include/polars_amd.h b/include/polars_amd.h
--- a/include/polars_amd.h
+++ b/include/polars_amd.h
@@ -332,6 +332,9 @@
 int32_t plx_last_scan_tile_rows(void);
 int32_t plx_last_lds_cells(void);
 void plx_set_shared_cells(int32_t on);
+void plx_set_groupby_tail(int32_t on);
+int32_t plx_last_groupby_tail(void);
+int32_t plx_last_download_mirrored(void);
 int32_t plx_cell_plan(int32_t static_shape_id, int32_t n_inputs, const int32_t* dtypes, const int32_t* nullable, int32_t n_ops, const uint8_t* ops, int32_t n_aggs, const uint8_t* aggs,
                       const uint8_t* known, const int64_t* lo, const int64_t* hi, uint64_t wg_rows, uint64_t n_rows, int32_t* out);
 uint64_t plx_lds_wg_rows(int64_t n_rows, int32_t grid, int32_t wide);
diff --git a/polars_amd/_ffi.py b/polars_amd/_ffi.py
--- a/polars_amd/_ffi.py
+++ b/polars_amd/_ffi.py
@@ -259,6 +259,9 @@
     "plx_last_scan_tile_rows": (C.c_int32, []),
     "plx_last_lds_cells": (C.c_int32, []),
     "plx_set_shared_cells": (None, [C.c_int32]),
+    "plx_set_groupby_tail": (None, [C.c_int32]),
+    "plx_last_groupby_tail": (C.c_int32, []),
+    "plx_last_download_mirrored": (C.c_int32, []),
     "plx_cell_plan": (C.c_int32, [C.c_int32, C.c_int32, C.POINTER(C.c_int32), C.POINTER(C.c_int32), C.c_int32, C.POINTER(C.c_uint8), C.c_int32, C.POINTER(C.c_uint8),
                                   C.POINTER(C.c_uint8), C.POINTER(C.c_int64), C.POINTER(C.c_int64), C.c_uint64, C.c_uint64, C.POINTER(C.c_int32)]),
     "plx_lds_wg_rows": (C.c_uint64, [C.c_int64, C.c_int32, C.c_int32]),
@@ -340,6 +343,18 @@
     lib().plx_set_shared_cells(int(bool(on)))
 
 
+def set_groupby_tail(on: bool) -> None:
+    lib().plx_set_groupby_tail(int(bool(on)))
+
+
+def last_groupby_tail() -> int:
+    return int(lib().plx_last_groupby_tail())
+
+
+def last_download_mirrored() -> int:
+    return int(lib().plx_last_download_mirrored())
+
+
 def cell_plan(facts, wg_rows, n_rows, static_shape_id=-1, dtypes=(), nullable=(), ops=(), aggs=()):
     n_aggs = len(facts)
     ni, no = len(dtypes), len(ops)
diff --git a/polars_amd/csrc/abi.cpp b/polars_amd/csrc/abi.cpp
--- a/polars_amd/csrc/abi.cpp
+++ b/polars_amd/csrc/abi.cpp
@@ -649,6 +649,24 @@
 int plx_frame_to_host(plx_frame f, void* const* values_out, uint8_t* const* validity_out, int32_t* has_validity_out) {
   PLX_TRY
   FramePtr fr = get_frame(f);
+  {
+    bool any = false, all = true;
+    for (size_t i = 0; i < fr->cols.size(); i++) {
+      if (!((values_out && values_out[i]) || (validity_out && validity_out[i]))) continue;
+      any = true;
+      if (!fr->cols[i]->host) { all = false; break; }
+    }
+    set_last_download_mirrored(any && all ? 1 : 0);
+    if (any && all) {
+      for (size_t i = 0; i < fr->cols.size(); i++) {
+        const Column& c = *fr->cols[i];
+        if ((values_out && values_out[i]) || (validity_out && validity_out[i]))
+          column_to_host_mirrored(c, values_out ? values_out[i] : nullptr, validity_out ? validity_out[i] : nullptr, nullptr);
+        if (has_validity_out) has_validity_out[i] = c.validity ? 1 : 0;
+      }
+      return PLX_OK;
+    }
+  }
   {
     struct Piece { const void* src; void* dst; size_t bytes; };
     std::vector<Piece> pieces;
@@ -1351,6 +1369,9 @@
 int32_t plx_last_scan_tile_rows(void) { return k::last_scan_tile_rows(); }
 int32_t plx_last_lds_cells(void) { return k::last_lds_cells(); }
 void plx_set_shared_cells(int32_t on) { k::set_shared_cells(on != 0); }
+void plx_set_groupby_tail(int32_t on) { k::set_groupby_tail(on != 0); }
+int32_t plx_last_groupby_tail(void) { return engine::last_groupby_tail(); }
+int32_t plx_last_download_mirrored(void) { return last_download_mirrored(); }
 uint64_t plx_lds_wg_rows(int64_t n_rows, int32_t grid, int32_t wide) { return (n_rows < 0 || grid < 1) ? 0 : k::lds_agg_wg_rows_of(n_rows, grid, wide != 0); }
 int32_t plx_cell_plan(int32_t static_shape_id, int32_t n_inputs, const int32_t* dtypes, const int32_t* nullable, int32_t n_ops, const uint8_t* ops, int32_t n_aggs, const uint8_t* aggs,
                       const uint8_t* known, const int64_t* lo, const int64_t* hi, uint64_t wg_rows, uint64_t n_rows, int32_t* out) {
@@ -1620,6 +1641,7 @@
     PLX_HIP(hipMemcpyAsync(copy->ptr, v->values->ptr, v->values->bytes, hipMemcpyDeviceToDevice, stream()));
     v->values = copy;
   }
+  drop_host_mirror(*v);
   k::strview_stamp_nulls(v->values->as<uint64_t>(), eff->values->as<uint64_t>(), m->len);
   PLX_HIP(hipStreamSynchronize(stream()));
   PLX_CATCH
diff --git a/polars_amd/csrc/comm.cpp b/polars_amd/csrc/comm.cpp
--- a/polars_amd/csrc/comm.cpp
+++ b/polars_amd/csrc/comm.cpp
@@ -96,7 +96,7 @@
   if (col->dtype == PLX_BOOL) out.push_back({bitmap_as_bytes(col->values, col->len), 1});
   else {
     auto v = std::make_shared<Column>(*col);
-    v->validity = nullptr;
+    v->validity = nullptr; v->host.reset();
     out.push_back({v, (size_t)dtype_width(col->dtype)});
   }
   if (with_validity) {
diff --git a/polars_amd/csrc/core.cpp b/polars_amd/csrc/core.cpp
--- a/polars_amd/csrc/core.cpp
+++ b/polars_amd/csrc/core.cpp
@@ -252,7 +252,24 @@
   return c;
 }
 
+static thread_local int t_last_download_mirrored = 0;
+int last_download_mirrored() { return t_last_download_mirrored; }
+void set_last_download_mirrored(int v) { t_last_download_mirrored = v; }
+void column_to_host_mirrored(const Column& c, void* values_out, uint8_t* validity_out, int32_t* has_validity) {
+  const HostMirror& m = *c.host;
+  const size_t vb = c.dtype == PLX_BOOL ? (size_t)((c.len + 7) / 8) : (size_t)c.len * dtype_width(c.dtype);
+  const size_t nb = (size_t)((c.len + 7) / 8);
+  PLX_REQUIRE(vb <= m.values_bytes && (!c.validity || nb <= m.valid_bytes), PLX_ERR_INVALID, "host mirror shorter than its column");
+  if (values_out && vb) memcpy(values_out, m.values(), vb);
+  if (validity_out && nb) {
+    if (c.validity) memcpy(validity_out, m.valid(), nb);
+    else memset(validity_out, 0xff, nb);
+  }
+  if (has_validity) *has_validity = c.validity ? 1 : 0;
+}
 void column_to_host(const ColumnPtr& c, void* values_out, uint8_t* validity_out, int32_t* has_validity) {
+  if (c->host) { column_to_host_mirrored(*c, values_out, validity_out, has_validity); t_last_download_mirrored = 1; return; }
+  t_last_download_mirrored = 0;
   size_t vb = c->dtype == PLX_BOOL ? (size_t)((c->len + 7) / 8) : (size_t)c->len * dtype_width(c->dtype);
   if (values_out && vb) PLX_HIP(hipMemcpyAsync(values_out, c->values->ptr, vb, hipMemcpyDeviceToHost, stream()));
   size_t nb = (size_t)((c->len + 7) / 8);
diff --git a/polars_amd/csrc/core.hpp b/polars_amd/csrc/core.hpp
--- a/polars_amd/csrc/core.hpp
+++ b/polars_amd/csrc/core.hpp
@@ -94,6 +94,13 @@
   int scans = 0;
   bool never_encode = false;
 };
+struct HostMirror {
+  std::shared_ptr<const std::vector<uint8_t>> bytes;
+  size_t values_off = 0, values_bytes = 0;
+  size_t valid_off = 0, valid_bytes = 0;
+  const uint8_t* values() const { return bytes->data() + values_off; }
+  const uint8_t* valid() const { return valid_bytes ? bytes->data() + valid_off : nullptr; }
+};
 struct Column {
   int dtype = PLX_I64;
   int64_t len = 0;
@@ -110,6 +117,7 @@
   int order_state = 0;
   std::shared_ptr<EncodedShadow> shadow;
   bool repeats_as_build_key = false;
+  std::shared_ptr<const HostMirror> host;
   const void* data() const { return values ? values->ptr : nullptr; }
   const uint64_t* valid_words() const { return validity ? validity->as<uint64_t>() : nullptr; }
 };
@@ -130,6 +138,10 @@
 ColumnPtr column_from_host(int dtype, const void* values, const uint8_t* validity, int64_t bit_offset, int64_t len);
 int64_t column_null_count(const ColumnPtr& c);
 void column_to_host(const ColumnPtr& c, void* values_out, uint8_t* validity_out, int32_t* has_validity);
+void column_to_host_mirrored(const Column& c, void* values_out, uint8_t* validity_out, int32_t* has_validity);
+int last_download_mirrored();
+void set_last_download_mirrored(int v);
+inline void drop_host_mirror(Column& c) { c.host.reset(); }
 
 plx_column register_column(ColumnPtr c);
 ColumnPtr get_column(plx_column h);
diff --git a/polars_amd/csrc/engine.cpp b/polars_amd/csrc/engine.cpp
--- a/polars_amd/csrc/engine.cpp
+++ b/polars_amd/csrc/engine.cpp
@@ -14,6 +14,7 @@
 #include "distinct.hpp"
 #include "encoded_inputs.hpp"
 #include "fused_shapes.hpp"
+#include "groupby_tail.hpp"
 #include "jit.hpp"
 #include "join.hpp"
 #include "kernels.hpp"
@@ -1340,12 +1341,19 @@
 }
 
 namespace {
+struct TailRequest {
+  const std::vector<FinalSpec>& specs;
+  std::vector<ColumnPtr> key_cols, agg_cols;
+  bool taken = false;
+};
 struct GroupByRun {
   Compiler& c; const KeyPlan& kp; const Shape& sh; const Args& args;
   const int len_idx, static_id;
   const bool may_partition;
   FusedAggResult& res; std::string& desc;
+  TailRequest* tail = nullptr;
 };
+bool groupby_tail_finish(GroupByRun& q, const Buf& cells, int G, const Buf& oob);
 std::string scan_tag(int static_id, int64_t n_rows) { return std::string("fused_scan[") + jit::program_mode(static_id, n_rows) + "]+"; }
 
 void finish_table(GroupByRun& q, const Buf& cells, int64_t G, const Buf& oob) {
@@ -1395,6 +1403,7 @@
   const CellPlan cell_plan = shared_cells_plan(q);
   k::fused_lds_agg(q.sh, q.args, G, q.static_id, cells->as<uint64_t>(), oob ? oob->as<unsigned int>() : nullptr, &cell_plan);
   q.desc += scan_tag(q.static_id, q.args.n_rows) + "lds_table(G=" + std::to_string(G) + ",copies=" + std::to_string(k::lds_agg_copies(G, q.sh.n_aggs)) + ")";
+  if (q.tail && groupby_tail_finish(q, cells, G, oob)) return;
   finish_table(q, cells, G, oob);
 }
 void dense_hbm_table(GroupByRun& q) {
@@ -1552,16 +1561,16 @@
 }
 
 static bool lds_table_route(const KeyPlan& kp, const Shape& sh) { return kp.packed && kp.total_bits <= 12 && k::lds_agg_copies(1 << kp.total_bits, sh.n_aggs) > 0; }
-static void run_fused_groupby(Compiler& c, const KeyPlan& kp, int len_idx, FusedAggResult& res, std::string& desc, std::string& encoded) {
+static void run_fused_groupby(Compiler& c, const KeyPlan& kp, int len_idx, FusedAggResult& res, std::string& desc, std::string& encoded, TailRequest* tail = nullptr) {
   const Shape& sh = c.shape;
   const int64_t n = c.args.n_rows;
   res.n_aggs = sh.n_aggs;
   if (n == 0) { res.n_groups = 0; res.acc = dev_alloc(8); res.packed_keys = dev_alloc(8); return; }
-  GroupByRun q{c, kp, sh, c.args, len_idx, find_static_shape(sh), !(c.plan.flags & PLX_PLAN_NO_PARTITION) && n >= ((int64_t)1 << 24), res, desc};
+  GroupByRun q{c, kp, sh, c.args, len_idx, find_static_shape(sh), !(c.plan.flags & PLX_PLAN_NO_PARTITION) && n >= ((int64_t)1 << 24), res, desc, tail};
   if (lds_table_route(kp, sh)) {
     const ScanProgram sp = scan_program_with_encodings(c, true);
     if (sp.note.empty()) return lds_table(q);
-    GroupByRun qe{c, kp, sp.shape, sp.args, len_idx, sp.static_id, q.may_partition, res, desc};
+    GroupByRun qe{c, kp, sp.shape, sp.args, len_idx, sp.static_id, q.may_partition, res, desc, tail};
     lds_table(qe);
     encoded += sp.note + "; ";
     return;
@@ -1573,31 +1582,39 @@
   hash_hbm_table(q, hs.log2_cap);
 }
 
+static bool final_nullable(const FinalSpec& fs) { return fs.kind == FIN_MEAN || fs.kind == FIN_MINMAX_I || fs.kind == FIN_MINMAX_F || fs.kind == FIN_VAR || fs.kind == FIN_STD; }
+static FinalSpec final_job_spec(const FinalSpec& fs) {
+  FinalSpec f = fs;
+  if (fs.kind == FIN_COPY64 && dtype_width(fs.out_dtype) < 4) f.kind = FIN_NARROW;
+  return f;
+}
 static ColumnPtr finalize_column(const FusedAggResult& r, const FinalSpec& fs, FinBatch& batch) {
   const int64_t G = r.n_groups;
   auto out = std::make_shared<Column>();
   out->dtype = fs.out_dtype; out->len = G;
   out->values = dev_alloc(values_bytes(fs.out_dtype, G));
-  const bool nullable = fs.kind == FIN_MEAN || fs.kind == FIN_MINMAX_I || fs.kind == FIN_MINMAX_F || fs.kind == FIN_VAR || fs.kind == FIN_STD;
+  const bool nullable = final_nullable(fs);
   if (nullable) out->validity = dev_alloc_zero(bitmap_bytes(G)); else out->null_count = 0;
-  FinalSpec f = fs;
-  if (fs.kind == FIN_COPY64 && dtype_width(fs.out_dtype) < 4) f.kind = FIN_NARROW;
+  const FinalSpec f = final_job_spec(fs);
   PLX_REQUIRE(batch.n < kMaxFinJobs, PLX_ERR_UNSUPPORTED, "too many output columns in one fused aggregation");
   FinJob& j = batch.jobs[batch.n++];
   j = FinJob{};
   j.is_key = 0; j.fs = f; j.out = out->values->ptr; j.out_valid = nullable ? out->validity->as<uint64_t>() : nullptr;
   return out;
 }
+static void append_output_expressions(const Plan& plan, const std::map<int, ColumnPtr>& overrides, const std::vector<int>& out_exprs, int64_t n_groups, Frame& frame) {
+  Frame groups; groups.height = n_groups;
+  for (int e : out_exprs) {
+    Evaluated ev = eval(plan, e, groups, &overrides);
+    frame.names.push_back(output_name(plan, e));
+    frame.cols.push_back(broadcast(ev, n_groups));
+  }
+}
 static void append_aggregate_columns(const Plan& plan, const FusedAggResult& r, const std::vector<int>& agg_nodes, const std::vector<FinalSpec>& specs, const std::vector<int>& out_exprs, FinBatch& batch, Frame& frame) {
   std::map<int, ColumnPtr> overrides;
   for (size_t i = 0; i < agg_nodes.size(); i++) overrides[agg_nodes[i]] = finalize_column(r, specs[i], batch);
   k::finalize_batch(r.acc->as<uint64_t>(), r.n_aggs, r.n_groups, batch);
-  Frame groups; groups.height = r.n_groups;
-  for (int e : out_exprs) {
-    Evaluated ev = eval(plan, e, groups, &overrides);
-    frame.names.push_back(output_name(plan, e));
-    frame.cols.push_back(broadcast(ev, r.n_groups));
-  }
+  append_output_expressions(plan, overrides, out_exprs, r.n_groups, frame);
 }
 
 static ColumnPtr decode_key_column(const FusedAggResult& r, const KeyPart& part, int key_index, FinBatch& batch) {
@@ -1620,6 +1637,78 @@
     j.kvalid = r.key_valid ? r.key_valid->as<unsigned char>() : nullptr;
   }
   return out;
+}
+
+static thread_local int t_last_groupby_tail = 0;
+int last_groupby_tail() { return t_last_groupby_tail; }
+namespace {
+ColumnPtr tail_column(int dtype, bool nullable, int64_t rows, FinJob& j) {
+  auto out = std::make_shared<Column>();
+  out->dtype = dtype; out->len = rows;
+  out->values = dev_alloc(values_bytes(dtype, rows));
+  if (nullable) out->validity = dev_alloc(bitmap_bytes(rows)); else out->null_count = 0;
+  j = FinJob{};
+  j.out = out->values->ptr; j.out_valid = nullable ? out->validity->as<uint64_t>() : nullptr;
+  return out;
+}
+bool groupby_tail_finish(GroupByRun& q, const Buf& cells, int G, const Buf& oob) {
+  TailRequest& t = *q.tail;
+  const size_t n_cols = q.kp.parts.size() + t.specs.size();
+  if (!k::groupby_tail_knob() || n_cols == 0 || n_cols > (size_t)kMaxFinJobs || G > gbt::kTailMaxSlots || !pinned_bounce()) return false;
+  int32_t dtypes[kMaxFinJobs]; uint8_t nullable[kMaxFinJobs];
+  int n = 0;
+  for (const KeyPart& part : q.kp.parts) { dtypes[n] = part.dtype; nullable[n++] = part.nullable ? 1 : 0; }
+  for (const FinalSpec& fs : t.specs) { dtypes[n] = fs.out_dtype; nullable[n++] = final_nullable(fs) ? 1 : 0; }
+  gbt::TailLayout L;
+  gbt::tail_layout(&L, G, dtypes, nullable, n);
+  if (!gbt::tail_block_fits(L, kBounceBytes)) return false;
+  FinBatch batch{};
+  std::vector<ColumnPtr> cols;
+  for (const KeyPart& part : q.kp.parts) {
+    FinJob& j = batch.jobs[batch.n++];
+    cols.push_back(tail_column(part.dtype, part.nullable, G, j));
+    j.is_key = 1; j.kd = part.dec;
+    if (part.dtype == PLX_F32) j.kd.dtype = PLX_F32;
+  }
+  for (const FinalSpec& fs : t.specs) {
+    FinJob& j = batch.jobs[batch.n++];
+    cols.push_back(tail_column(fs.out_dtype, final_nullable(fs), G, j));
+    j.is_key = 0; j.fs = final_job_spec(fs);
+  }
+  Buf block = dev_alloc(L.total);
+  k::groupby_tail(cells->as<uint64_t>(), q.sh.n_aggs, G, q.len_idx, oob ? oob->as<unsigned int>() : nullptr, batch, block->ptr);
+  auto bytes = std::make_shared<std::vector<uint8_t>>(L.total);
+  {
+    std::lock_guard<std::mutex> lk(bounce_mutex());
+    PLX_HIP(hipMemcpyAsync(pinned_bounce(), block->ptr, L.total, hipMemcpyDeviceToHost, stream()));
+    PLX_HIP(hipStreamSynchronize(stream()));
+    memcpy(bytes->data(), pinned_bounce(), L.total);
+  }
+  gbt::TailHeader h;
+  memcpy(&h, bytes->data(), sizeof h);
+  PLX_REQUIRE(h.version == gbt::kTailLayoutVersion && h.n_groups <= (uint32_t)G, PLX_ERR_INVALID, "group-by tail: the result block has no valid header");
+  if (h.oob) fail(PLX_ERR_INVALID, "group key outside the bounds declared or assumed for its column");
+  const int64_t g = h.n_groups;
+  for (int j = 0; j < n; j++) {
+    Column& c = *cols[j];
+    c.len = g;
+    auto m = std::make_shared<HostMirror>();
+    m->bytes = bytes; m->values_off = L.values_off[j]; m->values_bytes = L.values_bytes[j];
+    if (c.validity) {
+      m->valid_off = L.valid_off[j]; m->valid_bytes = (size_t)L.words * 8;
+      int64_t valid = 0;
+      for (uint32_t w = 0; w < L.words; w++) { uint64_t x; memcpy(&x, bytes->data() + m->valid_off + (size_t)w * 8, 8); valid += (int64_t)gbt::tail_popc64(x); }
+      c.null_count = g - valid;
+    }
+    c.host = std::move(m);
+  }
+  q.res.n_groups = g; q.res.n_aggs = q.sh.n_aggs; q.res.acc = cells;
+  t.key_cols.assign(cols.begin(), cols.begin() + (ptrdiff_t)q.kp.parts.size());
+  t.agg_cols.assign(cols.begin() + (ptrdiff_t)q.kp.parts.size(), cols.end());
+  t.taken = true;
+  t_last_groupby_tail = 1;
+  return true;
+}
 }
 
 static ColumnPtr first_row_permutation(const FusedAggResult& r, int first_idx) {
@@ -1788,8 +1877,10 @@
   if (sid_out) *sid_out = find_static_shape(c.shape);
   FusedAggResult r;
   std::string d;
+  TailRequest tail{specs};
+  t_last_groupby_tail = 0;
   try {
-    run_fused_groupby(c, kp, len_idx, r, d, plan.encoded);
+    run_fused_groupby(c, kp, len_idx, r, d, plan.encoded, node.maintain_order ? nullptr : &tail);
   } catch (const Error& e) {
     if (!forget_assumed_bounds(c.cols) || e.code != PLX_ERR_INVALID) throw;
     plan.desc += "AssumedBoundsViolated{exact statistics, second run}; ";
@@ -1798,6 +1889,13 @@
   plan.desc += kp.note + c.var_note + "FusedFilterGroupBy{" + d + ", inputs=" + std::to_string(c.shape.n_inputs) + ", ops=" + std::to_string(c.shape.n_ops) + ", aggs=" + std::to_string(c.shape.n_aggs) + ", groups=" + std::to_string(r.n_groups) + "}; ";
   out = std::make_shared<Frame>();
   out->height = r.n_groups;
+  if (tail.taken) {
+    for (size_t pi = 0; pi < kp.parts.size(); pi++) { out->names.push_back(output_name(plan, kp.parts[pi].expr)); out->cols.push_back(tail.key_cols[pi]); }
+    std::map<int, ColumnPtr> overrides;
+    for (size_t i = 0; i < agg_nodes.size(); i++) overrides[agg_nodes[i]] = tail.agg_cols[i];
+    append_output_expressions(plan, overrides, node.exprs, r.n_groups, *out);
+    return true;
+  }
   FinBatch batch{};
   for (size_t pi = 0; pi < kp.parts.size(); pi++) { out->names.push_back(output_name(plan, kp.parts[pi].expr)); out->cols.push_back(decode_key_column(r, kp.parts[pi], (int)pi, batch)); }
   append_aggregate_columns(plan, r, agg_nodes, specs, node.exprs, batch, *out);
diff --git a/polars_amd/csrc/engine.hpp b/polars_amd/csrc/engine.hpp
--- a/polars_amd/csrc/engine.hpp
+++ b/polars_amd/csrc/engine.hpp
@@ -55,6 +55,7 @@
 bool describe_filter_fusion(Plan& plan, int root, fused::Shape* shape, std::string* why_not);
 void encoded_set_decimal_min_rows(int64_t min_rows);
 int64_t encoded_decimal_min_rows();
+int last_groupby_tail();
 
 }
 }
diff --git a/polars_amd/csrc/groupby_tail.hpp b/polars_amd/csrc/groupby_tail.hpp
--- /dev/null
+++ b/polars_amd/csrc/groupby_tail.hpp
@@ -0,0 +1,85 @@
+#pragma once
+#include <stdint.h>
+
+#ifndef PLX_HD
+#if defined(__HIPCC__) || defined(__HIP__)
+#define PLX_HD __host__ __device__
+#else
+#define PLX_HD
+#endif
+#endif
+
+namespace plx {
+namespace gbt {
+
+constexpr uint32_t kTailLayoutVersion = 1;
+constexpr int kTailMaxCols = 24;
+constexpr int kTailMaxSlots = 4096;
+constexpr int kTailMaxWords = kTailMaxSlots / 64;
+constexpr uint32_t kTailHeaderBytes = 16;
+
+struct TailHeader {
+  uint32_t n_groups, oob, version, zero;
+};
+struct TailLayout {
+  uint32_t n_cols;
+  uint32_t words;
+  uint32_t values_off[kTailMaxCols];
+  uint32_t values_bytes[kTailMaxCols];
+  uint32_t valid_off[kTailMaxCols];
+  uint32_t total;
+};
+
+PLX_HD inline uint32_t tail_dtype_width(int dt) {
+  switch (dt) {
+    case 1: case 5: return 1;
+    case 2: case 6: return 2;
+    case 3: case 7: case 9: return 4;
+    case 4: case 8: case 10: return 8;
+    default: return 0;
+  }
+}
+PLX_HD inline uint32_t tail_align16(uint32_t x) { return (x + 15u) & ~15u; }
+
+PLX_HD inline void tail_layout(TailLayout* L, int G, const int32_t* dtypes, const uint8_t* nullable, int n_cols) {
+  if (n_cols > kTailMaxCols) n_cols = kTailMaxCols;
+  L->n_cols = (uint32_t)n_cols;
+  L->words = ((uint32_t)G + 63u) / 64u;
+  uint32_t at = kTailHeaderBytes;
+  for (int j = 0; j < n_cols; j++) {
+    const uint32_t w = tail_dtype_width(dtypes[j]);
+    L->values_off[j] = at;
+    L->values_bytes[j] = w ? (uint32_t)G * w : L->words * 8u;
+    at = tail_align16(at + L->values_bytes[j]);
+    L->valid_off[j] = 0;
+    if (nullable[j]) { L->valid_off[j] = at; at = tail_align16(at + L->words * 8u); }
+  }
+  for (int j = n_cols; j < kTailMaxCols; j++) { L->values_off[j] = 0; L->values_bytes[j] = 0; L->valid_off[j] = 0; }
+  L->total = at;
+}
+PLX_HD inline bool tail_block_fits(const TailLayout& L, uint64_t limit) { return (uint64_t)L.total <= limit; }
+
+PLX_HD inline uint32_t tail_popc64(uint64_t x) {
+  x = x - ((x >> 1) & 0x5555555555555555ull);
+  x = (x & 0x3333333333333333ull) + ((x >> 2) & 0x3333333333333333ull);
+  x = (x + (x >> 4)) & 0x0f0f0f0f0f0f0f0full;
+  return (uint32_t)((x * 0x0101010101010101ull) >> 56);
+}
+PLX_HD inline uint32_t tail_rank_bases(const uint64_t* occ, uint32_t words, uint32_t* base) {
+  uint32_t n = 0;
+  for (uint32_t w = 0; w < words; w++) { base[w] = n; n += tail_popc64(occ[w]); }
+  return n;
+}
+PLX_HD inline uint32_t tail_rank_of(const uint64_t* occ, const uint32_t* base, uint32_t slot) {
+  const uint32_t w = slot >> 6, b = slot & 63u;
+  return base[w] + tail_popc64(occ[w] & ((1ull << b) - 1ull));
+}
+PLX_HD inline uint64_t tail_rank_word(uint64_t bits, uint32_t w, uint32_t n_groups) {
+  const uint64_t lo = (uint64_t)w * 64u;
+  if (lo >= n_groups) return 0;
+  const uint64_t left = n_groups - lo;
+  return left >= 64 ? bits : bits & ((1ull << left) - 1ull);
+}
+
+}
+}
diff --git a/polars_amd/csrc/kernels_fused.hip b/polars_amd/csrc/kernels_fused.hip
--- a/polars_amd/csrc/kernels_fused.hip
+++ b/polars_amd/csrc/kernels_fused.hip
@@ -1,5 +1,6 @@
 #include "fused_sinks.hpp"
 #include "fused_cells.hpp"
+#include "groupby_tail.hpp"
 #include "kernels.hpp"
 #include "kernels_fused.hpp"
 #include "variance.hpp"
@@ -868,6 +869,90 @@
   hipLaunchKernelGGL(finalize_batch_kernel, dim3(grid_for(G, kBlock)), dim3(kBlock), 0, stream(), (const unsigned long long*)acc, n_aggs, G, b);
   PLX_HIP(hipGetLastError());
 }
+static_assert(gbt::kTailMaxCols == kMaxFinJobs, "the layout holds a piece per finalize job");
+__global__ __launch_bounds__(kBlock) void groupby_tail_kernel(const unsigned long long* __restrict__ acc, int n_aggs, int G, int len_idx,
+                                                              const unsigned int* __restrict__ oob, FinBatch b, unsigned char* __restrict__ block) {
+  __shared__ unsigned long long slot_of[gbt::kTailMaxSlots];
+  __shared__ uint64_t occ[gbt::kTailMaxWords];
+  __shared__ uint32_t base[gbt::kTailMaxWords];
+  __shared__ gbt::TailLayout L;
+  __shared__ int32_t dts[kMaxFinJobs];
+  __shared__ uint8_t nul[kMaxFinJobs];
+  __shared__ uint32_t n_sh;
+  const int lane = lane_id(), wave = threadIdx.x >> 6;
+  const uint32_t words = ((uint32_t)G + 63u) >> 6;
+  for (uint32_t w = wave; w < words; w += kBlock / 64) {
+    const uint32_t s = w * 64 + lane;
+    const uint64_t m = ballot(s < (uint32_t)G && acc[(size_t)s * n_aggs + len_idx] != 0);
+    if (lane == 0) occ[w] = m;
+  }
+  if ((int)threadIdx.x < b.n) {
+    const FinJob& job = b.jobs[threadIdx.x];
+    dts[threadIdx.x] = job.is_key ? (int32_t)job.kd.dtype : (int32_t)job.fs.out_dtype;
+    nul[threadIdx.x] = job.out_valid ? 1 : 0;
+  }
+  __syncthreads();
+  if (threadIdx.x == 0) n_sh = gbt::tail_rank_bases(occ, words, base);
+  if (threadIdx.x == 64) gbt::tail_layout(&L, G, dts, nul, b.n);
+  __syncthreads();
+  const uint32_t n = n_sh;
+  for (uint32_t w = wave; w < words; w += kBlock / 64) {
+    const uint32_t s = w * 64 + lane;
+    if ((occ[w] >> lane) & 1) slot_of[gbt::tail_rank_of(occ, base, s)] = s;
+  }
+  __syncthreads();
+  const uint32_t n_jobs = (uint32_t)b.n;
+  for (uint32_t t = wave; t < words * n_jobs; t += kBlock / 64) {
+    const uint32_t w = t / n_jobs, g = w * 64 + lane;
+    {
+      const int j = (int)(t - w * n_jobs);
+      const FinJob& job = b.jobs[j];
+      void* copy = block + L.values_off[j];
+      bool valid = false, bit = false;
+      if (g < n) {
+        if (job.is_key) {
+          valid = decode_one(slot_of, nullptr, job.kd, job.out, g, bit);
+          decode_one(slot_of, nullptr, job.kd, copy, g, bit);
+        } else {
+          const unsigned long long* cell = acc + (size_t)slot_of[g] * n_aggs;
+          valid = finalize_one(cell, job.fs, job.out, g);
+          finalize_one(cell, job.fs, copy, g);
+        }
+      }
+      if (job.is_key && job.kd.dtype == PLX_BOOL) {
+        const uint64_t bb = gbt::tail_rank_word(ballot(bit), w, n);
+        if (lane == 0) { reinterpret_cast<uint64_t*>(job.out)[w] = bb; reinterpret_cast<uint64_t*>(copy)[w] = bb; }
+      }
+      if (job.out_valid) {
+        const uint64_t m = gbt::tail_rank_word(ballot(valid), w, n);
+        if (lane == 0) { job.out_valid[w] = m; reinterpret_cast<uint64_t*>(block + L.valid_off[j])[w] = m; }
+      }
+    }
+  }
+  if ((int)threadIdx.x < b.n) {
+    const FinJob& job = b.jobs[threadIdx.x];
+    if (job.is_key && job.kd.dtype == PLX_BOOL) reinterpret_cast<uint64_t*>(job.out)[words] = 0;
+    if (job.out_valid) job.out_valid[words] = 0;
+  }
+  if (threadIdx.x == 0) {
+    gbt::TailHeader* h = reinterpret_cast<gbt::TailHeader*>(block);
+    h->n_groups = n; h->oob = oob ? *oob : 0u; h->version = gbt::kTailLayoutVersion; h->zero = 0;
+  }
+}
+void groupby_tail(const uint64_t* acc, int n_aggs, int G, int len_idx, const unsigned int* oob, const FinBatch& b, void* block) {
+  PLX_REQUIRE(G >= 1 && G <= gbt::kTailMaxSlots && b.n >= 1 && b.n <= kMaxFinJobs && len_idx >= 0 && len_idx < n_aggs, PLX_ERR_INVALID, "groupby_tail: arguments out of range");
+  ProfileScope ps("groupby_tail", (uint64_t)G * 8 * (uint64_t)n_aggs, (uint64_t)G);
+  hipLaunchKernelGGL(groupby_tail_kernel, dim3(1), dim3(kBlock), 0, stream(), (const unsigned long long*)acc, n_aggs, G, len_idx, oob, b, (unsigned char*)block);
+  PLX_HIP(hipGetLastError());
+}
+static std::atomic<int> g_groupby_tail{-1};
+bool groupby_tail_knob() {
+  int v = g_groupby_tail.load(std::memory_order_relaxed);
+  if (v < 0) { const char* e = getenv("PLX_GROUPBY_TAIL"); v = (e && e[0] == '0') ? 0 : 1; g_groupby_tail.store(v, std::memory_order_relaxed); }
+  return v != 0;
+}
+void set_groupby_tail(bool on) { g_groupby_tail.store(on ? 1 : 0, std::memory_order_relaxed); }
+
 void finalize_aggs(const uint64_t* acc, int n_aggs, int64_t G, const FinalSpec& sp, void* out, uint64_t* out_valid) {
   if (G == 0) return;
   hipLaunchKernelGGL(finalize_kernel, dim3(grid_for(G, kBlock)), dim3(kBlock), 0, stream(), (const unsigned long long*)acc, n_aggs, G, sp, out, out_valid);
diff --git a/polars_amd/csrc/kernels_fused.hpp b/polars_amd/csrc/kernels_fused.hpp
--- a/polars_amd/csrc/kernels_fused.hpp
+++ b/polars_amd/csrc/kernels_fused.hpp
@@ -64,6 +64,9 @@
 double sample_sortedness(const ColumnPtr& c);
 bool sample_minmax(const ColumnPtr& c, int64_t* mn, int64_t* mx, int blocks = 64);
 void finalize_batch(const uint64_t* acc, int n_aggs, int64_t G, const fused::FinBatch& b);
+void groupby_tail(const uint64_t* acc, int n_aggs, int G, int len_idx, const unsigned int* oob, const fused::FinBatch& b, void* block);
+bool groupby_tail_knob();
+void set_groupby_tail(bool on);
 void decode_key(const uint64_t* packed, const uint8_t* kvalid, int64_t G, const fused::KeyDecode& kd, void* out, uint64_t* out_valid);
 
 }
diff --git a/polars_amd/csrc/kernels_join.hip b/polars_amd/csrc/kernels_join.hip
--- a/polars_amd/csrc/kernels_join.hip
+++ b/polars_amd/csrc/kernels_join.hip
@@ -120,6 +120,7 @@
   if (!idx->len) return;
   plx_scalar s; s.u = kNoRow;
   ColumnPtr ok = ops::cmp_scalar(PLX_NE, idx, s);
+  drop_host_mirror(*idx);
   idx->validity = ok->values; idx->null_count = -1;
   if (column_null_count(idx) == 0) { idx->validity = nullptr; idx->null_count = 0; }
 }
diff --git a/polars_amd/csrc/ops.cpp b/polars_amd/csrc/ops.cpp
--- a/polars_amd/csrc/ops.cpp
+++ b/polars_amd/csrc/ops.cpp
@@ -367,7 +367,7 @@
   if (!c->validity || column_null_count(c) == 0) {
     if (!c->validity) return c;
     auto same = std::make_shared<Column>(*c);
-    same->validity = nullptr; same->null_count = 0;
+    same->validity = nullptr; same->null_count = 0; same->host.reset();
     return same;
   }
   auto out = std::make_shared<Column>();
```
